# Guillaume-SOULIER/SOS-Radiative-Transfer

Hardware: AMD Instinct MI355X
Metric: SOS columns/sec to 1e-4 convergence (Ntau=200, Nmu=128) (higher is better)
Workload: dtype f64

## Files before the change

include/sosrt.h:

```cpp
#ifndef SOSRT_H
#define SOSRT_H

#ifdef __cplusplus
extern "C" {
#endif

typedef struct sosrt_handle sosrt_t;

#define SOSRT_OK              0
#define SOSRT_E_INVALID      -1
#define SOSRT_E_HIP          -2
#define SOSRT_E_STATE        -3
#define SOSRT_E_NOMEM        -4

#define SOSRT_COL_OK           0
#define SOSRT_COL_INDEXERROR   1
#define SOSRT_COL_MAXORDERS    2
#define SOSRT_COL_INTERNAL     3

#define SOSRT_GEOM_THREE_ZONE  0
#define SOSRT_GEOM_SINGLE_SLAB 1

#define SOSRT_SURFACE_NONE       0
#define SOSRT_SURFACE_SPECULAR   1
// ... 49 lines not shown
int sosrt_set_columns_zones(sosrt_t* h, int B, int surface, int nzmax, const int* nz, const int* zone_r0, const int* zone_mix,
                            const double* mu0, const double* grd_alb, const double* alb_atm, const double* dtau_atm,
                            const double* zone_alb_aer, const double* zone_dtau_aer, const double* tauStar_tot);

int sosrt_first_order(sosrt_t* h, int B, const double* tau, const double* P0_atm, const double* P0_aer,
                      double* I1_out);
int sosrt_source(sosrt_t* h, int B, const double* In_1, double* Jn_out);
int sosrt_transport(sosrt_t* h, int B, const double* tau, const double* Jn, double* In_out, int* status_out);

int sosrt_solve(sosrt_t* h, int B, const double* tau, const double* P0_atm, const double* P0_aer,
                double tol, const double* I1_in,
                double* I_out, double* I_saved_out, int* n_orders_out, int* status_out);
int sosrt_solve_dev(sosrt_t* h, int B, const double* d_tau, const double* d_P0_atm, const double* d_P0_aer,
                    double tol, const double* d_I1_in,
                    double* d_I_out, double* d_I_saved_out, int* d_n_orders_out, int* d_status_out);
int sosrt_last_solve_stats(sosrt_t* h, int* max_orders_run, long long* sum_orders);

int sosrt_fluxes(sosrt_t* h, int B, const double* tau, const double* I, int beam_norm,
                 double* flux_down, double* flux_up);

int sosrt_epilogue_dev(sosrt_t* h, int B, const double* d_tau, const double* d_I, int beam_norm,
                       const double* d_z_profile, double* d_flux_down, double* d_flux_up, double* d_diffusivity,
                       double* d_heating_rate, double* d_net_toa);
int sosrt_epilogue(sosrt_t* h, int B, int beam_norm, const double* z_profile, double* flux_down, double* flux_up,
                   double* diffusivity, double* heating_rate, double* net_toa);

#define SOSRT_PHASE_ISO       0
#define SOSRT_PHASE_RAYLEIGH  1
#define SOSRT_PHASE_HG        2
#define SOSRT_PHASE_TABLE     3
int sosrt_phase_table(sosrt_t* h, const double* tab_mu, const double* tab_p, int ntab);
int sosrt_phase_table_dev(sosrt_t* h, const double* d_tab_mu, const double* d_tab_p, int ntab);

#define SOSRT_MIE_MAX_X 20000.0
#define SOSRT_MIE_MAX_MX 200000.0
#define SOSRT_MIE_MAX_WORKSPACE (2ull << 30)
int sosrt_mie_ensembles(sosrt_t* h, int S, const double* wl, const double* m_re, const double* m_im, const double* r_m,
                        const double* sig, int nb_radius, double r_min, double r_max, int ntab, double* p_out, double* bulk_out);
int sosrt_mie_ensembles_dev(sosrt_t* h, int S, const double* wl, const double* m_re, const double* m_im, const double* r_m,
                            const double* sig, int nb_radius, double r_min, double r_max, int ntab, double* d_p_out,
                            double* d_bulk_out);
int sosrt_mie_efficiencies(sosrt_t* h, int K, const double* m_re, const double* m_im, const double* x, double* out);
int sosrt_mie_timing(sosrt_t* h, double* ms );

int sosrt_phase_p0_dev(sosrt_t* h, int B, int kind, double g, const double* d_mu0, double* d_P0_out);
int sosrt_phase_p0(sosrt_t* h, int B, int kind, double g, const double* mu0, double* P0_out);
int sosrt_phase_matrix(sosrt_t* h, int kind, double g, double* P_out);
int sosrt_phase_matrix_dev(sosrt_t* h, int kind, double g, double* d_P_out);

#define SOSRT_MAX_MODES 64
int sosrt_phase_modes(sosrt_t* h, int kind, double g, int m_first, int m_count, int nphi, double* P_out);
int sosrt_phase_p0_modes_dev(sosrt_t* h, int B, int kind, double g, int m_first, int m_count, int nphi, const double* d_mu0,
                             double* d_P0_out);
int sosrt_phase_p0_modes(sosrt_t* h, int B, int kind, double g, int m_first, int m_count, int nphi, const double* mu0,
                         double* P0_out);
int sosrt_set_order_targets(sosrt_t* h, const int* d_targets);
int sosrt_azimuth_accumulate_dev(sosrt_t* h, int B, int m, const double* d_Im, int nlev, const int* d_levels, int nphi_out,
                                 const double* d_phi, double* d_out);

int sosrt_comm_unique_id(void* id_out);
int sosrt_comm_init(sosrt_t* h, int rank, int world, const void* unique_id);
int sosrt_gather(sosrt_t* h, int root, const long long* counts, const double* d_send, double* d_recv);
int sosrt_comm_destroy(sosrt_t* h);

int sosrt_limit_mu_down(sosrt_t* h, int R, int idx, const double* rows, double* out);
int sosrt_asymptotic_down(sosrt_t* h, int R, int stride, const int* len, const double* J, const double* tau,
                          const double* tau_t, const double* mu, double* out);

int sosrt_plan_weights(sosrt_t* h, double* w_out );
int sosrt_plan_fold(sosrt_t* h, int which , double* W_out );
int sosrt_plan_fix_table(sosrt_t* h, int idx, int* s0, int* ns, double* C_out);
int sosrt_plan_fix_count(double tau_ref, int N);
#define SOSRT_PLAN_GEMM_DENSE        0
#define SOSRT_PLAN_GEMM_LIVE64       1
#define SOSRT_PLAN_GEMM_LIVE32       2
#define SOSRT_PLAN_GEMM_LIVE32_DEEP  3
#define SOSRT_PLAN_GEMM_LIVE16_REGS  4
#define SOSRT_PLAN_TRANSPORT_GENERAL 0
#define SOSRT_PLAN_TRANSPORT_FAST    1
#define SOSRT_PLAN_TRANSPORT_RING    3
#define SOSRT_PLAN_TRANSPORT_SCAN    4
int sosrt_plan_launch(sosrt_t* h, int batch, int live, int surface, int zones, int cus, int* out );

#define SOSRT_K_GEMM      0
#define SOSRT_K_TRANSPORT 1
#define SOSRT_K_FIRST     2
#define SOSRT_K_SMALLMU   3
#define SOSRT_K_ORDER_LOOP 4
#define SOSRT_K_COUNT     5
int sosrt_profile_enable(sosrt_t* h, int on);
int sosrt_profile_reset(sosrt_t* h);
int sosrt_profile_get(sosrt_t* h, int kernel, double* total_ms, long long* launches, double* work );

int sosrt_debug_stamps(sosrt_t* h, unsigned long long* d_stamps);

int sosrt_microbench(sosrt_t* h, int which, double* result);

#ifdef __cplusplus
}
#endif
#endif
```

sos-radiative-transfer_amd/csrc/api.hip:

```cpp
#include <hip/hip_runtime.h>

#include <algorithm>
#include <cmath>
#include <cstdarg>
#include <cstdio>
#include <cstdlib>
#include <chrono>
#include <cstring>
#include <mutex>
#include <new>
#include <string>
#include <vector>

#include "../../include/sosrt.h"
#include "comm.hpp"
#include "kernels.hpp"
#include "plan.hpp"

using namespace sosrt;

namespace {
thread_local std::string g_err;

int fail(int code, const char* fmt, ...) {
// ... 32 lines not shown
    int saved_slots = 0;
    bool gpu = false;
    hipStream_t own_stream = nullptr, stream = nullptr;
    static constexpr int kMaxGroups = 2;
    hipStream_t stream2 = nullptr;
    hipEvent_t ev_fork = nullptr, ev_join = nullptr;
    int ngroups = 1, want_groups = 0, split_min = 48;
    int split_at = -1;
    int prio2 = 0;
    int coresident_pad = 0;
    int diag_ks_mult = 1;
    int coresident_slots = 3;
    double stagger = 1.0;
    int gb[kMaxGroups + 1] = {0, 0, 0};
    int main_off[kMaxGroups + 1] = {0, 0, 0};
    int slab_off[kMaxGroups + 1] = {0, 0, 0};
    Plan plan;
    bool have_grid = false, have_phase = false, have_aer = false, have_cols = false;
    int B = 0, geom = 0, surface = 0;
    std::vector<double> Wa_h, Wr_h;
    Grid g{};
    double *d_mu = nullptr, *d_Wa = nullptr, *d_Wr = nullptr, *d_wfdn = nullptr, *d_wfup = nullptr;
    double *d_w = nullptr;
    int first_order_mode = SOSRT_FIRST_ORDER_CODED;
    double *d_phi = nullptr;
    double *d_z = nullptr;
    double *d_tab = nullptr;
    double *d_modetab = nullptr;
    size_t modetab_cap = 0;
    const int* d_targets = nullptr;
    int ntab = 0;
    char* d_mie = nullptr;
    char* h_mie = nullptr;
    size_t mie_cap = 0, mie_hcap = 0;
    hipEvent_t mie_ev = nullptr, mie_t[4] = {nullptr, nullptr, nullptr, nullptr};
    bool mie_timed = false;
    bool resident = false;
    int resident_B = 0;
    FixTab* d_fix = nullptr;
    int* d_small = nullptr;
    int *d_idx_up = nullptr, *d_idx_down = nullptr;
    int *d_nz = nullptr, *d_zr0 = nullptr, *d_zmix = nullptr;
    double *d_zwr = nullptr, *d_zdtr = nullptr;
    int max_nz = 1;
    bool simple_zones = true;
    double* d_scal = nullptr;
    ColDesc* d_desc = nullptr;
    double *d_rca = nullptr, *d_rcr = nullptr;
    int* d_slabrows = nullptr;
    int* d_mainrows = nullptr;
    int nslab = 0, nmain = 0;
    int max_main = 0, max_slab = 0;
    static constexpr int kMaxMixGroups = 32;
    static constexpr int kMaxMixGroupsSets = 128;
    static constexpr size_t kMixCacheBytes = 256ull << 20;
    int mix_groups_max = 1 << 30;
    bool wr_on_device = false;
    int nsets = 1;
    std::vector<std::vector<double>> Wrx_h;
    double* d_Wrsets = nullptr;
    size_t wrsets_capacity = 0;
    double* d_Wrsets_s = nullptr;
    size_t wrsets_s_capacity = 0;
    int* d_mixset = nullptr;
    int max_set_used = 0;
    int p0_zones = 0;
    double* d_P0rz = nullptr;
    size_t p0rz_capacity = 0;
    std::vector<int> c_nz, c_zr0, c_zmix, c_zset;
    std::vector<double> c_zwr, c_zdtr, c_alb_atm, c_dtau_atm;
    int mix_groups = 0;
    bool mix_dirty = true;
    double *d_Wmix = nullptr, *d_mixca = nullptr, *d_mixcr = nullptr;
    int* d_mixgroup = nullptr;
    int* d_slabtilegroup = nullptr;
    int contraction = SOSRT_CONTRACT_F64;
    double asymmetry = 0;
    bool sym_ok = false;
    bool sym_dirty = true, symmix_dirty = true, symsets_dirty = true;
    double *d_Wa_s = nullptr, *d_Wr_s = nullptr, *d_Wmix_s = nullptr;
    int lr_rank = -1;
    double lr_residual = 0;
    double *d_lrU = nullptr, *d_lrV = nullptr;
    size_t mixs_capacity = 0;
    float *d_Wa32 = nullptr, *d_Wmix32 = nullptr;
    size_t mix32_capacity = 0;
    bool w32_dirty = true;
    int* d_livelist = nullptr;
    size_t mix_capacity = 0;
    double *d_tau = nullptr, *d_P0a = nullptr, *d_P0r = nullptr;
    double *d_Jn = nullptr, *d_InA = nullptr, *d_InB = nullptr, *d_I = nullptr, *d_E = nullptr;
    int use_etab = 1;
    int *d_active = nullptr, *d_norders = nullptr, *d_status = nullptr, *d_redo = nullptr, *d_erep = nullptr;
    int *d_nactive_sets = nullptr, *d_nactive = nullptr;
    int nactive_set = 0;
    unsigned long long* d_tauhash = nullptr;
    int transport_mode = 3;
    int scan_cols = 200;
    bool ring_ok = false, scan_ok = false, scan_split_ok = false;
    int scan_split = 1;
    int cu_count = 0;
    double* d_scan_scratch = nullptr;
    int* d_scan_sync = nullptr;
    int gemm_tail_cols = 1 << 30;
    double gemm_tail_frac = 0.6;
    int gemm_small_cols = 200;
    int dense_live_list = 1;
    int gemm_regs_cols = -1;
    bool fast_ok = false;
    double* d_ratio = nullptr;
    int* h_pub = nullptr;
    bool need_small = true;
    int pub_seq = 0;
    int last_max_orders = 0;
    long long last_sum_orders = 0;
    Prof prof[kMaxGroups];
    int order_loop = 0;
    double ol_frac = 0.5;
    int* d_olsync = nullptr;
    int* h_oldone = nullptr;
    unsigned long long* d_ollog = nullptr;
    int ol_launches = 0, ol_refused = 0;
    bool ol_group_used[kMaxGroups] = {false, false};
    Rccl::comm_t comm = nullptr;
    int comm_rank = -1, comm_world = 0;
};

namespace {

size_t field_elems(const sosrt_handle* h) { return (size_t)h->max_batch * h->L * h->D; }

template <class T>
int dalloc(T** p, size_t n) {
    hipError_t e = hipMalloc((void**)p, n * sizeof(T));
    if (e != hipSuccess) return fail(SOSRT_E_NOMEM, "hipMalloc of %zu bytes failed: %s", n * sizeof(T), hipGetErrorString(e));
    return 0;
}

void mie_linspace(double a, double b, int n, double* out) {
    if (n == 1) { out[0] = a; return; }
    const double step = (b - a) / (n - 1);
    for (int i = 0; i < n; ++i) {
        volatile double t = i * step;
        out[i] = t + a;
    }
    out[n - 1] = b;
}

bool prof_room(Prof& p) {
    if (p.used + 2 > p.ev.size()) {
        const size_t n0 = p.ev.size();
        p.ev.resize(n0 + 4096);
        for (size_t i = n0; i < p.ev.size(); ++i)
            if (hipEventCreateWithFlags(&p.ev[i], hipEventDisableSystemFence) != hipSuccess) { p.ev.resize(i); break; }
        if (p.used + 2 > p.ev.size()) return false;
    }
    if (p.nint >= p.kind.size()) {
        const size_t n = p.kind.size() + 4096;
        p.kind.resize(n, -1); p.first.resize(n, 0); p.last.resize(n, 0);
    }
    return true;
}
hipStream_t group_stream(sosrt_handle* h, int grp) { return grp == 0 ? h->stream : h->stream2; }
void prof_begin(sosrt_handle* h, int kind, int grp = 0) {
    Prof& p = h->prof[grp];
    p.open = -1;
// ... 118 lines not shown
    if (!std::isfinite(wmax)) return -1;
    int rank = -1;
    for (int r = 0; r <= kLowRankMax; ++r) {
        size_t at = 0;
        const double amax = absmax(R, &at);
        *residual = wmax > 0 ? amax / wmax : amax;
        if (std::isnan(amax)) return -1;
        if (amax <= SOSRT_LOWRANK_TOL * wmax) { rank = r; break; }
        if (r == kLowRankMax) return -1;
        const int i = (int)(at / D), j = (int)(at % D);
        const long double piv = R[at];
        for (int k = 0; k < D; ++k) Ut[(size_t)r * D + k] = (double)(R[(size_t)k * D + j] / piv);
        for (int m = 0; m < D; ++m) V[(size_t)r * D + m] = R[(size_t)i * D + m];
        for (int k = 0; k < D; ++k) {
            const long double u = Ut[(size_t)r * D + k];
            double* row = &R[(size_t)k * D];
            const double* v = &V[(size_t)r * D];
            for (int m = 0; m < D; ++m) row[m] = (double)(row[m] - u * v[m]);
        }
    }
    double res = 0;
    for (int k = 0; k < D; ++k)
        for (int m = 0; m < D; ++m) {
            long double uv = 0;
            for (int q = 0; q < rank; ++q) uv += (long double)Ut[(size_t)q * D + k] * V[(size_t)q * D + m];
            const double d = std::fabs((double)(W[(size_t)k * D + m] - uv));
            if (!(d <= res)) res = d;
        }
    *residual = wmax > 0 ? res / wmax : res;
    return (res <= SOSRT_LOWRANK_TOL * wmax) ? rank : -1;
}

int ensure_matrices(sosrt_handle* h, hipStream_t s) {
    const Grid& g = h->g;
    const size_t per = (size_t)g.Dp * g.Wld;
    const bool mixed = h->mix_groups > 0 && h->mix_dirty;
    if (mixed) {
        prof_break(h);
        const bool sets = h->max_set_used > 0;
        launch_wmix(s, per, h->mix_groups, h->d_Wa, sets ? h->d_Wrsets : h->d_Wr, h->d_mixca, h->d_mixcr, h->d_Wmix,
                    sets ? h->d_mixset : nullptr);
        h->mix_dirty = false;
        h->symmix_dirty = true;
    }
    if (!use_sym(h)) return 0;
    if (h->sym_dirty) {
        prof_break(h);
        if (!h->d_Wa_s) { if (int e = dalloc(&h->d_Wa_s, per)) return e; }
        if (!h->d_Wr_s) { if (int e = dalloc(&h->d_Wr_s, per)) return e; }
        launch_symfold(s, 1, g.N, g.D, g.Dp, g.Wld, h->d_Wa, h->d_Wa_s);
        launch_symfold(s, 1, g.N, g.D, g.Dp, g.Wld, h->d_Wr, h->d_Wr_s);
        h->sym_dirty = false;
        h->symsets_dirty = true;
    }
    if (h->symsets_dirty && h->nsets > 1 && h->mix_groups == 0 && h->max_set_used > 0) {
        prof_break(h);
        {
            if (per * h->nsets > h->wrsets_s_capacity) {
                if (h->d_Wrsets_s) hipFree(h->d_Wrsets_s);
                h->d_Wrsets_s = nullptr; h->wrsets_s_capacity = 0;
                if (int e = dalloc(&h->d_Wrsets_s, per * h->nsets)) return e;
                h->wrsets_s_capacity = per * h->nsets;
            }
            launch_symfold(s, h->nsets, g.N, g.D, g.Dp, g.Wld, h->d_Wrsets, h->d_Wrsets_s);
        }
        h->symsets_dirty = false;
    }
    if (h->mix_groups > 0 && h->symmix_dirty) {
        prof_break(h);
        const size_t need = per * h->mix_groups;
        if (need > h->mixs_capacity) {
            if (h->d_Wmix_s) hipFree(h->d_Wmix_s);
            h->d_Wmix_s = nullptr; h->mixs_capacity = 0;
            if (int e = dalloc(&h->d_Wmix_s, need)) return e;
            h->mixs_capacity = need;
        }
        launch_symfold(s, h->mix_groups, g.N, g.D, g.Dp, g.Wld, h->d_Wmix, h->d_Wmix_s);
        h->symmix_dirty = false;
    }
    return 0;
}

void run_source(sosrt_handle* h, const double* In_1, double* Jn, const int* active, int tail_cols = 0, int pub_tag = 0,
                int grp = -1, bool all_live = false, bool regs_tile = false, int dense_live_cap = 0) {
    const int g0 = grp < 0 ? 0 : grp, g1 = grp < 0 ? h->ngroups : grp + 1;
    const int pg = grp < 0 ? 0 : grp;
    hipStream_t s = group_stream(h, pg);
    GemmArgs ga;
    ga.A = In_1; ga.Wa = h->d_Wa; ga.Wr = h->d_Wr; ga.ca = h->d_rca; ga.cr = h->d_rcr;
    if (h->nslab > 0) {
        ga.rows_main = h->d_mainrows + h->main_off[g0];
        ga.n_main = h->main_off[g1] - h->main_off[g0];
    } else {
        ga.rows_main = nullptr;
        ga.n_main = (h->gb[g1] - h->gb[g0]) * h->L;
        ga.A = In_1 + (size_t)h->gb[g0] * h->L * h->D;
        Jn += (size_t)h->gb[g0] * h->L * h->D;
        ga.ca = h->d_rca + (size_t)h->gb[g0] * h->L;
        ga.cr = h->d_rcr + (size_t)h->gb[g0] * h->L;
        if (active) active += h->gb[g0];
    }
    ga.rows_slab = h->d_slabrows + h->slab_off[g0]; ga.n_slab = h->slab_off[g1] - h->slab_off[g0];
    ga.D = h->g.D; ga.Dp = h->g.Dp; ga.Wld = h->g.Wld; ga.L = h->L; ga.C = Jn; ga.active = active;
    if (grp >= 0 && h->ngroups > 1) ga.pad_lds = h->coresident_pad;
    if (pub_tag) {
        ga.nactive = h->d_nactive + pg; ga.need_small = h->d_nactive + sosrt_handle::kMaxGroups;
        ga.host_pub = h->h_pub + 8 * pg; ga.tag = pub_tag;
    }
    ga.check_tiles = all_live ? 0 : 1;
    if (ensure_matrices(h, s)) return;
    if (h->mix_groups > 0) {
        ga.Wmix = h->d_Wmix; ga.mix_group = h->d_mixgroup; ga.slab_tile_group = h->d_slabtilegroup + h->slab_off[g0] / 32;
    }
    const bool two_pass_sets = h->mix_groups == 0 && h->max_set_used > 0 && h->nslab > 0;
    if (two_pass_sets) {
        ga.Wr = h->d_Wrsets; ga.mix_group = h->d_mixgroup; ga.slab_tile_group = h->d_slabtilegroup + h->slab_off[g0] / 32;
    }
    if (use_lowrank(h)) { ga.lr_rank = h->lr_rank; ga.lrU = h->d_lrU; ga.lrV = h->d_lrV; }
    if (use_sym(h)) {
        ga.sym = 1; ga.Ks = (h->g.N + GEMM_KC - 1) / GEMM_KC * GEMM_KC;
#ifdef SOSRT_DIAG
        if (h->diag_ks_mult > 1 && ga.Ks * h->diag_ks_mult <= h->g.Dp) ga.Ks *= h->diag_ks_mult;
#endif
        ga.Wa = h->d_Wa_s; ga.Wr = two_pass_sets ? h->d_Wrsets_s : h->d_Wr_s;
        if (ga.Wmix) ga.Wmix = h->d_Wmix_s;
    }
    if (h->contraction == SOSRT_CONTRACT_F32) {
        if (h->w32_dirty) {
            prof_break(h);
            const size_t per = (size_t)h->g.Dp * h->g.Wld;
            launch_to_float(s, per, h->d_Wa, h->d_Wa32);
            if (h->mix_groups > 0) launch_to_float(s, per * h->mix_groups, h->d_Wmix, h->d_Wmix32);
            h->w32_dirty = false;
        }
        prof_begin(h, SOSRT_K_GEMM, pg);
        launch_gemm_f32(s, ga, h->d_Wa32, h->d_Wmix32);
        prof_end(h, SOSRT_K_GEMM, pg);
        return;
    }
    prof_begin(h, SOSRT_K_GEMM, pg);
    if (tail_cols > 0 && active && h->nslab >= 0) {
        ga.col0 = h->nslab > 0 ? h->gb[g0] : 0; ga.B = h->gb[g1] - h->gb[g0];
        ga.max_main = h->max_main; ga.max_slab = h->max_slab;
        ga.idx_up = h->nslab > 0 ? h->d_idx_up : nullptr; ga.idx_down = h->nslab > 0 ? h->d_idx_down : nullptr;
        ga.live_list = h->d_livelist + h->gb[g0]; ga.live_cap = tail_cols;
        launch_gemm_tail(s, ga, tail_cols, tail_cols <= h->gemm_small_cols, regs_tile);
    } else {
        if (dense_live_cap > 0 && active && h->nslab >= 0) {
            ga.col0 = h->nslab > 0 ? h->gb[g0] : 0; ga.B = h->gb[g1] - h->gb[g0];
            ga.live_list = h->d_livelist + h->gb[g0]; ga.live_cap = dense_live_cap;
        }
        launch_gemm(s, ga);
    }
    prof_end(h, SOSRT_K_GEMM, pg);
}

struct SolveShape {
    bool ring_like = false;
    bool fast = false;
    int nzcap = kRingZones;
    int ring_mode = 1;
};
SolveShape solve_shape(const sosrt_handle* h, int max_nz) {
    SolveShape sh;
    sh.ring_like = h->transport_mode >= 2 && h->ring_ok && (max_nz <= kRingZones || transport_ring_fits(h->g, max_nz));
    sh.fast = h->transport_mode >= 1 && h->fast_ok && (max_nz <= kRingZones || sh.ring_like);
    sh.nzcap = max_nz > kRingZones ? max_nz : kRingZones;
    sh.ring_mode = (h->transport_mode >= 2 && h->ring_ok) ? 3 : 1;
    return sh;
}
struct OrderInputs {
    int nb = 0;
    int known = 0;
    int surface = SOSRT_SURFACE_NONE;
    bool simple_zones = true;
    bool slabs_mixed = true;
    bool need_small = false;
    bool saving = false;
    int orders_left = 1 << 30;
    int cu_share = 0;
};
struct LaunchPlan {
    int tail_cols = 0;
    int live_cap = 0;
    int gemm = SOSRT_PLAN_GEMM_DENSE;
    int transport = SOSRT_PLAN_TRANSPORT_GENERAL;
    int parts = 1;
    int repair = 0;
    int order_loop = 0;
    int ol_parts = 0;
    int ol_grid = 0;
};
LaunchPlan plan_order(const sosrt_handle* h, const SolveShape& sh, const OrderInputs& in) {
    LaunchPlan pl;
    const Grid& g = h->g;
    const bool live_tiling = h->contraction != SOSRT_CONTRACT_F32 && in.simple_zones && in.known <= h->gemm_tail_cols &&
                             (in.known <= h->gemm_tail_frac * in.nb || in.nb <= h->gemm_small_cols) &&
                             (in.known < in.nb || in.nb <= h->gemm_small_cols);
    pl.tail_cols = live_tiling ? in.known : 0;
    pl.gemm = !live_tiling ? SOSRT_PLAN_GEMM_DENSE
                           : (pl.tail_cols <= h->gemm_small_cols ? ((use_sym(h) && pl.tail_cols <= 32) ? SOSRT_PLAN_GEMM_LIVE32_DEEP : SOSRT_PLAN_GEMM_LIVE32)
                                                                 : SOSRT_PLAN_GEMM_LIVE64);
    {
        const int nct = (g.D + GEMM_BN - 1) / GEMM_BN;
        const int auto_cap = (3 * h->cu_count / 2) / (((g.L + 15) / 16 + 1) * nct);
        const int cap = h->gemm_regs_cols >= 0 ? h->gemm_regs_cols : auto_cap;
        if (live_tiling && use_sym(h) && pl.tail_cols <= cap && 16 * (g.D + 2) * 8 <= 150 * 1024 &&
            ((g.N + GEMM_KC - 1) / GEMM_KC * GEMM_KC) % 64 == 0) pl.gemm = SOSRT_PLAN_GEMM_LIVE16_REGS;
    }
    pl.live_cap = live_tiling ? pl.tail_cols : ((h->contraction != SOSRT_CONTRACT_F32 && h->dense_live_list && in.known < in.nb) ? in.known : 0);
    {
        const int cols_now = pl.live_cap > 0 ? pl.live_cap : in.nb;
        const int split_cap = sh.ring_mode == 3 ? h->cu_count : 4 * h->cu_count;
        const bool can_split = h->scan_split && h->scan_split_ok && transport_scan_parts(g) * cols_now <= split_cap &&
                               (in.surface == SOSRT_SURFACE_SPECULAR || in.surface == SOSRT_SURFACE_NONE);
        const bool want_scan = h->transport_mode == 4 || (h->transport_mode == 3 && cols_now <= h->scan_cols);
        const bool split = can_split && transport_scan_fits(g, sh.nzcap, true) && (sh.fast || (h->use_etab && h->transport_mode >= 3));
        const bool scan = want_scan && ((sh.fast && sh.ring_mode == 3 && h->scan_ok && transport_scan_fits(g, sh.nzcap, false)) || split);
        pl.transport = scan ? SOSRT_PLAN_TRANSPORT_SCAN
                            : (!sh.fast ? SOSRT_PLAN_TRANSPORT_GENERAL : (sh.ring_mode == 3 ? SOSRT_PLAN_TRANSPORT_RING : SOSRT_PLAN_TRANSPORT_FAST));
        if (scan && split) pl.parts = transport_scan_parts(g);
        pl.repair = (h->N - 3 > 61 && pl.transport == SOSRT_PLAN_TRANSPORT_FAST) ? 1 : 0;
    }
    if (h->order_loop && in.cu_share > 0 && h->transport_mode == 3 && sh.fast && sh.ring_mode == 3 && sh.nzcap <= kRingZones &&
        use_sym(h) && in.simple_zones && in.slabs_mixed && !in.saving && !in.need_small && in.orders_left >= 1 &&
        in.known <= kOrderLoopMaxCols) {
        Grid gt = g;
        gt.nsmall = 0;
        const bool split_ok = h->scan_split && (in.surface == SOSRT_SURFACE_SPECULAR || in.surface == SOSRT_SURFACE_NONE) && order_loop_ok(gt, true);
        const int sp = order_loop_parts(gt, true);
        if (split_ok && sp * in.known <= h->ol_frac * in.cu_share) {
            pl.order_loop = 1; pl.ol_parts = sp;
        } else if (order_loop_ok(gt, false) && in.known <= h->ol_frac * in.cu_share) {
            pl.order_loop = 1; pl.ol_parts = 1;
        }
        if (pl.order_loop) pl.ol_grid = in.cu_share;
    }
    return pl;
}

std::mutex g_ol_mutex;
int g_ol_held[64];
int ol_acquire(int device, int total, int want, int least) {
    if (device < 0 || device >= 64) return 0;
    std::lock_guard<std::mutex> lk(g_ol_mutex);
    int got = total - g_ol_held[device];
    if (got > want) got = want;
    if (got < least || got <= 0) return 0;
    g_ol_held[device] += got;
    return got;
}
void ol_release(int device, int n) {
    if (device < 0 || device >= 64 || n <= 0) return;
    std::lock_guard<std::mutex> lk(g_ol_mutex);
    g_ol_held[device] -= n;
}

}

extern "C" {

const char* sosrt_last_error(void) { return g_err.c_str(); }
int sosrt_version(void) { return SOSRT_VERSION; }

int sosrt_plan_fix_count(double tau_ref, int N) { return fix_count(tau_ref, N); }

int sosrt_create(int device, int L, int N, int max_batch, int max_orders, sosrt_t** out) {
    if (!out) return fail(SOSRT_E_INVALID, "out is null");
    *out = nullptr;
    if (L < 2) return fail(SOSRT_E_INVALID, "nb_layers must be >= 2 (got %d)", L);
    if (N < 4) return fail(SOSRT_E_INVALID, "nb_angles must be >= 4 (got %d)", N);
    if (N > 1024) return fail(SOSRT_E_INVALID, "nb_angles must be <= 1024 (got %d)", N);
    if (max_batch < 1 || max_orders < 1) return fail(SOSRT_E_INVALID, "max_batch and max_orders must be >= 1");
    {
        const int nt = (N + 63) / 64 * 64;
        const size_t need = (size_t)(3 * (size_t)L + nt + nt / 64 + 4) * sizeof(double);
        if (need > 64 * 1024)
            return fail(SOSRT_E_INVALID, "nb_layers = %d does not fit: at most %d layers at nb_angles = %d", L,
                        (int)((64 * 1024 / sizeof(double) - nt - nt / 64 - 4) / 3), N);
    }
    sosrt_handle* h = new (std::nothrow) sosrt_handle();
    if (!h) return fail(SOSRT_E_NOMEM, "out of host memory");
    h->device = device; h->L = L; h->N = N; h->D = 2 * N; h->max_batch = max_batch; h->max_orders = max_orders;
    h->order_budget = max_orders;
    h->saved_slots = max_orders;
    h->gpu = device >= 0;
    h->cu_count = 256;
    if (const char* ev = getenv("SOSRT_ETAB")) h->use_etab = atoi(ev);
    if (const char* ev = getenv("SOSRT_CONTRACT"))
        if (strcmp(ev, "full") == 0) h->contraction = SOSRT_CONTRACT_F64_FULL;
    if (const char* ev = getenv("SOSRT_TRANSPORT"))
        h->transport_mode = strcmp(ev, "general") == 0 ? 0 : (strcmp(ev, "ring") == 0 ? 2 : (strcmp(ev, "scan") == 0 ? 4 : (strcmp(ev, "auto") == 0 ? 3 : 1)));
    if (const char* ev = getenv("SOSRT_SCAN_COLS")) h->scan_cols = atoi(ev);
    if (const char* ev = getenv("SOSRT_SCAN_SPLIT")) h->scan_split = atoi(ev);
    if (const char* ev = getenv("SOSRT_GEMM_TAIL")) h->gemm_tail_cols = atoi(ev);
    if (const char* ev = getenv("SOSRT_GEMM_TAIL_FRAC")) h->gemm_tail_frac = atof(ev);
    if (const char* ev = getenv("SOSRT_GEMM_SMALL")) h->gemm_small_cols = atoi(ev);
    if (const char* ev = getenv("SOSRT_DENSE_LIVE_LIST")) h->dense_live_list = atoi(ev) != 0;
    if (const char* ev = getenv("SOSRT_GEMM_REGS")) h->gemm_regs_cols = atoi(ev);
    if (const char* ev = getenv("SOSRT_GROUPS")) h->want_groups = atoi(ev) >= 2 ? 2 : (atoi(ev) == 1 ? 1 : 0);
    if (const char* ev = getenv("SOSRT_SPLIT_MIN")) h->split_min = atoi(ev);
    if (const char* ev = getenv("SOSRT_MIX_GROUPS")) h->mix_groups_max = atoi(ev);
#ifdef SOSRT_DIAG
    if (const char* ev = getenv("SOSRT_STAGGER")) h->stagger = atof(ev);
    if (const char* ev = getenv("SOSRT_GROUP_SPLIT")) h->split_at = atoi(ev);
    if (const char* ev = getenv("SOSRT_GROUP_PRIO")) h->prio2 = atoi(ev);
    if (const char* ev = getenv("SOSRT_GEMM_PAD_LDS")) h->coresident_pad = atoi(ev);
    if (const char* ev = getenv("SOSRT_GEMM_KS_MULT")) h->diag_ks_mult = atoi(ev);
#endif
    if (const char* ev = getenv("SOSRT_GROUP_RING_SLOTS")) h->coresident_slots = atoi(ev);
    if (const char* ev = getenv("SOSRT_ORDER_LOOP")) h->order_loop = atoi(ev) != 0;
    if (const char* ev = getenv("SOSRT_RING_SLOTS")) g_ring_slots = atoi(ev);
#ifdef SOSRT_RING_DEBUG
    if (const char* ev = getenv("SOSRT_RING_DEBUG")) g_ring_debug = atoi(ev);
#endif
    Grid& g = h->g;
    g.L = L; g.N = N; g.D = 2 * N;
    g.Dp = (g.D + GEMM_KC - 1) / GEMM_KC * GEMM_KC;
    g.Wld = (g.D + GEMM_BN - 1) / GEMM_BN * GEMM_BN;
    if (h->gpu) {
        int e = 0;
        auto body = [&]() -> int {
            HIPCHK(hipSetDevice(device));
            HIPCHK(hipStreamCreateWithFlags(&h->own_stream, hipStreamDefault));
            h->stream = h->own_stream;
            HIPCHK(hipEventCreateWithFlags(&h->ev_fork, hipEventDisableTiming));
            HIPCHK(hipEventCreateWithFlags(&h->ev_join, hipEventDisableTiming));
            const size_t mb = max_batch, fe = field_elems(h);
            if ((e = dalloc(&h->d_mu, g.D))) return e;
            if ((e = dalloc(&h->d_Wa, (size_t)g.Dp * g.Wld))) return e;
            if ((e = dalloc(&h->d_Wr, (size_t)g.Dp * g.Wld))) return e;
            if ((e = dalloc(&h->d_lrU, (size_t)kLowRankMax * g.D))) return e;
            if ((e = dalloc(&h->d_lrV, (size_t)kLowRankMax * g.D))) return e;
            if ((e = dalloc(&h->d_wfdn, N))) return e;
            if ((e = dalloc(&h->d_wfup, N))) return e;
            if ((e = dalloc(&h->d_w, g.D))) return e;
            if ((e = dalloc(&h->d_phi, 2 * kNPhi))) return e;
            if ((e = dalloc(&h->d_z, L))) return e;
            if ((e = dalloc(&h->d_fix, 4))) return e;
            if ((e = dalloc(&h->d_small, N))) return e;
            if ((e = dalloc(&h->d_idx_up, mb))) return e;
            if ((e = dalloc(&h->d_idx_down, mb))) return e;
            if ((e = dalloc(&h->d_nz, mb))) return e;
            if ((e = dalloc(&h->d_zr0, mb * kMaxZones))) return e;
            if ((e = dalloc(&h->d_zmix, mb * kMaxZones))) return e;
            if ((e = dalloc(&h->d_zwr, mb * kMaxZones))) return e;
            if ((e = dalloc(&h->d_zdtr, mb * kMaxZones))) return e;
            if ((e = dalloc(&h->d_scal, 7 * mb))) return e;
            if ((e = dalloc(&h->d_desc, mb))) return e;
            if ((e = dalloc(&h->d_rca, mb * L))) return e;
            if ((e = dalloc(&h->d_rcr, mb * L))) return e;
            if ((e = dalloc(&h->d_slabrows, mb * L + 64 * (size_t)sosrt_handle::kMaxMixGroupsSets * sosrt_handle::kMaxGroups))) return e;
            if ((e = dalloc(&h->d_slabtilegroup, mb * L / 32 + 2 * sosrt_handle::kMaxMixGroupsSets * sosrt_handle::kMaxGroups + 2))) return e;
            if ((e = dalloc(&h->d_mainrows, mb * L))) return e;
            if ((e = dalloc(&h->d_tau, mb * L))) return e;
            if ((e = dalloc(&h->d_P0a, mb * g.D))) return e;
            if ((e = dalloc(&h->d_P0r, mb * g.D))) return e;
            if ((e = dalloc(&h->d_Jn, fe))) return e;
            if ((e = dalloc(&h->d_InA, fe))) return e;
            if ((e = dalloc(&h->d_InB, fe))) return e;
            if ((e = dalloc(&h->d_I, fe))) return e;
            if ((e = dalloc(&h->d_E, fe))) return e;
            if ((e = dalloc(&h->d_active, mb))) return e;
            if ((e = dalloc(&h->d_norders, mb))) return e;
            if ((e = dalloc(&h->d_status, mb))) return e;
            if ((e = dalloc(&h->d_nactive_sets, 2 * (sosrt_handle::kMaxGroups + 1)))) return e;
            HIPCHK(hipMemset(h->d_nactive_sets, 0, 2 * (sosrt_handle::kMaxGroups + 1) * sizeof(int)));
            h->d_nactive = h->d_nactive_sets;
            if ((e = dalloc(&h->d_redo, mb))) return e;
            if ((e = dalloc(&h->d_erep, mb))) return e;
            if ((e = dalloc(&h->d_mixgroup, mb))) return e;
            if ((e = dalloc(&h->d_livelist, mb))) return e;
            if ((e = dalloc(&h->d_mixca, sosrt_handle::kMaxMixGroupsSets))) return e;
            if ((e = dalloc(&h->d_mixcr, sosrt_handle::kMaxMixGroupsSets))) return e;
            if ((e = dalloc(&h->d_mixset, sosrt_handle::kMaxMixGroupsSets))) return e;
            if ((e = dalloc(&h->d_tauhash, mb))) return e;
            if ((e = dalloc(&h->d_ratio, mb))) return e;
            if ((e = dalloc(&h->d_scan_scratch, mb * transport_scan_scratch_doubles()))) return e;
            if ((e = dalloc(&h->d_scan_sync, 2 * mb))) return e;
            if ((e = dalloc(&h->d_olsync, sosrt_handle::kMaxGroups * order_loop_sync_ints(kOrderLoopMaxCols)))) return e;
            HIPCHK(hipHostMalloc((void**)&h->h_oldone, 2 * sosrt_handle::kMaxGroups * sizeof(int), hipHostMallocCoherent));
            memset(h->h_oldone, 0, 2 * sosrt_handle::kMaxGroups * sizeof(int));
            HIPCHK(hipMemset(h->d_scan_sync, 0, 2 * mb * sizeof(int)));
            HIPCHK(hipDeviceGetAttribute(&h->cu_count, hipDeviceAttributeMultiprocessorCount, device));
            HIPCHK(hipHostMalloc((void**)&h->h_pub, (8 * sosrt_handle::kMaxGroups + 2) * sizeof(int), hipHostMallocCoherent));
            memset(h->h_pub, 0, (8 * sosrt_handle::kMaxGroups + 2) * sizeof(int));

            HIPCHK(hipMemset(h->d_Wa, 0, (size_t)g.Dp * g.Wld * sizeof(double)));
            HIPCHK(hipMemset(h->d_Wr, 0, (size_t)g.Dp * g.Wld * sizeof(double)));
            HIPCHK(hipMemset(h->d_status, 0, mb * sizeof(int)));
            HIPCHK(hipMemset(h->d_redo, 0, mb * sizeof(int)));
            HIPCHK(hipMemset(h->d_tau, 0, mb * L * sizeof(double)));
            return 0;
        };
        if ((e = body())) { sosrt_destroy(h); return e; }
        g.mu = h->d_mu; g.Wa = h->d_Wa; g.Wr = h->d_Wr; g.fix = h->d_fix; g.small_lanes = h->d_small;
        g.wflux_dn = h->d_wfdn; g.wflux_up = h->d_wfup; g.nsmall = 0;
    }
    *out = h;
    return 0;
}

int sosrt_destroy(sosrt_t* h) {
    if (!h) return 0;
    if (h->gpu) {
        hipSetDevice(h->device);
        if (h->comm) { rccl().CommDestroy(h->comm); h->comm = nullptr; }
        if (h->own_stream) hipStreamSynchronize(h->own_stream);
        void* ptrs[] = {h->d_mu, h->d_Wa, h->d_Wr, h->d_wfdn, h->d_wfup, h->d_fix, h->d_small, h->d_idx_up,
                        h->d_idx_down, h->d_scal, h->d_desc, h->d_rca, h->d_rcr, h->d_slabrows, h->d_mainrows, h->d_tau, h->d_P0a,
                        h->d_P0r, h->d_Jn, h->d_InA, h->d_InB, h->d_I, h->d_E, h->d_active, h->d_norders, h->d_status,
                        h->d_nactive_sets, h->d_ratio, h->d_redo, h->d_erep, h->d_tauhash, h->d_Wmix, h->d_mixca, h->d_mixcr,
                        h->d_mixgroup, h->d_Wa_s, h->d_Wr_s, h->d_Wmix_s, h->d_scan_scratch, h->d_scan_sync, h->d_w, h->d_phi, h->d_z, h->d_tab, h->d_slabtilegroup, h->d_livelist, h->d_Wa32, h->d_Wmix32, h->d_nz, h->d_zr0, h->d_zmix, h->d_zwr, h->d_zdtr, h->d_olsync, h->d_ollog, h->d_modetab, h->d_lrU, h->d_lrV, h->d_Wrsets, h->d_Wrsets_s, h->d_mixset, h->d_P0rz};
        for (void* p : ptrs)
            if (p) hipFree(p);
        if (h->h_pub) hipHostFree(h->h_pub);
        if (h->h_oldone) hipHostFree(h->h_oldone);
        if (h->d_mie) hipFree(h->d_mie);
        if (h->h_mie) hipHostFree(h->h_mie);
        if (h->mie_ev) hipEventDestroy(h->mie_ev);
        for (auto& e : h->mie_t)
            if (e) hipEventDestroy(e);

        for (auto& p : h->prof)
            for (auto& e : p.ev) hipEventDestroy(e);
        if (h->stream2) { hipStreamSynchronize(h->stream2); hipStreamDestroy(h->stream2); }
        if (h->ev_fork) hipEventDestroy(h->ev_fork);
        if (h->ev_join) hipEventDestroy(h->ev_join);
        if (h->own_stream) hipStreamDestroy(h->own_stream);
    }
    delete h;
    return 0;
}

int sosrt_set_stream(sosrt_t* h, void* s) {
    if (int e = need_gpu(h)) return e;
    h->stream = (hipStream_t)s;
    return 0;
}

int sosrt_use_own_stream(sosrt_t* h) {
    if (int e = need_gpu(h)) return e;
    h->stream = h->own_stream;
    return 0;
}

int sosrt_set_saved_orders(sosrt_t* h, int slots) {
    if (!h) return fail(SOSRT_E_INVALID, "null handle");
    if (slots < 1 || slots > h->max_orders) return fail(SOSRT_E_INVALID, "slots must be in 1..max_orders=%d (got %d)", h->max_orders, slots);
    h->saved_slots = slots;
    return 0;
}

int sosrt_set_order_budget(sosrt_t* h, int max_orders) {
    if (!h) return fail(SOSRT_E_INVALID, "null handle");
    if (max_orders < 1 || max_orders > h->max_orders)
        return fail(SOSRT_E_INVALID, "the order budget must be in 1..max_orders=%d of sosrt_create (got %d)", h->max_orders, max_orders);
    h->order_budget = max_orders;
    return 0;
}

int sosrt_set_first_order(sosrt_t* h, int mode) {
    if (int e = need_gpu(h)) return e;
    if (mode != SOSRT_FIRST_ORDER_CODED && mode != SOSRT_FIRST_ORDER_README) return fail(SOSRT_E_INVALID, "unknown first-order mode %d", mode);
    if (mode == SOSRT_FIRST_ORDER_README && (h->nsets > 1 || h->p0_zones > 0))
        return fail(SOSRT_E_INVALID, "SOSRT_FIRST_ORDER_README reads one aerosol matrix: it cannot be combined with several phase sets");
    if (mode == SOSRT_FIRST_ORDER_README && h->geom != SOSRT_GEOM_THREE_ZONE)
        return fail(SOSRT_E_INVALID, "the README's Lambertian first order needs the three-zone geometry (it has a surface)");
    h->first_order_mode = mode;
    return 0;
}

int sosrt_set_contraction(sosrt_t* h, int mode) {
    if (int e = need_gpu(h)) return e;
    if (mode != SOSRT_CONTRACT_F64 && mode != SOSRT_CONTRACT_F32 && mode != SOSRT_CONTRACT_F64_FULL && mode != SOSRT_CONTRACT_F64_DENSE) return fail(SOSRT_E_INVALID, "unknown contraction mode %d", mode);
    if (mode == SOSRT_CONTRACT_F32) {
        HIPCHK(hipSetDevice(h->device));
        const size_t per = (size_t)h->g.Dp * h->g.Wld;
        if (!h->d_Wa32) { if (int e = dalloc(&h->d_Wa32, per)) return e; }
        h->w32_dirty = true;
    }
    h->contraction = mode;
    return 0;
}

int sosrt_set_order_loop(sosrt_t* h, int mode) {
    if (!h) return fail(SOSRT_E_INVALID, "null handle");
    if (mode < 0 || mode > 2) return fail(SOSRT_E_INVALID, "order-loop mode must be 0, 1 or 2 (got %d)", mode);
    h->order_loop = mode;
    return 0;
}

int sosrt_order_loop_stats(sosrt_t* h, int* launches, int* refused, long long* column_orders) {
    if (!h) return fail(SOSRT_E_INVALID, "null handle");
    if (launches) *launches = h->ol_launches;
    if (refused) *refused = h->ol_refused;
    if (column_orders) {
        *column_orders = 0;
        if (h->gpu && h->ol_launches > 0) {
            HIPCHK(hipSetDevice(h->device));
            HIPCHK(hipStreamSynchronize(h->stream));
            if (h->stream2) HIPCHK(hipStreamSynchronize(h->stream2));
            for (int k = 0; k < sosrt_handle::kMaxGroups; ++k) {
                if (!h->ol_group_used[k]) continue;
                int v = 0;
                HIPCHK(hipMemcpy(&v, h->d_olsync + (size_t)k * order_loop_sync_ints(kOrderLoopMaxCols) + kOlOrders, sizeof v, hipMemcpyDeviceToHost));
                *column_orders += v;
            }
        }
    }
    return 0;
}

int sosrt_plan_launch(sosrt_t* h, int batch, int live, int surface, int zones, int cus, int* out) {
    if (!h || !out) return fail(SOSRT_E_INVALID, "null argument");
    if (!h->have_grid) return fail(SOSRT_E_STATE, "sosrt_set_grid has not been called");
    if (batch < 1 || live < 0 || live > batch) return fail(SOSRT_E_INVALID, "need 0 <= live <= batch, batch >= 1");
    if (zones < 1 || zones > kMaxZones) return fail(SOSRT_E_INVALID, "zones must be in 1..%d", kMaxZones);
    int want = h->want_groups;
    if (want == 0) want = batch > h->split_min ? 2 : 1;
    const int ng = (want >= 2 && batch >= h->split_min && batch >= 2) ? 2 : 1;
    const int nb = ng == 2 ? batch / 2 : batch;
    const int saved_cus = h->cu_count;
    if (cus > 0) h->cu_count = cus;
    const SolveShape sh = solve_shape(h, zones);
    OrderInputs oi;
    oi.nb = nb; oi.known = live < nb ? live : nb; oi.surface = surface;
    oi.simple_zones = zones == 3 || zones == 1;
    oi.cu_share = h->cu_count / ng;
    const bool saved_sym = h->sym_ok;
    if (!h->have_phase) h->sym_ok = true;
    const LaunchPlan pl = plan_order(h, sh, oi);
    h->sym_ok = saved_sym;
    h->cu_count = saved_cus;
    out[0] = ng; out[1] = pl.gemm; out[2] = pl.tail_cols; out[3] = pl.transport; out[4] = pl.parts; out[5] = pl.repair;
    out[6] = pl.order_loop; out[7] = pl.ol_parts; out[8] = pl.ol_grid;
    return 0;
}

int sosrt_phase_asymmetry(sosrt_t* h, double* asymmetry, int* uses_symmetry) {
    if (!h) return fail(SOSRT_E_INVALID, "null handle");
    if (!h->have_phase) return fail(SOSRT_E_STATE, "sosrt_set_phase has not been called");
    if (asymmetry) *asymmetry = h->asymmetry;
    if (uses_symmetry) *uses_symmetry = use_sym(h) ? 1 : 0;
    return 0;
}

int sosrt_phase_rank(sosrt_t* h, int* rank, double* residual, int* uses) {
    if (!h) return fail(SOSRT_E_INVALID, "null handle");
    if (!h->have_phase) return fail(SOSRT_E_STATE, "sosrt_set_phase has not been called");
    if (rank) *rank = h->lr_rank;
    if (residual) *residual = h->lr_residual;
    if (uses) *uses = use_lowrank(h) ? 1 : 0;
    return 0;
}

int sosrt_synchronize(sosrt_t* h) {
    if (int e = need_gpu(h)) return e;
    HIPCHK(hipStreamSynchronize(h->stream));
    return 0;
}

int sosrt_set_grid(sosrt_t* h, const double* mu) {
    if (!h || !mu) return fail(SOSRT_E_INVALID, "null argument");
    for (int k = 0; k < h->D; ++k)
        if (!std::isfinite(mu[k])) return fail(SOSRT_E_INVALID, "mu[%d] is not finite", k);
    for (int k = 0; k < h->N; ++k) {
        if (!(mu[k] <= 0)) return fail(SOSRT_E_INVALID, "mu[%d]=%g: the first nb_angles directions must be <= 0", k, mu[k]);
        if (!(mu[h->N + k] >= 0)) return fail(SOSRT_E_INVALID, "mu[%d]=%g: the last nb_angles directions must be >= 0", h->N + k, mu[h->N + k]);
    }
    h->plan.set_grid(h->N, mu);
    for (int b = 0; b < 4; ++b)
        if (h->plan.fix[b].idx > kFixMaxIdx) return fail(SOSRT_E_INVALID, "nb_angles too large for the extrapolation tables");
    h->have_grid = true;
    h->have_phase = false;
    h->fast_ok = transport_fast_ok(h->plan);
    if (h->gpu) {
        HIPCHK(hipSetDevice(h->device));
        HIPCHK(hipMemcpy(h->d_mu, mu, h->D * sizeof(double), hipMemcpyHostToDevice));
        HIPCHK(hipMemcpy(h->d_wfdn, h->plan.wflux_dn.data(), h->N * sizeof(double), hipMemcpyHostToDevice));
        HIPCHK(hipMemcpy(h->d_wfup, h->plan.wflux_up.data(), h->N * sizeof(double), hipMemcpyHostToDevice));
        HIPCHK(hipMemcpy(h->d_w, h->plan.w.data(), h->D * sizeof(double), hipMemcpyHostToDevice));
        {
            double phi[kNPhi], tab[2 * kNPhi];
            const double step = 3.141592653589793 / (kNPhi - 1);
            for (int q = 0; q < kNPhi; ++q) phi[q] = q * step;
            phi[kNPhi - 1] = 3.141592653589793;
            for (int q = 0; q < kNPhi; ++q) {
                tab[q] = std::cos(0 - phi[q]);
                tab[kNPhi + q] = ((q > 0 ? phi[q] - phi[q - 1] : 0.0) + (q + 1 < kNPhi ? phi[q + 1] - phi[q] : 0.0)) / 2;
            }
            HIPCHK(hipMemcpy(h->d_phi, tab, sizeof tab, hipMemcpyHostToDevice));
        }
        std::vector<FixTab> ft(4);
        for (int b = 0; b < 4; ++b) {
            const FixTable& t = h->plan.fix[b];
            memset(&ft[b], 0, sizeof(FixTab));
            ft[b].idx = t.idx; ft[b].s0 = t.s0; ft[b].ns = t.ns;
            for (size_t i = 0; i < t.C.size(); ++i) ft[b].C[i] = t.C[i];
        }
        HIPCHK(hipMemcpy(h->d_fix, ft.data(), 4 * sizeof(FixTab), hipMemcpyHostToDevice));
        h->g.nsmall = (int)h->plan.small_lanes.size();
        if (h->g.nsmall)
            HIPCHK(hipMemcpy(h->d_small, h->plan.small_lanes.data(), h->g.nsmall * sizeof(int), hipMemcpyHostToDevice));
    }
    h->g.nsmall = (int)h->plan.small_lanes.size();
    h->ring_ok = h->fast_ok && transport_ring_ok(h->g);
    h->scan_ok = h->ring_ok && transport_scan_ok(h->g);
    h->scan_split_ok = transport_scan_split_ok(h->g);
    return 0;
}

static int mix_group_cap(const sosrt_handle* h, bool sets);
static int set_phase_impl(sosrt_handle* h, const double* P_atm, int S, const double* P_aer, const double* d_P_aer = nullptr) {
    if (!h || !P_atm) return fail(SOSRT_E_INVALID, "null argument");
    if (!h->have_grid) return fail(SOSRT_E_STATE, "sosrt_set_grid has not been called");
    if (h->have_cols && h->max_set_used >= (S > 0 ? S : 1))
        return fail(SOSRT_E_INVALID, "the current columns use aerosol set %d, but only %d set(s) are given (sosrt_set_columns resets them to set 0)",
                    h->max_set_used, S > 0 ? S : 1);
// ... 530 lines not shown
    const double* src = I1 + (size_t)b * n;
    for (size_t i = tid; i < n; i += blockDim.x) {
        const double v = src[i];
        In1[(size_t)b * n + i] = v;
        I[(size_t)b * n + i] = v;
        if (saved) saved[(size_t)b * saved_col_stride + i] = v;
    }
    if (tid == 0) {
        double a = 1.0 / src[g.N];
        for (int m = g.N + 1; m < g.D; ++m) { const double x = 1.0 / src[m]; if (x > a) a = x; }
        const double* last = src + (size_t)(g.L - 1) * g.D;
        double bb = 1.0 / last[0];
        for (int m = 1; m < g.N; ++m) { const double x = 1.0 / last[m]; if (x > bb) bb = x; }
        const double r = (bb > a) ? bb : a;
        cv.ratio[b] = r; cv.norders[b] = 1; cv.status[b] = SOSRT_COL_OK;
        const int go = conv_go(cv, b, 1, r) ? 1 : 0;
        cv.active[b] = go;
        if (go) atomicAdd(cv.nactive, 1);
    }
}

int sosrt_solve_dev(sosrt_t* h, int B, const double* d_tau, const double* d_P0_atm, const double* d_P0_aer, double tol,
                    const double* d_I1_in, double* d_I_out, double* d_I_saved_out, int* d_n_orders_out,
                    int* d_status_out) {
    if (int e = check_ready(h, B, true)) return e;
    if (!d_tau || !d_I_out) return fail(SOSRT_E_INVALID, "null argument");
    if (!d_I1_in && !d_P0_atm) return fail(SOSRT_E_INVALID, "P0_atm is required unless I1 is supplied");
    if (!d_I1_in && h->geom == SOSRT_GEOM_THREE_ZONE && !d_P0_aer) return fail(SOSRT_E_INVALID, "three-zone geometry needs P0_aer");
    if (h->max_orders >= 65536) return fail(SOSRT_E_INVALID, "max_orders must be < 65536");
    HIPCHK(hipSetDevice(h->device));
    if (int e = ensure_w32(h)) return e;
    hipStream_t s = h->stream;
    const Grid& g = h->g;
    const size_t LD = (size_t)h->L * h->D;
    const size_t saved_stride = (size_t)h->saved_slots * LD;
    const int NG = h->ngroups;

    prof_break(h);
    h->nactive_set ^= 1;
    h->d_nactive = h->d_nactive_sets + h->nactive_set * (sosrt_handle::kMaxGroups + 1);
    SolveSetup su;
    su.zero_next = h->d_nactive_sets + (h->nactive_set ^ 1) * (sosrt_handle::kMaxGroups + 1);
    su.n_zero = sosrt_handle::kMaxGroups + 1;
    su.redo = h->d_redo;
    su.hash = h->d_tauhash;
    su.scan_sync = h->d_scan_sync;
    launch_prepare(s, g, B, h->geom, h->surface, scalars_of(h), d_tau, h->d_desc, h->d_rca, h->d_rcr,
                   h->d_nactive + sosrt_handle::kMaxGroups, su);
    h->need_small = true;
    const int small_tag = ((++h->pub_seq) & 0x3fffffff) | 0x40000000;
    bool small_published = false;
    const SolveShape shape = solve_shape(h, h->max_nz);
    const bool fast = shape.fast;
    const int nzcap = shape.nzcap;
    if (h->use_etab || fast) {
        launch_tau_groups(s, g, B, d_tau, h->d_tauhash, h->d_erep, h->d_nactive + sosrt_handle::kMaxGroups,
                          h->h_pub + 8 * sosrt_handle::kMaxGroups, small_tag);
        launch_attenuation(s, g, B, d_tau, h->d_E, h->d_erep);
        small_published = true;
    }
    if (int e = ensure_matrices(h, s)) return e;
    bool forked = false;
    int ol_held[sosrt_handle::kMaxGroups] = {0, 0};
    auto bail = [&](int code) {
        if (forked && hipEventRecord(h->ev_join, h->stream2) == hipSuccess) (void)hipStreamWaitEvent(s, h->ev_join, 0);
        for (int k = 0; k < NG; ++k)
            if (ol_held[k]) {
                (void)hipStreamSynchronize(group_stream(h, k));
                ol_release(h->device, ol_held[k]);
                ol_held[k] = 0;
            }
        return code;
    };

    struct GroupState {
        int b0 = 0, nb = 0, n = 1, known = 0;
        bool done = false, started = false;
        bool ol_pending = false, ol_off = false;
        int ol_tag = 0;
        unsigned ol_polls = 0;
        double *In_1 = nullptr, *In = nullptr;
        Conv cv;
    } gs[sosrt_handle::kMaxGroups];
    h->ol_launches = 0; h->ol_refused = 0;
    for (bool& u : h->ol_group_used) u = false;
    bool used_order_loop = false;
    const int tagbase = ((++h->pub_seq) & 0x3fff) << 16;
    for (int k = 0; k < NG; ++k) {
        GroupState& q = gs[k];
        q.b0 = h->gb[k]; q.nb = h->gb[k + 1] - h->gb[k]; q.known = q.nb;
        q.In_1 = h->d_InA; q.In = h->d_InB;
        if (!d_I1_in && h->first_order_mode != SOSRT_FIRST_ORDER_README) q.In_1 = d_I_out;
        q.cv = make_conv(h, tol);
        q.cv.active += q.b0; q.cv.norders += q.b0; q.cv.status += q.b0; q.cv.ratio += q.b0; q.cv.redo += q.b0;
        q.cv.nactive = h->d_nactive + k;
        if (h->d_targets) q.cv.target = h->d_targets + q.b0;
    }
    auto start_group = [&](int k) {
        GroupState& q = gs[k];
        q.started = true;
        hipStream_t sg = group_stream(h, k);
        const size_t fo = (size_t)q.b0 * LD;
        prof_begin(h, SOSRT_K_FIRST, k);
        if (d_I1_in)
            hipLaunchKernelGGL(k_init_from_I1, dim3(q.nb), dim3(256), 0, sg, g, d_I1_in + fo, q.In_1 + fo, d_I_out + fo,
                               d_I_saved_out ? d_I_saved_out + (size_t)q.b0 * saved_stride : nullptr, saved_stride, q.cv);
        else if (h->first_order_mode == SOSRT_FIRST_ORDER_README)
            launch_first_order_readme(sg, g, h->d_w, q.nb, d_tau + (size_t)q.b0 * h->L, d_P0_atm + (size_t)q.b0 * g.D,
                                      d_P0_aer ? d_P0_aer + (size_t)q.b0 * g.D : nullptr, h->d_desc + q.b0, q.In_1 + fo,
                                      d_I_out + fo, d_I_saved_out ? d_I_saved_out + (size_t)q.b0 * saved_stride : nullptr,
                                      saved_stride, q.cv, 1);
        else
            launch_first_order(sg, g, q.nb, d_tau + (size_t)q.b0 * h->L, d_P0_atm + (size_t)q.b0 * g.D,
                               d_P0_aer ? d_P0_aer + (size_t)q.b0 * g.D * (h->p0_zones > 0 ? h->p0_zones : 1) : nullptr, h->d_desc + q.b0,
                               d_I_out + fo, nullptr, d_I_saved_out ? d_I_saved_out + (size_t)q.b0 * saved_stride : nullptr, saved_stride,
                               q.cv, 1, h->p0_zones);
        prof_end(h, SOSRT_K_FIRST, k);
    };
    start_group(0);
    if (NG > 1) {
        HIPCHK(hipEventRecord(h->ev_fork, s));
        HIPCHK(hipStreamWaitEvent(h->stream2, h->ev_fork, 0));
        forked = true;
    }
    if (small_published && g.nsmall > 0) {
        volatile int* slot = h->h_pub + 8 * sosrt_handle::kMaxGroups;
        const auto t0 = std::chrono::steady_clock::now();
        for (unsigned it = 1; __atomic_load_n(&slot[1], __ATOMIC_ACQUIRE) != small_tag; ++it) {
            if ((it & 0x3fff) == 0 && std::chrono::steady_clock::now() - t0 > std::chrono::seconds(120))
                return bail(fail(SOSRT_E_HIP, "order loop: no progress for 120 s"));
            __builtin_ia32_pause();
        }
        h->need_small = slot[0] != 0;
    }
    int live_groups = NG, n_max = 1;
    while (live_groups > 0) {
        bool progressed = false;
        for (int k = 0; k < NG; ++k) {
            GroupState& q = gs[k];
            if (q.done) continue;
            if (q.ol_pending) {
                volatile int* dw = h->h_oldone + 2 * k;
                if (__atomic_load_n(&dw[1], __ATOMIC_ACQUIRE) != q.ol_tag) {
                    if ((++q.ol_polls & 0x3fff) != 0) continue;
                    const hipError_t qe = hipStreamQuery(group_stream(h, k));
                    if (qe != hipSuccess && qe != hipErrorNotReady) return bail(fail(SOSRT_E_HIP, "order loop: %s", hipGetErrorString(qe)));
                    if (qe == hipSuccess && __atomic_load_n(&dw[1], __ATOMIC_ACQUIRE) != q.ol_tag)
                        return bail(fail(SOSRT_E_HIP, "order loop: the order-loop launch ended without reporting"));
                    continue;
                }
                const int state = dw[0];
                q.ol_pending = false;
                ol_release(h->device, ol_held[k]);
                ol_held[k] = 0;
                progressed = true;
#ifdef SOSRT_OL_STAMPS
                if (h->d_ollog && getenv("SOSRT_OL_LOG")) {
                    std::vector<unsigned long long> lg(65001);
                    (void)hipStreamSynchronize(group_stream(h, k));
                    (void)hipMemcpy(lg.data(), h->d_ollog, lg.size() * 8, hipMemcpyDeviceToHost);
                    if (FILE* f = fopen(getenv("SOSRT_OL_LOG"), "a")) {
                        fprintf(f, "# launch columns<=%d order0=%d events=%llu\n", q.known, q.n + 1, lg[0]);
                        for (unsigned long long i = 0; i < lg[0] && i < 65000; ++i)
                            fprintf(f, "%llu %llu %llu %llu\n", lg[1 + i] >> 48, (lg[1 + i] >> 40) & 0xff, (lg[1 + i] >> 32) & 0xff, lg[1 + i] & 0xffffffffull);
                        fclose(f);
                    }
                }
// ... 14 lines not shown
                                     w[kOlArrive], w[kOlLeft], q.n + 1, q.known, cols.c_str()));
                }
                q.ol_off = true;
                ++h->ol_refused;
            }
            if (!q.started) {
                const GroupState& p = gs[k - 1];
                if (!(p.done || (p.n >= 2 && p.known <= h->stagger * p.nb))) continue;
                start_group(k);
            }
            progressed = true;
            if (q.n >= h->order_budget) { q.done = true; --live_groups; continue; }
            if (q.n >= 2) {
                const int live = wait_published(h, k, tagbase + q.n - 1);
                if (live < 0) return bail(live);
                if (live == 0) { q.done = true; --live_groups; continue; }
                q.known = live;
            }
            hipStream_t sg = group_stream(h, k);
            const size_t fo = (size_t)q.b0 * LD;
            const double* tau_g = d_tau + (size_t)q.b0 * h->L;
            const int* erep_g = h->d_erep + q.b0;
            OrderInputs oi;
            oi.nb = q.nb; oi.known = q.known; oi.surface = h->surface;
            oi.simple_zones = h->simple_zones; oi.slabs_mixed = h->nslab == 0 || h->mix_groups > 0;
            oi.need_small = g.nsmall > 0 && h->need_small; oi.saving = d_I_saved_out != nullptr;
            oi.orders_left = h->order_budget - q.n;
            oi.cu_share = (q.ol_off || h->d_targets) ? 0 : h->cu_count / NG;
            LaunchPlan pl = plan_order(h, shape, oi);
            if (pl.order_loop) {
                const int got = ol_acquire(h->device, h->cu_count, pl.ol_grid, (int)(pl.ol_parts * q.known / h->ol_frac));
                if (got == 0) { oi.cu_share = 0; pl = plan_order(h, shape, oi); }
                else { pl.ol_grid = got; ol_held[k] = got; }
            }
            if (pl.order_loop && h->order_loop == 2) pl.ol_grid = 2 * h->cu_count;
            if (pl.order_loop) {
                OrderLoopArgs oa;
                Grid gt = g;
                gt.nsmall = 0;
                oa.t = TransportArgs{gt, tau_g, h->d_Jn + fo, nullptr, d_I_out + fo, nullptr, 0, h->d_desc + q.b0, q.cv, 0, 1, h->d_E, erep_g, nullptr};
                oa.t.nzcap = kRingZones;
                oa.t.scan_split = pl.ol_parts > 1 ? 1 : 0;
                oa.t.scan_scratch = h->d_scan_scratch + (size_t)q.b0 * transport_scan_scratch_doubles();
                oa.t.scan_sync = h->d_scan_sync + 2 * q.b0;
                GemmArgs& ga = oa.gm;
                ga.A = nullptr; ga.Wa = h->d_Wa_s; ga.Wr = h->d_Wr_s; ga.ca = h->d_rca; ga.cr = h->d_rcr;
                ga.D = g.D; ga.Dp = g.Dp; ga.Wld = g.Wld; ga.L = h->L; ga.C = h->d_Jn;
                ga.sym = 1; ga.Ks = (g.N + GEMM_KC - 1) / GEMM_KC * GEMM_KC;
                if (use_lowrank(h)) { ga.lr_rank = h->lr_rank; ga.lrU = h->d_lrU; ga.lrV = h->d_lrV; }
                ga.max_main = h->max_main; ga.max_slab = h->max_slab;
                ga.idx_up = h->nslab > 0 ? h->d_idx_up : nullptr; ga.idx_down = h->nslab > 0 ? h->d_idx_down : nullptr;
                if (h->mix_groups > 0) { ga.Wmix = h->d_Wmix_s; ga.mix_group = h->d_mixgroup; }
                oa.in0 = q.In_1;
                oa.gbufP = q.In;
                oa.gbufQ = (q.In_1 == d_I_out) ? h->d_InA : q.In_1;
                oa.bufP = oa.gbufP + fo; oa.bufQ = oa.gbufQ + fo;
                oa.order0 = q.n + 1; oa.kmax = h->order_budget - q.n;
                oa.B = q.nb; oa.col0 = q.b0;
                oa.fixcap = (int)(0.06 * g.N) + 1;
                oa.sync = h->d_olsync + (size_t)k * order_loop_sync_ints(kOrderLoopMaxCols);
                oa.host_done = h->h_oldone + 2 * k;
                oa.tag = q.ol_tag = ((++h->pub_seq) & 0x3fffffff) | 0x40000000;
#ifdef SOSRT_OL_STAMPS
                if (getenv("SOSRT_OL_LOG")) {
                    if (!h->d_ollog) { if (int e = dalloc(&h->d_ollog, 65001)) return bail(e); }
                    HIPCHK(hipMemsetAsync(h->d_ollog, 0, 8, sg));
                    oa.log = h->d_ollog;
                }
#endif
                prof_break(h);
                HIPCHK(hipMemsetAsync(oa.sync, 0, order_loop_sync_ints(q.known) * sizeof(int), sg));
                prof_begin(h, SOSRT_K_ORDER_LOOP, k);
                const hipError_t le = launch_order_loop(sg, pl.ol_grid, pl.ol_parts > 1, oa);
                prof_end(h, SOSRT_K_ORDER_LOOP, k);
                if (le != hipSuccess) return bail(fail(SOSRT_E_HIP, "order-loop launch failed: %s", hipGetErrorString(le)));
                q.ol_pending = true;
                used_order_loop = true;
                ++h->ol_launches;
                continue;
            }
            const int n = ++q.n;
            n_max = n > n_max ? n : n_max;
            const int tail_cols = pl.tail_cols;
            run_source(h, q.In_1, h->d_Jn, h->d_active, tail_cols, tagbase + n - 1, k, q.known == q.nb, pl.gemm == SOSRT_PLAN_GEMM_LIVE16_REGS,
                       tail_cols > 0 ? 0 : pl.live_cap);
            if (g.nsmall > 0 && h->need_small) {
                prof_begin(h, SOSRT_K_SMALLMU, k);
                launch_smallmu(sg, g, q.nb, tau_g, h->d_Jn + fo, q.In + fo, h->d_desc + q.b0, q.cv.active);
                prof_end(h, SOSRT_K_SMALLMU, k);
            }
            prof_begin(h, SOSRT_K_TRANSPORT, k);
            double* sv_n = (d_I_saved_out && n <= h->saved_slots) ? d_I_saved_out + (size_t)q.b0 * saved_stride + (size_t)(n - 1) * LD : nullptr;
            if (pl.transport != SOSRT_PLAN_TRANSPORT_GENERAL) {
                Grid gt = g;
                if (pl.transport >= SOSRT_PLAN_TRANSPORT_RING && !h->need_small) gt.nsmall = 0;
                launch_transport(sg, gt, q.nb, tau_g, h->d_Jn + fo, q.In + fo, d_I_out + fo, sv_n, saved_stride, h->d_desc + q.b0, q.cv, n, 1,
                                 h->d_E, pl.transport, erep_g, pl.live_cap, h->d_livelist + q.b0, NG > 1 ? h->coresident_slots : 0,
                                 pl.parts > 1 ? 1 : 0, h->d_scan_scratch + (size_t)q.b0 * transport_scan_scratch_doubles(),
                                 h->d_scan_sync + 2 * q.b0, nzcap);
                if (pl.repair)
                    launch_transport(sg, g, q.nb, tau_g, h->d_Jn + fo, q.In + fo, d_I_out + fo, sv_n, saved_stride, h->d_desc + q.b0, q.cv, n, 1,
                                     h->d_E, 2, erep_g);
            } else {
                launch_transport(sg, g, q.nb, tau_g, h->d_Jn + fo, q.In + fo, d_I_out + fo, sv_n, saved_stride, h->d_desc + q.b0, q.cv, n, 1,
                                 h->use_etab ? h->d_E : nullptr, 0, erep_g);
            }
            prof_end(h, SOSRT_K_TRANSPORT, k);
            if (q.In_1 == d_I_out) { q.In_1 = q.In; q.In = h->d_InA; }
            else { double* tmp = q.In_1; q.In_1 = q.In; q.In = tmp; }
        }
        if (!progressed) __builtin_ia32_pause();
    }
    if (NG > 1) {
        HIPCHK(hipEventRecord(h->ev_join, h->stream2));
        HIPCHK(hipStreamWaitEvent(s, h->ev_join, 0));
    }
    prof_break(h);
    launch_finalize(s, B, make_conv(h, tol), h->order_budget, d_n_orders_out, d_status_out);
    HIPCHK(hipGetLastError());
    h->last_max_orders = used_order_loop ? -1 : n_max;
    h->last_sum_orders = -1;
    return 0;
}

int sosrt_solve(sosrt_t* h, int B, const double* tau, const double* P0_atm, const double* P0_aer, double tol,
                const double* I1_in, double* I_out, double* I_saved_out, int* n_orders_out, int* status_out) {
    if (int e = check_ready(h, B, true)) return e;
    if (!tau) return fail(SOSRT_E_INVALID, "null argument");
    HIPCHK(hipSetDevice(h->device));
    hipStream_t s = h->stream;
    h->resident = false;
    const size_t LD = (size_t)h->L * h->D, n = (size_t)B * LD;
    HIPCHK(hipMemcpyAsync(h->d_tau, tau, (size_t)B * h->L * sizeof(double), hipMemcpyHostToDevice, s));
    if (P0_atm) HIPCHK(hipMemcpyAsync(h->d_P0a, P0_atm, (size_t)B * h->D * sizeof(double), hipMemcpyHostToDevice, s));
    const double* d_p0r = nullptr;
    if (int e = stage_p0_aer(h, B, P0_aer, s, &d_p0r)) return e;
    double* d_I1 = nullptr;
    double* d_saved = nullptr;
    int rc = 0;
    auto body = [&]() -> int {
        if (I1_in) {
            if (int e = dalloc(&d_I1, n)) return e;
            HIPCHK(hipMemcpyAsync(d_I1, I1_in, n * sizeof(double), hipMemcpyHostToDevice, s));
        }
        if (I_saved_out) {
            if (int e = dalloc(&d_saved, (size_t)B * h->saved_slots * LD)) return e;
            HIPCHK(hipMemsetAsync(d_saved, 0, (size_t)B * h->saved_slots * LD * sizeof(double), s));
        }
        if (int e = sosrt_solve_dev(h, B, h->d_tau, P0_atm ? h->d_P0a : nullptr, d_p0r, tol, d_I1,
                                    h->d_I, d_saved, nullptr, nullptr))
            return e;
        if (I_out) HIPCHK(hipMemcpyAsync(I_out, h->d_I, n * sizeof(double), hipMemcpyDeviceToHost, s));
        if (I_saved_out)
            HIPCHK(hipMemcpyAsync(I_saved_out, d_saved, (size_t)B * h->saved_slots * LD * sizeof(double), hipMemcpyDeviceToHost, s));
        std::vector<int> no(B);
        HIPCHK(hipMemcpyAsync(no.data(), h->d_norders, B * sizeof(int), hipMemcpyDeviceToHost, s));
        if (status_out) HIPCHK(hipMemcpyAsync(status_out, h->d_status, B * sizeof(int), hipMemcpyDeviceToHost, s));
        HIPCHK(hipStreamSynchronize(s));
        long long sum = 0;
        int mx = 1;
        for (int b = 0; b < B; ++b) { sum += no[b] - 1; mx = no[b] > mx ? no[b] : mx; if (n_orders_out) n_orders_out[b] = no[b]; }
        h->last_sum_orders = sum;
        if (h->last_max_orders < 0) h->last_max_orders = mx;
        h->resident = true; h->resident_B = B;
        return 0;
    };
    rc = body();
    if (d_I1) hipFree(d_I1);
    if (d_saved) hipFree(d_saved);
    return rc;
}

int sosrt_last_solve_stats(sosrt_t* h, int* max_orders_run, long long* sum_orders) {
    if (int e = need_gpu(h)) return e;
    if ((h->last_sum_orders < 0 || h->last_max_orders < 0) && h->B > 0) {
        std::vector<int> no(h->B);
        HIPCHK(hipMemcpyAsync(no.data(), h->d_norders, h->B * sizeof(int), hipMemcpyDeviceToHost, h->stream));
        HIPCHK(hipStreamSynchronize(h->stream));
        long long sum = 0;
        int mx = 1;
        for (int v : no) { sum += v - 1; mx = v > mx ? v : mx; }
        h->last_sum_orders = sum;
// ... 729 lines not shown
```

sos-radiative-transfer_amd/csrc/jn_gemm_tile.hpp:

```cpp
#pragma once
#include "kernels.hpp"
#include "transport_util.hpp"

namespace sosrt {

namespace {

typedef double f64x4 __attribute__((ext_vector_type(4)));

constexpr int A_LD = GEMM_KC + 2;
constexpr int B_LD = GEMM_BN + 16;

struct ListRows {
    const int* rows;
    int n;
    __device__ int operator()(int lr) const { return lr < n ? (rows ? rows[lr] : lr) : -1; }
};
struct ColumnRows {
    int base, iu, ns, n;
    bool slab;
    __device__ int operator()(int lr) const {
        if (lr >= n) return -1;
        return base + (slab ? iu + lr : (lr < iu ? lr : lr + ns));
    }
// ... 260 lines not shown
    }
}
template <bool SLAB, bool PRELOADED>
__device__ __forceinline__ void gemm_tile_lone(const GemmArgs& g, double* sRaw, int tile, int bn0, ColumnRows row_of,
                                               LoneFrag& f0, LoneFrag& f1, const double* __restrict__ wmix = nullptr) {
    static_assert(!(SLAB && PRELOADED), "two passes start from the column's own coefficients");
    typedef __attribute__((address_space(3))) void* lds_ptr_t_;
    const int tid = threadIdx.x, lane = tid & 63;
    const int wave = __builtin_amdgcn_readfirstlane(tid) >> 6;
    const int D = g.D, Wld = g.Wld, Nn = D >> 1, Nh = Wld >> 1;
    const int RS = D + 2;
    const int fr = lane & 15, fk = lane >> 4;
    const int nkb = (g.Ks >> 2) / LONE_KB;
    const int nblk = (SLAB ? 2 : 1) * nkb;
    const int grow = row_of(tile * 16 + fr);
    const double cf_a = grow >= 0 ? (wmix ? 1.0 : g.ca[grow]) : 0.0;
    const double cf_r = (SLAB && grow >= 0) ? g.cr[grow] : 0.0;
    const __amdgpu_buffer_rsrc_t rA = make_rsrc(g.A + (size_t)row_of.base * D, g.L * D * 8);
    const int rowbytes = D * 8, pieces = (rowbytes + 1023) / 1024;
    for (int r = wave; r < 16; r += 4) {
        const int gr_ = row_of(tile * 16 + r);
        if (gr_ < 0) continue;
        const int ro = (gr_ - row_of.base) * rowbytes;
        for (int pc = 0; pc < pieces; ++pc)
            if (pc * 1024 + lane * 16 < rowbytes)
                __builtin_amdgcn_raw_ptr_buffer_load_lds(rA, (lds_ptr_t_)(sRaw + (size_t)r * RS + pc * 128), 16, lane * 16, ro + pc * 1024, 0, 0);
    }
    const int mcol = (bn0 >> 1) + wave * 16 + fr;
#define SOSRT_LONE_LOAD(F, blk_)                                                                                  \
    {                                                                                                             \
        const int b_ = (blk_);                                                                                    \
        if (b_ < nblk) {                                                                                          \
            const int pass_ = b_ >= nkb ? 1 : 0;                                                                  \
            lone_load(F, pass_ ? rW1 : rW0, b_ - pass_ * nkb, fk, Wld, Nh, mcol);                                 \
        }                                                                                                         \
    }
    const __amdgpu_buffer_rsrc_t rW0 = make_rsrc(wmix ? wmix : g.Wa, g.Dp * Wld * 8);
    const __amdgpu_buffer_rsrc_t rW1 = make_rsrc(SLAB ? g.Wr : g.Wa, g.Dp * Wld * 8);
    if (!PRELOADED) {
        SOSRT_LONE_LOAD(f0, 0);
        SOSRT_LONE_LOAD(f1, 1);
    }
    asm volatile("s_waitcnt vmcnt(0)" ::: "memory");
    __syncthreads();
    f64x4 accx = (f64x4){0, 0, 0, 0}, accy = (f64x4){0, 0, 0, 0};
    const double* __restrict__ arow = sRaw + (size_t)fr * RS;
#define SOSRT_LONE_COMPUTE(F, blk_)                                                                               \
    {                                                                                                             \
        const int b_ = (blk_);                                                                                    \
        const int pass_ = b_ >= nkb ? 1 : 0;                                                                      \
        const double cf_ = pass_ ? cf_r : cf_a;                                                                   \
        const int k0_ = 4 * (b_ - pass_ * nkb) * LONE_KB + fk;                                                    \
        _Pragma("unroll") for (int q = 0; q < LONE_KB; ++q) {                                                     \
            const int k_ = k0_ + 4 * q;                                                                           \
            const bool ok_ = grow >= 0 && k_ < Nn;                                                                \
            const double a_ = arow[k_], m_ = arow[D - 1 - k_];                  \
            const double u_ = ok_ ? cf_ * (a_ + m_) : 0.0, v_ = ok_ ? cf_ * (a_ - m_) : 0.0;                      \
            accx = __builtin_amdgcn_mfma_f64_16x16x4f64(u_, F.s[q], accx, 0, 0, 0);                               \
            accy = __builtin_amdgcn_mfma_f64_16x16x4f64(v_, F.a[q], accy, 0, 0, 0);                               \
        }                                                                                                         \
    }
    for (int blk = 0; blk < nblk; blk += 2) {
        SOSRT_LONE_COMPUTE(f0, blk);
        SOSRT_LONE_LOAD(f0, blk + 2);
        if (blk + 1 < nblk) {
            SOSRT_LONE_COMPUTE(f1, blk + 1);
            SOSRT_LONE_LOAD(f1, blk + 3);
        }
    }
#undef SOSRT_LONE_LOAD
#undef SOSRT_LONE_COMPUTE
#pragma unroll
    for (int r = 0; r < 4; ++r) {
        const int gr = row_of(tile * 16 + 4 * r + fk);
        if (gr >= 0 && mcol < Nn) {
            const double x = accx[r], y = accy[r];
            g.C[(size_t)gr * D + mcol] = x + y;
            g.C[(size_t)gr * D + D - 1 - mcol] = x - y;
        }
    }
}

constexpr int LR_ROWS = 4;
template <bool COH>
__device__ __forceinline__ void lowrank_rows(const GemmArgs& g, const int (&rows)[LR_ROWS], int lane) {
    const int D = g.D, R = g.lr_rank;
    __amdgpu_buffer_rsrc_t rA[LR_ROWS], rC[LR_ROWS];
    double cf[LR_ROWS];
#pragma unroll
    for (int i = 0; i < LR_ROWS; ++i) {
        const int r = rows[i] >= 0 ? rows[i] : rows[0];
        const int bytes = rows[i] >= 0 ? D * 8 : 0;
        rA[i] = make_rsrc(g.A + (size_t)r * D, bytes);
        rC[i] = make_rsrc(g.C + (size_t)r * D, bytes);
        cf[i] = rows[i] >= 0 ? g.ca[rows[i]] : 0.0;
    }
    const double* __restrict__ U = g.lrU;
    const double* __restrict__ V = g.lrV;
    double m[LR_ROWS][kLowRankMax];
#pragma unroll
    for (int i = 0; i < LR_ROWS; ++i)
#pragma unroll
        for (int q = 0; q < kLowRankMax; ++q) m[i][q] = 0.0;
#pragma unroll 2
    for (int k = 2 * lane; k < D; k += 128) {
        double2 x[LR_ROWS];
#pragma unroll
        for (int i = 0; i < LR_ROWS; ++i) x[i] = bload2_aux<COH ? 16 : 0>(rA[i], k * 8, 0);
#pragma unroll
        for (int q = 0; q < kLowRankMax; ++q) {
            if (q < R) {
                const double2 u = *reinterpret_cast<const double2*>(U + (size_t)q * D + k);
#pragma unroll
                for (int i = 0; i < LR_ROWS; ++i) m[i][q] = __builtin_fma(x[i].y, u.y, __builtin_fma(x[i].x, u.x, m[i][q]));
            }
        }
    }
#pragma unroll
    for (int s = 32; s >= 1; s >>= 1)
#pragma unroll
        for (int q = 0; q < kLowRankMax; ++q)
            if (q < R) {
#pragma unroll
                for (int i = 0; i < LR_ROWS; ++i) m[i][q] += __shfl_xor(m[i][q], s);
            }
#pragma unroll 2
    for (int k = 2 * lane; k < D; k += 128) {
        double2 o[LR_ROWS];
#pragma unroll
        for (int i = 0; i < LR_ROWS; ++i) o[i] = make_double2(0.0, 0.0);
#pragma unroll
        for (int q = 0; q < kLowRankMax; ++q) {
            if (q < R) {
                const double2 v = *reinterpret_cast<const double2*>(V + (size_t)q * D + k);
#pragma unroll
                for (int i = 0; i < LR_ROWS; ++i) {
                    o[i].x = __builtin_fma(m[i][q], v.x, o[i].x);
                    o[i].y = __builtin_fma(m[i][q], v.y, o[i].y);
                }
            }
        }
#pragma unroll
        for (int i = 0; i < LR_ROWS; ++i) bstore2_aux<COH ? 17 : 0>(rC[i], k * 8, 0, make_double2(cf[i] * o[i].x, cf[i] * o[i].y));
    }
}
template <bool COH, class RowOf>
__device__ __forceinline__ void lowrank_tile(const GemmArgs& g, RowOf row_of, int tile, int BM, int bn0, bool check_active) {
    const int nct = (g.D + GEMM_BN - 1) / GEMM_BN, ct = bn0 / GEMM_BN;
    const int lane = threadIdx.x & 63, wave = __builtin_amdgcn_readfirstlane(threadIdx.x) >> 6;
    const int per = (BM - ct + nct - 1) / nct;
    const bool chk = check_active && g.active && g.check_tiles;
    for (int j = LR_ROWS * wave; j < per; j += 4 * LR_ROWS) {
        int rows[LR_ROWS];
        int n = 0;
#pragma unroll
        for (int i = 0; i < LR_ROWS; ++i) {
            int r = j + i < per ? __builtin_amdgcn_readfirstlane(row_of(tile * BM + ct + nct * (j + i))) : -1;
            if (chk && r >= 0 && !g.active[r / g.L]) r = -1;
            rows[i] = r;
            n += r >= 0 ? 1 : 0;
        }
        if (n == 0) continue;
        if (rows[0] < 0)
#pragma unroll
            for (int i = 1; i < LR_ROWS; ++i)
                if (rows[i] >= 0) { rows[0] = rows[i]; rows[i] = -1; break; }
        lowrank_rows<COH>(g, rows, lane);
    }
}

constexpr int TAIL_RT_SLAB = 1;
constexpr int TAIL_RT = 2;

}
}
```

sos-radiative-transfer_amd/csrc/kernels.hip:

```cpp
#include <cstdlib>

#include "kernels.hpp"

#include "../../include/sosrt.h"

namespace sosrt {


typedef double f64x4 __attribute__((ext_vector_type(4)));

#define SOSRT_PI 3.14159265358979323846

__device__ __forceinline__ double wave_fmax(double v) {
#pragma unroll
    for (int o = 32; o > 0; o >>= 1) v = fmax(v, __shfl_xor(v, o, 64));
    return v;
}
__device__ __forceinline__ double wave_sum(double v) {
#pragma unroll
    for (int o = 32; o > 0; o >>= 1) v += __shfl_xor(v, o, 64);
    return v;
}

__device__ double block_pymax(double x, bool valid, double* s_red, int first_tid = 0) {
// ... 927 lines not shown
        } else {
            const double dl = tau[min(t + 1, g.L - 1)] - tau[t];
            if (m > g.N) E = exp(-dl * (1.0 / mu));
        }
        E_all[(size_t)b * LD + i] = E;
    }
}

void launch_attenuation(hipStream_t s, const Grid& g, int B, const double* tau, double* Etab, const int* erep) {
    const int slices = erep ? 64 : 8;
    hipLaunchKernelGGL(k_attenuation, dim3(slices, B), dim3(256), 0, s, g, B, tau, Etab, erep);
}

__global__ void k_tau_rep(int L, const double* __restrict__ tau_all, const unsigned long long* __restrict__ hash,
                          int* __restrict__ erep, const int* __restrict__ need_small, int* __restrict__ host_flag, int tag) {
    const int b = blockIdx.x, lane = threadIdx.x;
    if (host_flag && b == 0 && lane == 0) {
        __hip_atomic_store(host_flag, need_small[0], __ATOMIC_RELAXED, __HIP_MEMORY_SCOPE_SYSTEM);
        __hip_atomic_store(host_flag + 1, tag, __ATOMIC_RELEASE, __HIP_MEMORY_SCOPE_SYSTEM);
    }
    const unsigned long long hb = hash[b];
    const double* tb = tau_all + (size_t)b * L;
    int rep = b;
    for (int c0 = 0; c0 < b && rep == b; c0 += 64) {
        const int c = c0 + lane;
        unsigned long long cand = __ballot(c < b && hash[c] == hb);
        while (cand && rep == b) {
            const int cc = c0 + __ffsll((long long)cand) - 1;
            cand &= cand - 1;
            const double* tc = tau_all + (size_t)cc * L;
            bool same = true;
            for (int i = lane; i < L; i += 64) same = same && (tb[i] == tc[i]);
            if (__ballot(!same) == 0) rep = cc;
        }
    }
    if (lane == 0) erep[b] = rep;
}
void launch_tau_groups(hipStream_t s, const Grid& g, int B, const double* tau, unsigned long long* hash, int* erep,
                       const int* need_small, int* host_flag, int tag) {
    hipLaunchKernelGGL(k_tau_rep, dim3(B), dim3(64), 0, s, g.L, tau, hash, erep, need_small, host_flag, tag);
}

template <int MAXT>
static void launch_transport_t(hipStream_t s, dim3 grid, dim3 block, size_t shm, const TransportArgs& a, int mode) {
    if (mode == 1) {
        launch_transport_fast(s, grid, block, a);
    } else if (mode == 3) {
        launch_transport_ring(s, grid, a, g_ring_slots);
    } else if (mode == 4) {
        launch_transport_scan(s, grid, a);
    } else if (mode == 2) {
        if (a.accumulate) {
            if (a.saved) hipLaunchKernelGGL((k_transport<MAXT, true, true, true, true>), grid, block, shm, s, a);
            else hipLaunchKernelGGL((k_transport<MAXT, true, false, true, true>), grid, block, shm, s, a);
        } else {
            hipLaunchKernelGGL((k_transport<MAXT, false, false, true, true>), grid, block, shm, s, a);
        }
    } else if (a.accumulate) {
        if (a.Etab) {
            if (a.saved) hipLaunchKernelGGL((k_transport<MAXT, true, true, true>), grid, block, shm, s, a);
            else hipLaunchKernelGGL((k_transport<MAXT, true, false, true>), grid, block, shm, s, a);
        } else {
            if (a.saved) hipLaunchKernelGGL((k_transport<MAXT, true, true, false>), grid, block, shm, s, a);
            else hipLaunchKernelGGL((k_transport<MAXT, true, false, false>), grid, block, shm, s, a);
        }
    } else {
        if (a.Etab) hipLaunchKernelGGL((k_transport<MAXT, false, false, true>), grid, block, shm, s, a);
        else hipLaunchKernelGGL((k_transport<MAXT, false, false, false>), grid, block, shm, s, a);
    }
}

unsigned long long* g_transport_stamps = nullptr;
int g_ring_slots = 3, g_ring_debug = 0;

bool transport_fast_ok(const Plan& plan) {
    for (int bkt = 0; bkt < 4; ++bkt)
        if (plan.fix[bkt].idx > 0 && (plan.fix[bkt].s0 >> 6) != ((plan.N - 1) >> 6)) return false;
    return true;
}

void launch_transport(hipStream_t s, const Grid& g, int B, const double* tau, const double* Jn, double* In, double* I,
                      double* saved, size_t saved_col_stride, const ColDesc* desc, Conv cv, int order,
                      int accumulate, const double* Etab, int mode, const int* erep, int live, const int* live_list,
                      int ring_slots, int scan_split, double* scan_scratch, int* scan_sync, int nzcap) {
    const int nt = round64(g.N);
    const size_t shm = (size_t)(g.L + 2 * TC * (nt + 2) + 2 * nt + nt / 64 + 2) * sizeof(double);
    TransportArgs a{g, tau, Jn, In, I, accumulate ? saved : nullptr, saved_col_stride, desc, cv, order, accumulate, Etab, Etab ? erep : nullptr, g_transport_stamps};
    a.slots = ring_slots;
    a.nzcap = nzcap > kRingZones ? nzcap : kRingZones;
    if (mode == 4 && scan_split && scan_scratch && scan_sync) { a.scan_split = 1; a.scan_scratch = scan_scratch; a.scan_sync = scan_sync; }
    if ((mode == 3 || mode == 4) && accumulate && live > 0 && live < B && live_list) {
        a.live = live;
        a.live_list = live_list;
        B = live;
    }
    if (nt <= 128) launch_transport_t<128>(s, dim3(B), dim3(nt), shm, a, mode);
    else if (nt <= 256) launch_transport_t<256>(s, dim3(B), dim3(nt), shm, a, mode);
    else if (nt <= 512) launch_transport_t<512>(s, dim3(B), dim3(nt), shm, a, mode);
    else launch_transport_t<1024>(s, dim3(B), dim3(nt), shm, a, mode);
}

__global__ void k_finalize(int B, Conv cv, int max_orders, int* __restrict__ n_out, int* __restrict__ status_out) {
    const int b = blockIdx.x * blockDim.x + threadIdx.x;
    if (b >= B) return;
    int st = cv.status[b];
    if (cv.active[b]) { st = SOSRT_COL_MAXORDERS; cv.status[b] = st; }
    if (n_out) n_out[b] = cv.norders[b];
    if (status_out) status_out[b] = st;
}
void launch_finalize(hipStream_t s, int B, Conv cv, int max_orders, int* n_out, int* status_out) {
    hipLaunchKernelGGL(k_finalize, dim3((B + 127) / 128), dim3(128), 0, s, B, cv, max_orders, n_out, status_out);
}

__global__ void k_fluxes(Grid g, int B, const double* __restrict__ tau_all, const double* __restrict__ I_all,
                         const ColDesc* __restrict__ desc, int beam_norm, double* __restrict__ fdn,
                         double* __restrict__ fup) {
    const int row = blockIdx.x * (blockDim.x >> 6) + (threadIdx.x >> 6);
    if (row >= B * g.L) return;
    const int lane = threadIdx.x & 63, b = row / g.L, t = row % g.L;
    const double* I = I_all + (size_t)row * g.D;
    double sd = 0, su = 0;
    for (int k = lane; k < g.N; k += 64) {
        sd += g.wflux_dn[k] * I[k];
        su += g.wflux_up[k] * I[g.N + k];
    }
    sd = wave_sum(sd);
    su = wave_sum(su);
    if (lane == 0) {
        const ColDesc& d = desc[b];
        const double* tau = tau_all + (size_t)b * g.L;
        const double F0 = SOSRT_PI / d.mu0;
        const double fb = beam_norm ? F0 : F0 / (4 * SOSRT_PI);
        fdn[row] = sd - fb * exp(-tau[t] / d.mu0);
        fup[row] = su + fb * d.rho * exp(-(2 * tau[g.L - 1] - tau[t]) / d.mu0);
    }
}
void launch_fluxes(hipStream_t s, const Grid& g, int B, const double* tau, const double* I, const ColDesc* desc,
                   int beam_norm, double* fdn, double* fup) {
    const int rows = B * g.L;
    hipLaunchKernelGGL(k_fluxes, dim3((rows + 3) / 4), dim3(256), 0, s, g, B, tau, I, desc, beam_norm, fdn, fup);
}

__global__ void k_limit_rows(Grid g, int R, int table, const double* __restrict__ rows, double* __restrict__ out) {
    const FixTab& ft = g.fix[table];
    const int e = blockIdx.x * blockDim.x + threadIdx.x;
    if (e >= R * ft.idx) return;
    const int r = e / ft.idx, i = e % ft.idx;
    double acc = 0;
    for (int q = 0; q < ft.ns; ++q) acc += ft.C[i * ft.ns + q] * rows[(size_t)r * g.N + ft.s0 + q];
    out[e] = acc;
}
void launch_limit_rows(hipStream_t s, const Grid& g, int R, int table, const double* rows, double* out) {
    const int n = R * kFixMaxIdx;
    hipLaunchKernelGGL(k_limit_rows, dim3((n + 127) / 128), dim3(128), 0, s, g, R, table, rows, out);
}

__global__ void k_asymptotic(int R, int stride, const int* __restrict__ len, const double* __restrict__ J,
                             const double* __restrict__ tau, const double* __restrict__ tau_t,
                             const double* __restrict__ mu, double* __restrict__ out) {
    const int r = blockIdx.x * blockDim.x + threadIdx.x;
    if (r >= R) return;
    const int n = len[r];
    if (n <= 0) { out[r] = 0.0; return; }
    const double* Jr = J + (size_t)r * stride;
    const double* tr = tau + (size_t)r * stride;
    const double m = mu[r], tt = tau_t[r];
    const double Jl = Jr[n - 1];
    if (fabs(m) < kMuVerySmall) {
        double slope = 0;
        if (n > 1) slope = (Jl - Jr[n - 2]) / (tr[n - 1] - tr[n - 2]);
        out[r] = -Jl + m * slope;
        return;
// ... 73 lines not shown
```

sos-radiative-transfer_amd/csrc/kernels.hpp:

```cpp
#pragma once
#include <hip/hip_runtime.h>

#include "plan.hpp"

namespace sosrt {

constexpr int kMaxZones = 8;
constexpr int kRingZones = 3;

struct alignas(16) ColDesc {
    int nz;
    int r0[kMaxZones];
    int r1[kMaxZones];
    int mix[kMaxZones];
    int nfix[kMaxZones];
    int fixtab[kMaxZones];
    int surface;
    int geom;
    double mu0, rho, T, tau_bottom;
    double wa;
    double wr[kMaxZones];
    double fa[kMaxZones];
    double fr[kMaxZones];
    double ca[kMaxZones];
// ... 5 lines not shown
    double C[kFixMaxIdx * kFixMaxSrc];
};

struct ColScalars {
    const int* nz;
    const int* zr0;
    const int* zmix;
    const double* zwr;
    const double* zdtr;
    const int* idx_up;
    const int* idx_down;
    const double* mu0;
    const double* rho;
    const double* alb_atm;
    const double* alb_aer;
    const double* dtau_atm;
    const double* dtau_aer;
    const double* T;
};

struct Grid {
    int L, N, D;
    int Dp;
    int Wld;
    const double* mu;
    const double* Wa;
    const double* Wr;
    const FixTab* fix;
    const int* small_lanes;
    int nsmall;
    const double* wflux_dn;
    const double* wflux_up;
};

struct Conv {
    int* active;
    int* norders;
    int* status;
    int* nactive;
    double* ratio;
    int* redo;
    const int* target;
    double tol;
};

__device__ __forceinline__ bool conv_go(const Conv& cv, int b, int order, double r) {
    return cv.target ? order < cv.target[b] : r >= cv.tol;
}

constexpr int GEMM_BM = 64, GEMM_BN = 128, GEMM_KC = 16;
#ifndef SOSRT_GEMM_RT
#define SOSRT_GEMM_RT 4
#endif
#ifndef SOSRT_GEMM_WPS
#define SOSRT_GEMM_WPS 3
#endif
constexpr int GEMM_RT = SOSRT_GEMM_RT;
constexpr int GEMM_WPS = SOSRT_GEMM_WPS;

constexpr int TC = 8;

struct TransportArgs {
    Grid g;
    const double* tau;
    const double* Jn;
    double* In;
    double* I;
    double* saved;
    size_t saved_col_stride;
    const ColDesc* desc;
    Conv cv;
    int order;
    int accumulate;
    const double* Etab;
    const int* erep;
    unsigned long long* stamps;
    int live = 0;
    const int* live_list = nullptr;
    int slots = 0;
    int nzcap = kRingZones;
    int scan_split = 0;
    double* scan_scratch = nullptr;
    int* scan_sync = nullptr;
};
void launch_transport_fast(hipStream_t s, dim3 grid, dim3 block, const TransportArgs& a);
bool transport_ring_ok(const Grid& g);
bool transport_ring_fits(const Grid& g, int nzcap);
void launch_transport_ring(hipStream_t s, dim3 grid, const TransportArgs& a, int slots);
bool transport_scan_ok(const Grid& g);
bool transport_scan_split_ok(const Grid& g);
bool transport_scan_fits(const Grid& g, int nzcap, bool split);
int transport_scan_parts(const Grid& g);
size_t transport_scan_scratch_doubles();
void launch_transport_scan(hipStream_t s, dim3 grid, const TransportArgs& a);
constexpr int kOrderLoopMaxCols = 256;
constexpr int kOlArrive = 0, kOlState = 32, kOlLeft = 64, kOlAbort = 96, kOlOrders = 100, kOlCols = 128;
constexpr int kOlColStride = 64, kOlOrdDone = 0, kOlColStop = 1, kOlJnDone = 32;
constexpr int kOlReady = 1, kOlNotResident = 2, kOlAborted = 3;
inline size_t order_loop_sync_ints(int cols) { return (size_t)kOlCols + (size_t)cols * kOlColStride; }
extern int g_ring_slots, g_ring_debug;
extern unsigned long long* g_transport_stamps;

struct SolveSetup {
    int* zero_next = nullptr;
    int n_zero = 0;
    int* redo = nullptr;
    unsigned long long* hash = nullptr;
    int* scan_sync = nullptr;
};
void launch_prepare(hipStream_t s, const Grid& g, int B, int geom, int surface, ColScalars sc, const double* tau,
                    ColDesc* desc, double* rowcoef_a, double* rowcoef_r, int* need_small = nullptr, SolveSetup su = SolveSetup());
void launch_first_order_readme(hipStream_t s, const Grid& g, const double* w, int B, const double* tau, const double* P0a,
                               const double* P0r, const ColDesc* desc, double* I1_out, double* I_out, double* saved,
                               size_t saved_col_stride, Conv cv, int do_conv);
void launch_first_order(hipStream_t s, const Grid& g, int B, const double* tau, const double* P0a, const double* P0r,
                        const ColDesc* desc, double* I1_out, double* I_out, double* saved, size_t saved_col_stride,
                        Conv cv, int do_conv, int p0r_zones = 0 );
struct GemmArgs {
    const double* A;
    const double* Wa;
    const double* Wr;
    const double* ca;
    const double* cr;
    const int* rows_main;
    int n_main;
    const int* rows_slab;
    int n_slab;
    int D, Dp, Wld, L;
    double* C;
    const int* active;
    int B = 0;
    int col0 = 0;
    const int* idx_up = nullptr;
    const int* idx_down = nullptr;
    int max_main = 0, max_slab = 0;
    const double* Wmix = nullptr;
    const int* mix_group = nullptr;
    int pad_lds = 0;
    int* live_list = nullptr;
    int live_cap = 0;
    const int* slab_tile_group = nullptr;
    const int* nactive = nullptr;
    const int* need_small = nullptr;
    int* host_pub = nullptr;
    int tag = 0;
    int sym = 0;
    int Ks = 0;
    int check_tiles = 1;
    int lr_rank = -1;
    const double* lrU = nullptr;
    const double* lrV = nullptr;
};
constexpr int kLowRankMax = 4;

__device__ inline void publish_live_now(const GemmArgs& g) {
    const int live = __hip_atomic_load(g.nactive, __ATOMIC_RELAXED, __HIP_MEMORY_SCOPE_AGENT);
    int* slot = g.host_pub + 4 * (g.tag & 1);
    __hip_atomic_store(slot, live, __ATOMIC_RELAXED, __HIP_MEMORY_SCOPE_SYSTEM);
    __hip_atomic_store(slot + 2, g.need_small ? g.need_small[0] : 1, __ATOMIC_RELAXED, __HIP_MEMORY_SCOPE_SYSTEM);
    __hip_atomic_store(slot + 1, g.tag, __ATOMIC_RELEASE, __HIP_MEMORY_SCOPE_SYSTEM);
}
__device__ inline void publish_live(const GemmArgs& g) {
    if (g.host_pub && blockIdx.x == 0 && blockIdx.y == 0 && threadIdx.x == 0) publish_live_now(g);
}
struct PerDeviceOnce {
    bool seen[64] = {};
    bool first() {
        int d = 0;
        if (hipGetDevice(&d) != hipSuccess || d < 0 || d >= 64) return true;
        if (seen[d]) return false;
        seen[d] = true;
        return true;
    }
};
void launch_gemm(hipStream_t s, const GemmArgs& a);
struct OrderLoopArgs {
    TransportArgs t;
    GemmArgs gm;
    const double* in0;
    double* gbufP;
    double* gbufQ;
    double* bufP;
    double* bufQ;
    int order0;
    int kmax;
    int B, col0;
    int fixcap;
    int* sync;
    int* host_done;
    int tag;
    unsigned long long* log = nullptr;
    int astage = 0;
};
bool order_loop_ok(const Grid& g, bool split);
int order_loop_parts(const Grid& g, bool split);
hipError_t launch_order_loop(hipStream_t s, int grid, bool split, const OrderLoopArgs& p);
void launch_gemm_f32(hipStream_t s, const GemmArgs& a, const float* Wa32, const float* Wmix32);
void launch_to_float(hipStream_t s, size_t n, const double* src, float* dst);
void launch_wmix(hipStream_t s, size_t n, int ngroups, const double* Wa, const double* Wr, const double* ca, const double* cr,
                 double* Wmix, const int* gset = nullptr );
void launch_fold_sets(hipStream_t s, int S, int D, int Wld, size_t per, const double* w, const double* P, double* W);
void launch_fold_asymmetry(hipStream_t s, int S, int nblk, int D, int Wld, size_t per, const double* W, double* out);
void launch_symfold(hipStream_t s, int nmat, int N, int D, int Dp, int Wld, const double* W, double* SA);
void launch_gemm_tail(hipStream_t s, const GemmArgs& a, int cols, bool small_tiles, bool regs = false);
void launch_smallmu(hipStream_t s, const Grid& g, int B, const double* tau, const double* Jn, double* In,
                    const ColDesc* desc, const int* active);
void launch_transport(hipStream_t s, const Grid& g, int B, const double* tau, const double* Jn, double* In, double* I,
                      double* saved, size_t saved_col_stride, const ColDesc* desc, Conv cv, int order, int accumulate,
                      const double* Etab, int mode, const int* erep = nullptr, int live = 0, const int* live_list = nullptr,
                      int ring_slots = 0, int scan_split = 0, double* scan_scratch = nullptr, int* scan_sync = nullptr,
                      int nzcap = kRingZones);
bool transport_fast_ok(const Plan& plan);
void launch_attenuation(hipStream_t s, const Grid& g, int B, const double* tau, double* Etab, const int* erep);
void launch_tau_groups(hipStream_t s, const Grid& g, int B, const double* tau, unsigned long long* hash, int* erep,
                       const int* need_small = nullptr, int* host_flag = nullptr, int tag = 0);
void launch_fluxes(hipStream_t s, const Grid& g, int B, const double* tau, const double* I, const ColDesc* desc,
                   int beam_norm, double* fdn, double* fup);
struct EpilogueOut {
    double* flux_down;
    double* flux_up;
    double* diffusivity;
    double* heating_rate;
    double* net_toa;
};
void launch_epilogue(hipStream_t s, const Grid& g, const double* w, int B, const double* tau, const double* I,
                     const ColDesc* desc, int beam_norm, const double* z_profile, const EpilogueOut& out);
void launch_phase_p0(hipStream_t s, const Grid& g, const double* w, int B, int kind, double gpar, const double* tab_mu,
                     const double* tab_p, int ntab, const double* cosphi, const double* wphi, int nphi,
                     const double* mu0, double* P0);
void launch_phase_matrix(hipStream_t s, const Grid& g, const double* w, int kind, double gpar, const double* tab_mu,
                         const double* tab_p, int ntab, const double* cosphi, const double* wphi, int nphi, double* P);
constexpr int kMaxModes = 64;
void launch_phase_modes(hipStream_t s, const Grid& g, const double* w, int kind, double gpar, const double* tab_mu,
                        const double* tab_p, int ntab, const double* cosphi, const double* tab, int nphi, int m_first,
                        int m_count, double* P_out);
void launch_phase_p0_modes(hipStream_t s, const Grid& g, const double* w, int B, int kind, double gpar, const double* tab_mu,
                           const double* tab_p, int ntab, const double* cosphi, const double* tab, int nphi, int m_first,
                           int m_count, const double* mu0, double* P0_out);
void launch_azimuth_accumulate(hipStream_t s, const Grid& g, int B, int m, const double* Im, int nlev, const int* levels,
                               int nphi_out, const double* phi, double* out);
constexpr int kMieQ = 6;
constexpr int kMieChunk = 4;
inline int mie_chunks(int R) { return (R + kMieChunk - 1) / kMieChunk; }
void launch_mie_coefficients(hipStream_t s, int nlanes, int R, int n_cap, const double* x, const int* nmax, const int* nstart,
                             const double* m_re, const double* m_im, const double* radii, const double* r_m, const double* sig,
                             double* ab, double* qw);
void launch_mie_angles(hipStream_t s, int S, int R, int ntab, int n_cap, const double* mu, const double* ab, const int* nmax,
                       const double* tn, const double* qw, double* part);
void launch_mie_integrate(hipStream_t s, int S, int R, int ntab, const double* part, const double* radii, const double* qw,
                          double* p, double* bulk);
void launch_limit_rows(hipStream_t s, const Grid& g, int R, int table, const double* rows, double* out);
void launch_asymptotic(hipStream_t s, int R, int stride, const int* len, const double* J, const double* tau,
                       const double* tau_t, const double* mu, double* out);
void launch_finalize(hipStream_t s, int B, Conv cv, int max_orders, int* n_out = nullptr, int* status_out = nullptr);
void launch_bench(hipStream_t s, int which, double* a, double* b, size_t n, int iters);

}
```

sos-radiative-transfer_amd/csrc/transport_ring.hip:

```cpp
#include <type_traits>

#include "../../include/sosrt.h"
#include "kernels.hpp"
#include "transport_util.hpp"

namespace sosrt {

namespace {

#ifndef SOSRT_RING_STORE_AUX
#define SOSRT_RING_STORE_AUX 0
#endif
__device__ __forceinline__ void rstore(__amdgpu_buffer_rsrc_t r, int voff, int soff, double x) { bstore_aux<SOSRT_RING_STORE_AUX>(r, voff, soff, x); }

typedef __attribute__((address_space(3))) void* lds_ptr_t;

constexpr size_t kRingLdsBytes = 152 * 1024;

template <int CNT>
__device__ __forceinline__ void wait_vm() {
    asm volatile("s_waitcnt vmcnt(%0)" ::"n"(CNT) : "memory");
}
__device__ __forceinline__ void wg_barrier() {
    asm volatile("s_waitcnt lgkmcnt(0)\n\ts_barrier" ::: "memory");
}

template <bool ACC, bool SAVED, int PIECES, bool MZ>
__global__ __launch_bounds__(512) void k_transport_ring(TransportArgs a, int NS, int dbg_arg, int fixcap) {
    constexpr int NWL = 2;
#ifdef SOSRT_RING_DEBUG
    const int dbg = dbg_arg;
#else
    constexpr int dbg = 0;
    (void)dbg_arg;
#endif
    int b = blockIdx.x;
    if (ACC && a.live > 0) {
        b = a.live_list[blockIdx.x];
        if (b < 0) return;
    } else if (ACC && !a.cv.active[b]) {
        return;
    }
    const Grid& g = a.g;
    const int tid = threadIdx.x, lane = tid & 63;
    const int wid = __builtin_amdgcn_readfirstlane(tid) >> 6;
    const int L = g.L, N = g.N, D = g.D;
    const int nwc = (N + 63) >> 6;
    const bool loader = wid >= nwc;
    const int lid = wid - nwc;
    const bool w0 = wid == 0 && !(dbg & 8);
    const bool wl = wid == ((N - 1) >> 6) && !(dbg & 4);
    auto stamp = [&](int i) {
        if (a.stamps && (tid == 0 || tid == 64)) a.stamps[((size_t)b * 2 + (tid >> 6)) * 8 + i] = clock64();
    };
    stamp(0);
    constexpr int NARR = ACC ? 3 : 2;
    constexpr int RS = 128 * PIECES;
    constexpr int SLOT = NARR * TC * RS;
    constexpr int IPC = NARR * TC * PIECES;
    extern __shared__ double sm[];
    double* ring = sm;
    double* s_sfc = ring + (size_t)NS * SLOT;
    double* s_fixc = s_sfc;
    double* s_red = s_sfc + max(RS, (MZ ? a.nzcap : kRingZones) * fixcap * kFixMaxSrc);
    double* s_hd = s_red + (blockDim.x >> 6) + 2;
    double* s_S = s_hd + L + 1;
    double* s_x = s_S + (size_t)g.nsmall * L;
    double* s_prmu = s_x + TC * 16;
    int* s_nf = reinterpret_cast<int*>(s_prmu + 16);
    const int xb_dn = max(((N - 1) & 63) - 15, 0);
    __shared__ int s_flag[3];
    const ColDesc* __restrict__ dg = a.desc + b;
    const int nz = dg->nz;
    const ZoneRows<MZ> zr(dg);
    const int nfix0 = dg->nfix[0], nfix1 = dg->nfix[1], nfix2 = dg->nfix[2];
    const int surface = dg->surface;
    const double rho = dg->rho;
    const int fbytes = L * D * 8, RB = D * 8;
    const int lbytes = (dbg & 1) ? 0 : fbytes, sbytes = (dbg & 2) ? 0 : fbytes;
    const __amdgpu_buffer_rsrc_t rJ = make_rsrc(a.Jn + (size_t)b * L * D, lbytes);
    const __amdgpu_buffer_rsrc_t rE = make_rsrc(a.Etab + (size_t)(a.erep ? a.erep[b] : b) * L * D, lbytes);
    const __amdgpu_buffer_rsrc_t rIn = make_rsrc(a.In + (size_t)b * L * D, sbytes);
    const __amdgpu_buffer_rsrc_t rIl = make_rsrc(ACC ? a.I + (size_t)b * L * D : a.In, ACC ? lbytes : 0);
    const __amdgpu_buffer_rsrc_t rI = make_rsrc(ACC ? a.I + (size_t)b * L * D : a.In, ACC ? sbytes : 0);
    const __amdgpu_buffer_rsrc_t rS = make_rsrc(SAVED ? a.saved + (size_t)b * a.saved_col_stride : a.In, SAVED ? sbytes : 0);
    const int NCH = (L + TC - 1) / TC, NQ = 2 * NCH, R = NS - 1;
    const bool valid = tid < N;
    const int tidc = valid ? tid : N - 1;
    unsigned long long sp_dn = NCH > 64 ? ~0ull : 1ull << (NCH - 1), sp_up = sp_dn;
    if (NCH <= 64) {
        sp_dn |= zr.boundary_chunks(L, TC, false);
        sp_up |= zr.boundary_chunks(L, TC, true);
    }
    auto plain_run = [&](unsigned long long mask, int j) {
        const unsigned long long rest = NCH > 64 ? 1ull : mask >> j;
        return rest ? __builtin_ctzll(rest) : 0;
    };
    double rdn_v = 0, rdn_i = 1, rup_v = 0, rup_i = 1;
    double sfc_own = 0;
    int slot_rd = 0;

    int slot_ld = 0;
    auto issue = [&](int q) {
        const bool up = q >= NCH;
        const int j = up ? q - NCH : q;
        double* dst = ring + (size_t)slot_ld * SLOT;
        slot_ld = slot_ld + 1 == NS ? 0 : slot_ld + 1;
        const int half = up ? N * 8 : 0;
        const int vo = lane * 16;
#pragma unroll
        for (int i = 0; i < TC / NWL; ++i) {
            const int u = i * NWL + lid;
            const int row = up ? max(L - 1 - j * TC - u, 0) : min(j * TC + u, L - 1);
#pragma unroll
            for (int p = 0; p < PIECES; ++p) {
                const int so = row * RB + half + p * 1024;
                __builtin_amdgcn_raw_ptr_buffer_load_lds(rJ, (lds_ptr_t)(dst + (0 * TC + u) * RS + p * 128), 16, vo, so, 0, 0);
                __builtin_amdgcn_raw_ptr_buffer_load_lds(rE, (lds_ptr_t)(dst + (1 * TC + u) * RS + p * 128), 16, vo, so, 0, 0);
                if (ACC) __builtin_amdgcn_raw_ptr_buffer_load_lds(rIl, (lds_ptr_t)(dst + (2 * TC + u) * RS + p * 128), 16, vo, so, 0, 0);
            }
        }
    };
    auto loader_phase = [&](auto keep_t, int qa, int qb) {
        constexpr int KEEP = decltype(keep_t)::value;
        for (int q = qa; q < qb; ++q) {
            if (q + R < NQ) {
                issue(q + R);
                wait_vm<KEEP>();
            } else {
                wait_vm<0>();
            }
            wg_barrier();
        }
    };
    const int ncomp = nwc * 64;
    if (loader) {
        for (int q = 0; q < min(R, NQ); ++q) issue(q);
    } else {
        for (int zz = 0; zz < (MZ ? nz : kRingZones); ++zz) {
            const FixTab& src = g.fix[dg->fixtab[zz]];
            for (int i = tid; i < fixcap * kFixMaxSrc; i += ncomp) s_fixc[zz * fixcap * kFixMaxSrc + i] = src.C[i];
        }
        if (tid < 3) s_flag[tid] = 0;
        for (int i = tid; i < (L + 31) / 32; i += ncomp) s_nf[i] = 0;
        const double* __restrict__ tau = a.tau + (size_t)b * L;
        for (int t = tid; t <= L; t += ncomp) s_hd[t] = (t == 0 || t == L) ? 0.0 : (tau[t] - tau[t - 1]) * 0.5;
        if (tid < 16) s_prmu[tid] = (tid > 0 && tid < N) ? 1.0 / g.mu[N + tid] : 0.0;
        const double* __restrict__ In0 = a.In + (size_t)b * L * D;
        for (int i = tid; i < g.nsmall * L; i += ncomp) {
            const int k = i / L, t = i - k * L;
            s_S[i] = In0[(size_t)t * D + g.small_lanes[k]];
        }
    }
    __syncthreads();

    const int seam_barriers = surface == SOSRT_SURFACE_NONE ? 0 : (surface == SOSRT_SURFACE_SPECULAR ? 1 : 3);
    double Bv = 0;
    if (loader) {
        constexpr int PER = IPC / NWL;
        auto run = [&](auto keep_t) {
            loader_phase(keep_t, 0, NCH);
            for (int i = 0; i < seam_barriers; ++i) wg_barrier();
            loader_phase(keep_t, NCH, NQ);
            wait_vm<0>();
        };
        if (R <= 1) run(std::integral_constant<int, 0>{});
        else if (R == 2) run(std::integral_constant<int, (PER < 60 ? PER : 60)>{});
        else if (R == 3) run(std::integral_constant<int, (2 * PER < 60 ? 2 * PER : 60)>{});
        else run(std::integral_constant<int, (3 * PER < 60 ? 3 * PER : 60)>{});
    } else {
    stamp(1);
    const double mu_up = (valid && tid > 0) ? g.mu[N + tidc] : 1.0;
    const int uT = lane >> 3, pT = lane & 7;
    const double muT = (pT + 1 < N) ? g.mu[N + pT + 1] : 1.0;
    const double* xrow = s_x + uT * 16;
    {
        const int m = tidc;
        const int vo = m * 8;
        const double mu = g.mu[m];
        const bool tr = valid && m <= N - 2;
        const bool small = tr && fabs(mu) < kMuThreshold;
        const bool stdl = tr && !small;
        const double nrmu = stdl ? -1.0 / mu : 0.0;
        const bool has_small = wl && g.nsmall > 0;
        double Dv = 0, Jprev = 0;
        double c[kFixMaxSrc] = {0, 0, 0, 0, 0};
        double cT[kFixMaxSrc] = {0, 0, 0, 0, 0};
        int sl[kFixMaxSrc] = {0, 0, 0, 0, 0};
        int nfx = 0;
        bool fixlane = false;
        auto load_fix = [&](int zz) {
            const double* ftC = s_fixc + zz * fixcap * kFixMaxSrc;
            nfx = zz == 0 ? nfix0 : (zz == 1 ? nfix1 : ((!MZ || zz == 2) ? nfix2 : zr.nfix(zz)));
            const int ns = nfx < 2 ? 2 : (nfx < kFixMaxSrc ? nfx : kFixMaxSrc);
            fixlane = valid && nfx > 0 && m >= N - nfx;
            const int i = fixlane ? N - 1 - m : 0;
            const int s0 = nfx < 2 ? N - nfx - 2 : N - nfx - ns;
#pragma unroll
            for (int q = 0; q < kFixMaxSrc; ++q) {
                c[q] = (fixlane && q < ns) ? ftC[i * ns + min(q, ns - 1)] : 0.0;
                cT[q] = (pT < nfx && q < ns) ? ftC[pT * ns + min(q, ns - 1)] : 0.0;
                sl[q] = (s0 + min(q, ns - 1)) & 63;
            }
        };
        if (wl) load_fix(0);
        const int sbase = small ? (m - g.small_lanes[0]) * L : 0;
        int t0 = 0, q = 0;
        auto process = [&](auto special_t, auto mode_t, const double* slot, double (&Jc)[TC], double (&Ic)[TC], double (&Ec)[TC]) __attribute__((always_inline)) {
            constexpr bool SP = decltype(special_t)::value;
            constexpr int MODE = decltype(mode_t)::value;
            double cc[TC], v[TC], Sc[TC];
#pragma unroll
            for (int u = 0; u < TC; ++u) Sc[u] = 0;
            if ((SP || MODE == 2) && has_small) {
#pragma unroll
                for (int u = 0; u < TC; ++u) {
                    const double sv = s_S[sbase + min(t0 + u, L - 1)];
                    Sc[u] = small ? sv : 0.0;
                }
            }
#pragma unroll
            for (int u = 0; u < TC; ++u) {
                const int t = SP ? min(t0 + u, L - 1) : t0 + u;
                const double hk = s_hd[t];
                const double Jp = u == 0 ? Jprev : Jc[u - 1];
                cc[u] = rec_src(rec_hr(hk, nrmu), Jp, Ec[u], Jc[u]);
            }
            if (!SP) {
                {
                    double d = 0, p = 1, dl[TC], pl[TC];
#pragma unroll
                    for (int u = 0; u < TC; ++u) {
                        d = rec_step(d, Ec[u], cc[u]);
                        p = u == 0 ? Ec[0] : rec_hr(p, Ec[u]);
                        dl[u] = d; pl[u] = p;
                    }
#pragma unroll
                    for (int u = 0; u < TC; ++u) v[u] = rec_step(Dv, pl[u], dl[u]);
                    Dv = v[TC - 1];
                }
                if (MODE == 2 && has_small) {
#pragma unroll
                    for (int u = 0; u < TC; ++u) v[u] = rec_add(v[u], Sc[u]);
                }
                const bool tfix = MODE == 1 || (MODE == 2 && wl && nfx > 0 && nfx <= 8 && sl[0] >= xb_dn);
                if (tfix) {
#pragma unroll
                    for (int u = 0; u < TC; ++u)
                        if (lane >= xb_dn && lane < xb_dn + 16) s_x[u * 16 + lane - xb_dn] = v[u];
                    double acc = 0;
#pragma unroll
                    for (int k = 0; k < kFixMaxSrc; ++k) acc = fix_acc(cT[k], xrow[max(sl[k] - xb_dn, 0)], acc);
                    const int mT = N - 1 - pT;
                    const double IcT = ACC ? slot[(2 * TC + uT) * RS + max(mT, 0)] : 0.0;
                    if (pT < nfx) {
                        const int voT = (t0 + uT) * RB + mT * 8;
                        rstore(rIn, voT, 0, acc);
                        if (ACC) rstore(rI, voT, 0, IcT + acc);
                        if (SAVED) rstore(rS, voT, 0, acc);
                    }
                } else if (MODE == 2 && wl && nfx > 0) {
#pragma unroll
                    for (int u = 0; u < TC; ++u) {
                        double acc = 0;
#pragma unroll
                        for (int k = 0; k < kFixMaxSrc; ++k) acc = fix_acc(c[k], readlane_f64(v[u], sl[k]), acc);
                        v[u] = fixlane ? acc : v[u];
                    }
                }
                if (valid && !(tfix && fixlane)) {
#pragma unroll
                    for (int u = 0; u < TC; ++u) {
                        const int so = (t0 + u) * RB;
                        rstore(rIn, vo, so, v[u]);
                        if (ACC) rstore(rI, vo, so, Ic[u] + v[u]);
                        if (SAVED) rstore(rS, vo, so, v[u]);
                    }
                }
            } else {
#pragma unroll
                for (int u = 0; u < TC; ++u) {
                    const int t = t0 + u;
                    if (wl) { const int zs = zr.starts(t); if (zs) load_fix(zs); }
                    const double Dn = rec_step(Dv, Ec[u], cc[u]);
                    double x = has_small ? rec_add(Dn, Sc[u]) : Dn;
                    if (wl && nfx > 0) {
                        double acc = 0;
#pragma unroll
                        for (int k = 0; k < kFixMaxSrc; ++k) acc = fix_acc(c[k], readlane_f64(x, sl[k]), acc);
                        x = fixlane ? acc : x;
                    }
                    v[u] = x;
                    const bool zone_end = zr.ends(t);
                    Dv = t < L ? (zone_end ? (stdl ? x : 0.0) : Dn) : Dv;
                    if (valid && t < L) {
                        const int so = t * RB;
                        rstore(rIn, vo, so, x);
                        if (ACC) rstore(rI, vo, so, Ic[u] + x);
                        if (SAVED) rstore(rS, vo, so, x);
                    }
                }
            }
            if (SP && t0 + TC >= L) {
#pragma unroll
                for (int u = 0; u < TC; ++u)
                    if (t0 + u == L - 1) { sfc_own = v[u]; rdn_v = v[u]; rdn_i = Ic[u] + v[u]; }
            }
            Jprev = Jc[TC - 1];
            t0 += TC;
        };
        auto chunk = [&](auto special_t, auto mode_t) __attribute__((always_inline)) {
            const double* sp = ring + (size_t)slot_rd * SLOT + tid;
            slot_rd = slot_rd + 1 == NS ? 0 : slot_rd + 1;
            double Jc[TC], Ic[TC], Ec[TC];
#pragma unroll
            for (int u = 0; u < TC; ++u) {
                Jc[u] = sp[(0 * TC + u) * RS];
                Ec[u] = sp[(1 * TC + u) * RS];
                Ic[u] = ACC ? sp[(2 * TC + u) * RS] : 0.0;
            }
            process(special_t, mode_t, sp - tid, Jc, Ic, Ec);
            wg_barrier();
        };
        using M0 = std::integral_constant<int, 0>;
        using M1 = std::integral_constant<int, 1>;
        using M2 = std::integral_constant<int, 2>;
        while (q < NCH) {
            const int qe = q + plain_run(sp_dn, q);
            const int mode = (!wl || (nfx == 0 && !has_small)) ? 0 : ((!has_small && nfx <= 8 && sl[0] >= xb_dn) ? 1 : 2);
            if (mode == 0) for (; q < qe; ++q) chunk(std::false_type{}, M0{});
            else if (mode == 1) for (; q < qe; ++q) chunk(std::false_type{}, M1{});
            else for (; q < qe; ++q) chunk(std::false_type{}, M2{});
            if (q < NCH) { chunk(std::true_type{}, M2{}); ++q; }
        }
    }

    stamp(2);
    if (surface != SOSRT_SURFACE_NONE) {
        if (valid) s_sfc[tid] = sfc_own;
        wg_barrier();
    }
    if (surface == SOSRT_SURFACE_SPECULAR) {
        Bv = valid ? rho * s_sfc[N - 1 - tid] : 0.0;
    } else if (surface == SOSRT_SURFACE_LAMBERTIAN || surface == SOSRT_SURFACE_LAMBERTIAN_README) {
        double term = 0;
        if (tid <= N - 3) {
            const int k0 = N - 2 - tid, k1 = k0 - 1;
            const double x0 = g.mu[k0], x1 = g.mu[k1];
            term = (x1 - x0) * (s_sfc[k1] * x1 + s_sfc[k0] * x0) / 2;
        }
        double ws = wave_sum_(term);
        wg_barrier();
        if (lane == 0) s_red[tid >> 6] = ws;
        wg_barrier();
        double S = 0;
        for (int i = 0; i < nwc; ++i) S += s_red[i];
        Bv = (surface == SOSRT_SURFACE_LAMBERTIAN_README ? 2 : -2) * rho * S;
    }

    stamp(3);
    {
        const int mj = N + tidc;
        const int vo = mj * 8;
        const bool tr = valid && tid > 0;
        const double mu = mu_up;
        const double prmu = tr ? 1.0 / mu : 0.0;
        const int last_cand = min(N - 3, 61);
        bool notfound = false;
        double U = Bv, Jnext = 0;
        auto blend = [&](double x, int t) {
            const double x1 = lane_up1(x), x2 = lane_up1(x1);
            const bool stop = lane >= 1 && lane <= last_cand && !(fabs((x - x1) - (x1 - x2)) > 0.0001);
            const unsigned long long mk = __ballot(stop);
            const int kf = mk ? __ffsll((long long)mk) : 1;
            if (mk == 0) {
                notfound = true;
                if (N - 3 > 61 && lane == 0) {
                    if (zr.starts(t)) s_flag[0] = 1;
                    else { flag_row(s_nf, t); s_flag[2] = 1; }
                }
            }
            const double r0 = readlane_f64(x, 0), rk = readlane_f64(x, kf);
            const double w = blend_weight(mu, readlane_f64(prmu, kf));
            const double bl = blend_val(w, r0, rk);
            return (tr && tid < kf) ? bl : x;
        };
        int t0 = L - 1, q = NCH;
        auto process = [&](auto special_t, auto mode_t, const double* slot, double (&Jc)[TC], double (&Ic)[TC], double (&Ec)[TC]) __attribute__((always_inline)) {
            constexpr bool SP = decltype(special_t)::value;
            constexpr int MODE = decltype(mode_t)::value;
            double cc[TC], v[TC];
#pragma unroll
            for (int u = 0; u < TC; ++u) {
                const int t = SP ? max(t0 - u, 0) : t0 - u;
                const double hk = s_hd[t + 1];
                const double Jx = u == 0 ? Jnext : Jc[u - 1];
                const double src = rec_src(rec_hr(hk, prmu), Jx, Ec[u], Jc[u]);
                cc[u] = (SP && zr.ends(t)) ? 0.0 : src;
            }
            if (!SP) {
                {
                    double d = 0, p = 1, dl[TC], pl[TC];
// ... 3 lines not shown
                        p = u == 0 ? Ec[0] : rec_hr(p, Ec[u]);
                        dl[u] = d; pl[u] = p;
                    }
#pragma unroll
                    for (int u = 0; u < TC; ++u) v[u] = rec_step(U, pl[u], dl[u]);
                    U = v[TC - 1];
                }
                bool tblend = false;
                if (MODE == 1) {
#pragma unroll
                    for (int u = 0; u < TC; ++u) {
                        v[u] = tid == 0 ? Jc[u] : v[u];
                        if (lane < 16) s_x[u * 16 + lane] = v[u];
                    }
                    const int k = pT + 1;
                    const double xa = xrow[k], xb = xrow[k + 1], xc = xrow[k + 2];
                    const bool stop = (k <= last_cand) & !(fabs((xa - xb) - (xb - xc)) > 0.0001);
                    const unsigned long long mk = __ballot(stop);
                    const unsigned bits = (unsigned)(mk >> (8 * uT)) & 0xffu;
                    tblend = __ballot(bits != 0) == ~0ull;
                    if (tblend) {
                        const int kf = __ffs((int)bits) + 1;
                        const double r0 = xrow[0], rk = xrow[kf];
                        const double w = blend_weight(muT, s_prmu[kf]);
                        const double bl = blend_val(w, r0, rk);
                        const double val = k < kf ? bl : xa;
                        const double IcT = ACC ? slot[(2 * TC + uT) * RS + k] : 0.0;
                        if (k < N) {
                            const int voT = (t0 - uT) * RB + (N + k) * 8;
                            rstore(rIn, voT, 0, val);
                            if (ACC) rstore(rI, voT, 0, IcT + val);
                            if (SAVED) rstore(rS, voT, 0, val);
                        }
                    } else {
#pragma unroll
                        for (int u = 0; u < TC; ++u) {
                            const double xb_ = blend(v[u], t0 - u);
                            if (valid) {
                                const int so = (t0 - u) * RB;
                                rstore(rIn, vo, so, xb_);
                                if (ACC) rstore(rI, vo, so, Ic[u] + xb_);
                                if (SAVED) rstore(rS, vo, so, xb_);
                            }
                        }
                    }
                }
                if (valid && (MODE == 0 || (tblend && !(tid >= 1 && tid <= 8)))) {
#pragma unroll
                    for (int u = 0; u < TC; ++u) {
                        const int so = (t0 - u) * RB;
                        rstore(rIn, vo, so, v[u]);
                        if (ACC) rstore(rI, vo, so, Ic[u] + v[u]);
                        if (SAVED) rstore(rS, vo, so, v[u]);
                    }
                }
            } else {
#pragma unroll
                for (int u = 0; u < TC; ++u) {
                    const int t = t0 - u;
                    const double Un = rec_step(U, Ec[u], cc[u]);
                    double x = Un;
                    if (w0 && t >= 0) x = blend(tid == 0 ? Jc[u] : Un, t);
                    v[u] = x;
                    const bool zone_start = zr.starts(t) != 0;
                    U = t >= 0 ? ((zone_start && tr) ? x : Un) : U;
                    if (valid && t >= 0) {
                        const int so = t * RB;
                        rstore(rIn, vo, so, x);
                        if (ACC) rstore(rI, vo, so, Ic[u] + x);
                        if (SAVED) rstore(rS, vo, so, x);
                    }
                }
            }
            if (SP && t0 - TC < 0) {
#pragma unroll
                for (int u = 0; u < TC; ++u)
                    if (t0 - u == 0) { rup_v = v[u]; rup_i = Ic[u] + v[u]; }
            }
            Jnext = Jc[TC - 1];
            t0 -= TC;
        };
        auto chunk = [&](auto special_t, auto mode_t) __attribute__((always_inline)) {
            const double* sp = ring + (size_t)slot_rd * SLOT + tid;
            slot_rd = slot_rd + 1 == NS ? 0 : slot_rd + 1;
            double Jc[TC], Ic[TC], Ec[TC];
#pragma unroll
            for (int u = 0; u < TC; ++u) {
                Jc[u] = sp[(0 * TC + u) * RS];
                Ec[u] = sp[(1 * TC + u) * RS];
                Ic[u] = ACC ? sp[(2 * TC + u) * RS] : 0.0;
            }
            process(special_t, mode_t, sp - tid, Jc, Ic, Ec);
            wg_barrier();
        };
        using M0 = std::integral_constant<int, 0>;
        using M1 = std::integral_constant<int, 1>;
        while (q < NQ) {
            const int qe = q + plain_run(sp_up, q - NCH);
            if (!w0) for (; q < qe; ++q) chunk(std::false_type{}, M0{});
            else for (; q < qe; ++q) chunk(std::false_type{}, M1{});
            if (q < NQ) { chunk(std::true_type{}, M1{}); ++q; }
        }
        if (w0 && notfound && lane == 0 && N - 3 <= 61) s_flag[1] = 1;
    }
    }
    stamp(4);
    __syncthreads();
    stamp(5);
    if (s_flag[1]) {
        if (tid == 0) {
            a.cv.status[b] = SOSRT_COL_INDEXERROR;
            if (ACC) { a.cv.active[b] = 0; a.cv.norders[b] = a.order; atomicSub(a.cv.nactive, 1); }
        }
        return;
    }
    if (!s_flag[0] && s_flag[2]) {
        if (finish_flagged_rows<ACC, SAVED>(s_nf, L, N, RB, g.mu, rIn, rI, rS, ring, rup_v, rup_i)) {
            if (tid == 0) {
                a.cv.status[b] = SOSRT_COL_INDEXERROR;
                if (ACC) { a.cv.active[b] = 0; a.cv.norders[b] = a.order; atomicSub(a.cv.nactive, 1); }
            }
            return;
        }
    }
    if (s_flag[0]) {
        const bool missing = redo_upward_sweep<ACC, SAVED, MZ>(L, N, RB, zr, s_hd, g.mu, rJ, rE, rIn, rI, rS, Bv, ring,
                                                            rup_v, rup_i);
        if (missing) {
            if (tid == 0) {
                a.cv.status[b] = SOSRT_COL_INDEXERROR;
                if (ACC) { a.cv.active[b] = 0; a.cv.norders[b] = a.order; atomicSub(a.cv.nactive, 1); }
            }
            return;
        }
    }
    if (ACC) {
        const double ra = block_pymax_(rup_v / rup_i, valid, s_red, 0);
        const double rb = block_pymax_(rdn_v / rdn_i, valid, s_red, 0);
        const double r = (rb > ra) ? rb : ra;
        if (tid == 0) {
            a.cv.ratio[b] = r;
            a.cv.norders[b] = a.order;
            if (!conv_go(a.cv, b, a.order, r)) {
                a.cv.active[b] = 0;
                atomicSub(a.cv.nactive, 1);
            }
        }
    } else if (tid == 0 && a.cv.status) {
        a.cv.status[b] = SOSRT_COL_OK;
    }
}

inline int ring_fixcap(const Grid& g) { return (int)(0.06 * g.N) + 1; }
inline size_t ring_extra_doubles(const Grid& g, int nt, int nzcap = kRingZones) {
    const int rs = g.N <= 128 ? 128 : 256, fc = nzcap * ring_fixcap(g) * kFixMaxSrc;
    return (size_t)(rs > fc ? rs : fc) + nt / 64 + 2 + g.L + 1 + (size_t)g.nsmall * g.L + TC * 16 + 16 + (g.L + 63) / 64;
}

template <int PIECES>
void launch_p(hipStream_t s, dim3 grid, dim3 block, const TransportArgs& a, int NS) {
    const int nt = (int)block.x;
    const int narr = a.accumulate ? 3 : 2;
    const size_t shm = ((size_t)NS * narr * TC * 128 * PIECES + ring_extra_doubles(a.g, nt, a.nzcap)) * sizeof(double);
#define SOSRT_RING_LAUNCH_Z(ACC_, SAVED_, MZ_)                                                                 \
    do {                                                                                                       \
        auto kern = k_transport_ring<ACC_, SAVED_, PIECES, MZ_>;                                               \
        static PerDeviceOnce big_lds;                                                                                 \
        if (big_lds.first()) {                                                                                        \
            hipFuncSetAttribute(reinterpret_cast<const void*>(kern), hipFuncAttributeMaxDynamicSharedMemorySize, \
                                (int)kRingLdsBytes);                                                                   \
        }                                                                                                      \
        hipLaunchKernelGGL(kern, grid, block, shm, s, a, NS, g_ring_debug, ring_fixcap(a.g));                           \
    } while (0)
#define SOSRT_RING_LAUNCH(ACC_, SAVED_)                                                                        \
    do {                                                                                                       \
        if (a.nzcap > kRingZones) SOSRT_RING_LAUNCH_Z(ACC_, SAVED_, true);                                     \
        else SOSRT_RING_LAUNCH_Z(ACC_, SAVED_, false);                                                         \
    } while (0)
    if (a.accumulate) {
        if (a.saved) SOSRT_RING_LAUNCH(true, true);
        else SOSRT_RING_LAUNCH(true, false);
    } else {
        SOSRT_RING_LAUNCH(false, false);
    }
#undef SOSRT_RING_LAUNCH
#undef SOSRT_RING_LAUNCH_Z
}

}

bool transport_ring_ok(const Grid& g) {
    if (g.N % 2 || g.N < 4 || g.N > 256) return false;
    const int nwc = (g.N + 63) / 64, pieces = g.N <= 128 ? 1 : 2;
    const size_t slot_bytes = (size_t)3 * TC * 128 * pieces * sizeof(double);
    if (flagged_rows_work_doubles(g.L, g.N) * sizeof(double) > 2 * slot_bytes * 2 / 3) return false;
    return 2 * slot_bytes + ring_extra_doubles(g, (nwc + 4) * 64) * sizeof(double) <= kRingLdsBytes;
}

bool transport_ring_fits(const Grid& g, int nzcap) {
    if (!transport_ring_ok(g)) return false;
    const int nwc = (g.N + 63) / 64, pieces = g.N <= 128 ? 1 : 2;
    const size_t slot_bytes = (size_t)3 * TC * 128 * pieces * sizeof(double);
    return 2 * slot_bytes + ring_extra_doubles(g, (nwc + 4) * 64, nzcap < kRingZones ? kRingZones : nzcap) * sizeof(double) <= kRingLdsBytes;
}

void launch_transport_ring(hipStream_t s, dim3 grid, const TransportArgs& a, int slots) {
    if (a.slots > 0) slots = a.slots;
    const int N = a.g.N;
    const int nwc = (N + 63) / 64;
    const int pieces = N <= 128 ? 1 : 2;
    const int narr = a.accumulate ? 3 : 2;
    const dim3 block((nwc + 2) * 64);
    const size_t slot_bytes = (size_t)narr * TC * 128 * pieces * sizeof(double);
    const size_t extra = ring_extra_doubles(a.g, (int)block.x, a.nzcap) * sizeof(double);
    int NS = slots < 2 ? 2 : slots;
    while (NS > 2 && NS * slot_bytes + extra > kRingLdsBytes) --NS;
    if (pieces == 1) launch_p<1>(s, grid, block, a, NS);
    else launch_p<2>(s, grid, block, a, NS);
}

}
```

sos-radiative-transfer_amd/csrc/transport_util.hpp:

```cpp
#pragma once
#include <hip/hip_runtime.h>

#include "kernels.hpp"

namespace sosrt {
namespace {

__device__ __forceinline__ double readlane_f64(double v, int srclane) {
    int lo = __double2loint(v), hi = __double2hiint(v);
    lo = __builtin_amdgcn_readlane(lo, srclane);
    hi = __builtin_amdgcn_readlane(hi, srclane);
    return __hiloint2double(hi, lo);
}

typedef unsigned int u32x2 __attribute__((ext_vector_type(2)));

__device__ __forceinline__ __amdgpu_buffer_rsrc_t make_rsrc(const void* p, int bytes) {
    return __builtin_amdgcn_make_buffer_rsrc(const_cast<void*>(p), 0, bytes, 0x00020000);
}
__device__ __forceinline__ double bload(__amdgpu_buffer_rsrc_t r, int voff, int soff) {
    const u32x2 v = __builtin_amdgcn_raw_buffer_load_b64(r, voff, soff, 0);
    return __hiloint2double((int)v.y, (int)v.x);
}
__device__ __forceinline__ double bload_glc(__amdgpu_buffer_rsrc_t r, int voff, int soff) {
// ... 155 lines not shown
                m |= 1ull << ((up ? L - 1 - rb : rb) / tc);
                m |= 1ull << ((up ? L - 1 - re : re) / tc);
            }
        }
        return m;
    }
};

constexpr int kNfBatch = 8;
__host__ __device__ inline size_t flagged_rows_work_doubles(int L, int N) { return (size_t)kNfBatch * (N + 2) + (L + kNfBatch + 2 + 1) / 2 + 1; }
__device__ __forceinline__ void flag_row(int* s_nf, int t) { atomicOr(&s_nf[t >> 5], 1 << (t & 31)); }
#ifdef SOSRT_HELPERS_AS_CALLS
#define SOSRT_HELPER_INLINE __attribute__((noinline))
#else
#define SOSRT_HELPER_INLINE __forceinline__
#endif
template <bool ACC, bool SAVED, int LDX = 0, int STX = 0>
__device__ SOSRT_HELPER_INLINE bool finish_flagged_rows(const int* s_nf, int L, int N, int RB, const double* __restrict__ gmu, __amdgpu_buffer_rsrc_t rIn,
                                    __amdgpu_buffer_rsrc_t rI, __amdgpu_buffer_rsrc_t rS, double* s_work, double& rup_v, double& rup_i) {
    const int tid = threadIdx.x, NP = N + 2;
    double* s_rows = s_work;
    int* s_list = reinterpret_cast<int*>(s_work + kNfBatch * NP);
    int* s_kf = s_list + L;
    int* s_cnt = s_kf + kNfBatch;
    if (tid == 0) {
        int c = 0;
        for (int t = L - 1; t >= 0; --t)
            if ((s_nf[t >> 5] >> (t & 31)) & 1) s_list[c++] = t;
        *s_cnt = c;
    }
    __syncthreads();
    const int cnt = *s_cnt;
    const bool act = tid < N, tr = act && tid > 0;
    const int j = act ? tid : 0;
    const double mu = tr ? gmu[N + j] : 1.0;
    const int vo = (N + j) * 8;
    bool missing = false;
    for (int c0 = 0; c0 < cnt; c0 += kNfBatch) {
        const int nb = min(kNfBatch, cnt - c0);
        double xo[kNfBatch], Io[kNfBatch];
#pragma unroll
        for (int i = 0; i < kNfBatch; ++i) {
            const int t = s_list[c0 + min(i, nb - 1)];
            xo[i] = bload_aux<LDX ? LDX : 1>(rIn, vo, t * RB);
            Io[i] = ACC ? bload_aux<LDX ? LDX : 1>(rI, vo, t * RB) : 0.0;
        }
#pragma unroll
        for (int i = 0; i < kNfBatch; ++i)
            if (act) s_rows[i * NP + j] = xo[i];
        if (tid < kNfBatch) s_kf[tid] = 1 << 30;
        __syncthreads();
#pragma unroll
        for (int i = 0; i < kNfBatch; ++i) {
            const double* r = s_rows + i * NP;
            if (i < nb && act && j >= 1 && j <= N - 3 && !(fabs((r[j] - r[j + 1]) - (r[j + 1] - r[j + 2])) > 0.0001)) atomicMin(&s_kf[i], j);
        }
        __syncthreads();
#pragma unroll
        for (int i = 0; i < kNfBatch; ++i) {
            if (i >= nb) continue;
            const double* r = s_rows + i * NP;
            const int ks = s_kf[i];
            missing |= ks == (1 << 30);
            const int kf = ks == (1 << 30) ? 1 : ks + 1;
            const int t = s_list[c0 + i];
            if (tr && tid < kf) {
                const double x = blend_val(blend_weight(mu, 1.0 / gmu[N + kf]), r[0], r[kf]);
                bstore_aux<STX>(rIn, vo, t * RB, x);
                double It = 0;
                if (ACC) {
                    It = Io[i] + (x - xo[i]);
                    bstore_aux<STX>(rI, vo, t * RB, It);
                }
                if (SAVED) bstore_aux<STX>(rS, vo, t * RB, x);
                if (t == 0) { rup_v = x; rup_i = It; }
            }
        }
        __syncthreads();
    }
    return missing;
}

constexpr int kRedoRows = 8;
template <bool ACC, bool SAVED, bool MZ, int LDX = 0, int STX = 0>
__device__ SOSRT_HELPER_INLINE bool redo_upward_sweep(int L, int N, int RB, const ZoneRows<MZ>& zr, const double* s_hd,
                                  const double* __restrict__ gmu, __amdgpu_buffer_rsrc_t rJ, __amdgpu_buffer_rsrc_t rE,
                                  __amdgpu_buffer_rsrc_t rIn, __amdgpu_buffer_rsrc_t rI, __amdgpu_buffer_rsrc_t rS, double U0,
                                  double* s_work, double& rup_v, double& rup_i) {
    const int tid = threadIdx.x;
    double* s_row = s_work;
    int* s_kf = reinterpret_cast<int*>(s_work + 2 * (N + 2));
    const bool act = tid < N, tr = act && tid > 0;
    const int j = act ? tid : 0;
    const double mu = tr ? gmu[N + j] : 1.0;
    const double prmu = tr ? 1.0 / mu : 0.0;
    const int vo = (N + j) * 8;
    double U = U0, Jnext = 0;
    bool missing = false;
    if (tid < 2) s_kf[tid] = 1 << 30;
    __syncthreads();
    int par = 0;
    for (int t0 = L - 1; t0 >= 0; t0 -= kRedoRows) {
        double Jc[kRedoRows], Ec[kRedoRows], xo[kRedoRows], Io[kRedoRows];
#pragma unroll
        for (int u = 0; u < kRedoRows; ++u) {
            const int t = max(t0 - u, 0);
            Jc[u] = bload_aux<LDX>(rJ, vo, t * RB);
            Ec[u] = bload(rE, vo, t * RB);
            xo[u] = bload_aux<LDX ? LDX : 1>(rIn, vo, t * RB);
            Io[u] = ACC ? bload_aux<LDX ? LDX : 1>(rI, vo, t * RB) : 0.0;
        }
#pragma unroll
        for (int u = 0; u < kRedoRows; ++u) {
            const int t = t0 - u;
            if (t < 0) break;
            double* row = s_row + par * (N + 2);
            const double src = rec_src(rec_hr(s_hd[t + 1], prmu), Jnext, Ec[u], Jc[u]);
            const double Un = rec_step(U, Ec[u], zr.ends(t) ? 0.0 : src);
            if (act) row[j] = tid == 0 ? Jc[u] : Un;
            __syncthreads();
            if (act && j >= 1 && j <= N - 3 && !(fabs((row[j] - row[j + 1]) - (row[j + 1] - row[j + 2])) > 0.0001)) atomicMin(&s_kf[par], j);
            if (tid == 0) s_kf[par ^ 1] = 1 << 30;
            __syncthreads();
            const int ks = s_kf[par];
            missing |= ks == (1 << 30);
            const int kf = ks == (1 << 30) ? 1 : ks + 1;
            double x = act ? row[j] : 0.0;
            if (tr && tid < kf) x = blend_val(blend_weight(mu, 1.0 / gmu[N + kf]), row[0], row[kf]);
            const bool zone_start = zr.starts(t) != 0;
            U = (zone_start && tr) ? x : Un;
            Jnext = Jc[u];
            if (act) {
                bstore_aux<STX>(rIn, vo, t * RB, x);
                double It = 0;
                if (ACC) {
                    It = Io[u] + (x - xo[u]);
                    bstore_aux<STX>(rI, vo, t * RB, It);
                }
                if (SAVED) bstore_aux<STX>(rS, vo, t * RB, x);
                if (t == 0) { rup_v = x; rup_i = It; }
            }
            par ^= 1;
        }
    }
    __syncthreads();
    return missing;
}

__device__ __forceinline__ double block_pymax_(double x, bool valid, double* s_red, int first_tid) {
    const int tid = threadIdx.x, nw = blockDim.x >> 6;
    double v = wave_fmax_(valid ? x : __builtin_nan(""));
    __syncthreads();
    if ((tid & 63) == 0) s_red[tid >> 6] = v;
    if (tid == first_tid) s_red[nw] = x;
    __syncthreads();
    double r = s_red[0];
    for (int i = 1; i < nw; ++i) r = fmax(r, s_red[i]);
    const double first = s_red[nw];
    return (first != first) ? first : r;
}

}
}
```

sos-radiative-transfer_amd/sosrt/_lib.py:

```python
import ctypes
import os
from ctypes import POINTER, c_char_p, c_double, c_int, c_longlong, c_void_p

_HERE = os.path.dirname(os.path.abspath(__file__))
LIB_PATH = os.environ.get("SOSRT_LIB") or os.path.join(os.path.dirname(_HERE), "libsosrt.so")

SOSRT_OK, E_INVALID, E_HIP, E_STATE, E_NOMEM = 0, -1, -2, -3, -4
COL_OK, COL_INDEXERROR, COL_MAXORDERS, COL_INTERNAL = 0, 1, 2, 3
GEOM_THREE_ZONE, GEOM_SINGLE_SLAB = 0, 1
SURFACE_NONE, SURFACE_SPECULAR, SURFACE_LAMBERTIAN, SURFACE_LAMBERTIAN_README = 0, 1, 2, 3
K_GEMM, K_TRANSPORT, K_FIRST, K_SMALLMU, K_ORDER_LOOP = 0, 1, 2, 3, 4
PLAN_GEMM_DENSE, PLAN_GEMM_LIVE64, PLAN_GEMM_LIVE32, PLAN_GEMM_LIVE32_DEEP, PLAN_GEMM_LIVE16_REGS = 0, 1, 2, 3, 4
PLAN_TRANSPORT_GENERAL, PLAN_TRANSPORT_FAST, PLAN_TRANSPORT_RING, PLAN_TRANSPORT_SCAN = 0, 1, 3, 4
CONTRACT_F64, CONTRACT_F32, CONTRACT_F64_FULL, CONTRACT_F64_DENSE = 0, 1, 2, 3
FIRST_ORDER_CODED, FIRST_ORDER_README = 0, 1
PHASE_ISO, PHASE_RAYLEIGH, PHASE_HG, PHASE_TABLE = 0, 1, 2, 3
MAX_MODES = 64
MAX_PHASE_SETS = 64

_dp = POINTER(c_double)
_ip = POINTER(c_int)

SIGNATURES = {
    "sosrt_last_error": (c_char_p, []),
    "sosrt_version": (c_int, []),
    "sosrt_create": (c_int, [c_int, c_int, c_int, c_int, c_int, POINTER(c_void_p)]),
    "sosrt_destroy": (c_int, [c_void_p]),
    "sosrt_set_stream": (c_int, [c_void_p, c_void_p]),
    "sosrt_use_own_stream": (c_int, [c_void_p]),
    "sosrt_synchronize": (c_int, [c_void_p]),
    "sosrt_set_saved_orders": (c_int, [c_void_p, c_int]),
    "sosrt_set_order_budget": (c_int, [c_void_p, c_int]),
    "sosrt_set_contraction": (c_int, [c_void_p, c_int]),
    "sosrt_phase_asymmetry": (c_int, [c_void_p, POINTER(c_double), _ip]),
    "sosrt_phase_rank": (c_int, [c_void_p, _ip, POINTER(c_double), _ip]),
    "sosrt_set_order_loop": (c_int, [c_void_p, c_int]),
    "sosrt_order_loop_stats": (c_int, [c_void_p, _ip, _ip, POINTER(c_longlong)]),
    "sosrt_plan_launch": (c_int, [c_void_p, c_int, c_int, c_int, c_int, c_int, _ip]),
    "sosrt_set_first_order": (c_int, [c_void_p, c_int]),
    "sosrt_set_grid": (c_int, [c_void_p, c_void_p]),
    "sosrt_set_phase": (c_int, [c_void_p, c_void_p, c_void_p]),
    "sosrt_set_phase_sets": (c_int, [c_void_p, c_void_p, c_int, c_void_p]),
    "sosrt_set_phase_sets_dev": (c_int, [c_void_p, c_void_p, c_int, c_void_p]),
    "sosrt_phase_matrix_dev": (c_int, [c_void_p, c_int, c_double, c_void_p]),
    "sosrt_set_aerosol_sets": (c_int, [c_void_p, c_int, c_int, c_void_p]),
    "sosrt_phase_sets_info": (c_int, [c_void_p, _ip]),
    "sosrt_set_columns": (c_int, [c_void_p, c_int, c_int, c_int] + [c_void_p] * 9),
    "sosrt_set_columns_zones": (c_int, [c_void_p, c_int, c_int, c_int] + [c_void_p] * 10),
    "sosrt_first_order": (c_int, [c_void_p, c_int, c_void_p, c_void_p, c_void_p, c_void_p]),
    "sosrt_source": (c_int, [c_void_p, c_int, c_void_p, c_void_p]),
    "sosrt_transport": (c_int, [c_void_p, c_int, c_void_p, c_void_p, c_void_p, c_void_p]),
    "sosrt_solve": (c_int, [c_void_p, c_int, c_void_p, c_void_p, c_void_p, c_double, c_void_p, c_void_p, c_void_p, c_void_p, c_void_p]),
    "sosrt_solve_dev": (c_int, [c_void_p, c_int, c_void_p, c_void_p, c_void_p, c_double, c_void_p, c_void_p, c_void_p, c_void_p, c_void_p]),
    "sosrt_last_solve_stats": (c_int, [c_void_p, _ip, POINTER(c_longlong)]),
    "sosrt_fluxes": (c_int, [c_void_p, c_int, c_void_p, c_void_p, c_int, c_void_p, c_void_p]),
    "sosrt_epilogue_dev": (c_int, [c_void_p, c_int, c_void_p, c_void_p, c_int] + [c_void_p] * 6),
    "sosrt_epilogue": (c_int, [c_void_p, c_int, c_int] + [c_void_p] * 6),
    "sosrt_phase_table": (c_int, [c_void_p, c_void_p, c_void_p, c_int]),
    "sosrt_phase_table_dev": (c_int, [c_void_p, c_void_p, c_void_p, c_int]),
    "sosrt_mie_ensembles": (c_int, [c_void_p, c_int] + [c_void_p] * 5 + [c_int, c_double, c_double, c_int, c_void_p, c_void_p]),
    "sosrt_mie_ensembles_dev": (c_int, [c_void_p, c_int] + [c_void_p] * 5 + [c_int, c_double, c_double, c_int, c_void_p, c_void_p]),
    "sosrt_mie_efficiencies": (c_int, [c_void_p, c_int, c_void_p, c_void_p, c_void_p, c_void_p]),
    "sosrt_mie_timing": (c_int, [c_void_p, _dp]),
    "sosrt_phase_p0_dev": (c_int, [c_void_p, c_int, c_int, c_double, c_void_p, c_void_p]),
    "sosrt_phase_p0": (c_int, [c_void_p, c_int, c_int, c_double, c_void_p, c_void_p]),
    "sosrt_phase_matrix": (c_int, [c_void_p, c_int, c_double, c_void_p]),
    "sosrt_phase_modes": (c_int, [c_void_p, c_int, c_double, c_int, c_int, c_int, c_void_p]),
    "sosrt_phase_p0_modes_dev": (c_int, [c_void_p, c_int, c_int, c_double, c_int, c_int, c_int, c_void_p, c_void_p]),
    "sosrt_phase_p0_modes": (c_int, [c_void_p, c_int, c_int, c_double, c_int, c_int, c_int, c_void_p, c_void_p]),
    "sosrt_set_order_targets": (c_int, [c_void_p, c_void_p]),
    "sosrt_azimuth_accumulate_dev": (c_int, [c_void_p, c_int, c_int, c_void_p, c_int, c_void_p, c_int, c_void_p, c_void_p]),
    "sosrt_comm_unique_id": (c_int, [c_void_p]),
    "sosrt_comm_init": (c_int, [c_void_p, c_int, c_int, c_void_p]),
    "sosrt_gather": (c_int, [c_void_p, c_int, c_void_p, c_void_p, c_void_p]),
    "sosrt_comm_destroy": (c_int, [c_void_p]),
    "sosrt_limit_mu_down": (c_int, [c_void_p, c_int, c_int, c_void_p, c_void_p]),
    "sosrt_asymptotic_down": (c_int, [c_void_p, c_int, c_int, c_void_p, c_void_p, c_void_p, c_void_p, c_void_p, c_void_p]),
    "sosrt_plan_weights": (c_int, [c_void_p, c_void_p]),
    "sosrt_plan_fold": (c_int, [c_void_p, c_int, c_void_p]),
    "sosrt_plan_fix_table": (c_int, [c_void_p, c_int, _ip, _ip, c_void_p]),
    "sosrt_plan_fix_count": (c_int, [c_double, c_int]),
    "sosrt_debug_stamps": (c_int, [c_void_p, c_void_p]),
    "sosrt_microbench": (c_int, [c_void_p, c_int, _dp]),
    "sosrt_profile_enable": (c_int, [c_void_p, c_int]),
    "sosrt_profile_reset": (c_int, [c_void_p]),
    "sosrt_profile_get": (c_int, [c_void_p, c_int, _dp, POINTER(c_longlong), _dp]),
}

_lib = None


def _preload_hip_runtime():
    import importlib.util
    try:
        spec = importlib.util.find_spec("torch")
    except (ImportError, ValueError):
        spec = None
    if spec is None or not spec.submodule_search_locations:
        return
    p = os.path.join(list(spec.submodule_search_locations)[0], "lib", "libamdhip64.so")
    if os.path.exists(p):
        try:
            ctypes.CDLL(p, mode=ctypes.RTLD_GLOBAL)
        except OSError:
            pass


def lib():
    global _lib
    if _lib is None:
        if not os.path.exists(LIB_PATH):
            raise ImportError(
                "libsosrt.so not found at %s: build it with `python __graft_entry__.py build` "
                "(hipcc --offload-arch=gfx950); there is no CPU fallback" % LIB_PATH)
        _preload_hip_runtime()
        L = ctypes.CDLL(LIB_PATH)
# ... 22 lines not shown
```

sos-radiative-transfer_amd/sosrt/solver.py:

```python
from __future__ import annotations

import ctypes
from dataclasses import dataclass
from typing import Optional

import numpy as np

from . import _lib
from ._lib import check, lib


def _f64(a, shape=None, name="array"):
    a = np.ascontiguousarray(a, dtype=np.float64)
    if shape is not None and a.shape != tuple(shape):
        raise ValueError("%s has shape %s, expected %s" % (name, a.shape, tuple(shape)))
    return a


def _i32(a, n, name):
    a = np.ascontiguousarray(a, dtype=np.int32)
    if a.shape != (n,):
        raise ValueError("%s has shape %s, expected (%d,)" % (name, a.shape, n))
    return a


def _ptr(a):
    return None if a is None else a.ctypes.data_as(ctypes.c_void_p)


def _vec(x, B, name):
    a = np.ascontiguousarray(np.broadcast_to(np.asarray(x, dtype=np.float64), (B,)))
    return a


@dataclass
class DevicePhaseSets:
    address: int
    S: int
    keep: object = None


@dataclass
class SolveResult:
    I: np.ndarray
    n: np.ndarray
    status: np.ndarray
    I_saved: Optional[np.ndarray]


class Solver:

    def __init__(self, nb_layers: int, nb_angles: int, max_batch: int = 1, max_orders: int = 64, device: int = 0):
        self.L, self.N, self.D = int(nb_layers), int(nb_angles), 2 * int(nb_angles)
        self.max_batch, self.max_orders, self.device = int(max_batch), int(max_orders), int(device)
        self._h = ctypes.c_void_p()
        check(lib().sosrt_create(self.device, self.L, self.N, self.max_batch, self.max_orders, ctypes.byref(self._h)))
        self.B = 0
        self.order_budget = self.max_orders
        self.mu = None
        self._P = (None, None)
        self._p0_zones = 0

    def close(self):
        if getattr(self, "_h", None) is not None and self._h.value:
            lib().sosrt_destroy(self._h)
            self._h = ctypes.c_void_p()

    def __del__(self):
        try:
            self.close()
        except Exception:
            pass

    def set_stream(self, stream_handle: Optional[int]):
        if stream_handle is None:
            check(lib().sosrt_use_own_stream(self._h))
        else:
            check(lib().sosrt_set_stream(self._h, ctypes.c_void_p(stream_handle) if stream_handle else None))

    def synchronize(self):
        check(lib().sosrt_synchronize(self._h))

    def set_contraction(self, mode="f64"):
        m = {"f64": _lib.CONTRACT_F64, "f32": _lib.CONTRACT_F32, "f64_full": _lib.CONTRACT_F64_FULL,
             "f64_dense": _lib.CONTRACT_F64_DENSE}.get(mode)
        if m is None:
            raise ValueError("contraction must be 'f64', 'f64_dense', 'f64_full' or 'f32'")
        check(lib().sosrt_set_contraction(self._h, m))

    def set_order_budget(self, max_orders: int):
        check(lib().sosrt_set_order_budget(self._h, int(max_orders)))
        self.order_budget = int(max_orders)

    def set_order_loop(self, on=True):
        check(lib().sosrt_set_order_loop(self._h, int(on) if on in (0, 1, 2) else (1 if on else 0)))

    def order_loop_stats(self, column_orders=False):
        a, b, c = ctypes.c_int(), ctypes.c_int(), ctypes.c_longlong()
        check(lib().sosrt_order_loop_stats(self._h, ctypes.byref(a), ctypes.byref(b), ctypes.byref(c) if column_orders else None))
        return (a.value, b.value, c.value) if column_orders else (a.value, b.value)

    def phase_asymmetry(self):
        a, u = ctypes.c_double(), ctypes.c_int()
        check(lib().sosrt_phase_asymmetry(self._h, ctypes.byref(a), ctypes.byref(u)))
        return a.value, bool(u.value)

    def phase_rank(self):
        r, a, u = ctypes.c_int(), ctypes.c_double(), ctypes.c_int()
        check(lib().sosrt_phase_rank(self._h, ctypes.byref(r), ctypes.byref(a), ctypes.byref(u)))
        return r.value, a.value, bool(u.value)

    def set_first_order(self, mode="coded"):
        m = {"coded": _lib.FIRST_ORDER_CODED, "readme": _lib.FIRST_ORDER_README}.get(mode)
        if m is None:
            raise ValueError("first_order must be 'coded' or 'readme'")
        check(lib().sosrt_set_first_order(self._h, m))

    def set_grid(self, mu):
        mu = _f64(mu, (self.D,), "mu")
        check(lib().sosrt_set_grid(self._h, _ptr(mu)))
        self.mu = mu.copy()
        self._P = (None, None)

    def set_phase(self, P_atm, P_aer=None):
        Pa = _f64(P_atm, (self.D, self.D), "P_atm")
        Pr = None if P_aer is None else _f64(P_aer, (self.D, self.D), "P_aer")
        check(lib().sosrt_set_phase(self._h, _ptr(Pa), _ptr(Pr)))
        self._P = (Pa.copy(), None if Pr is None else Pr.copy())

    def set_phase_sets(self, P_atm, P_aer_sets):
        Pa = _f64(P_atm, (self.D, self.D), "P_atm")
        Pr = np.ascontiguousarray(P_aer_sets, dtype=np.float64)
        if Pr.ndim != 3 or Pr.shape[1:] != (self.D, self.D):
            raise ValueError("P_aer_sets has shape %s, expected (S, %d, %d)" % (Pr.shape, self.D, self.D))
        check(lib().sosrt_set_phase_sets(self._h, _ptr(Pa), int(Pr.shape[0]), _ptr(Pr)))
        self._P = (Pa.copy(), Pr.copy())

    def set_phase_sets_device(self, P_atm, d_P_aer: int, S: int):
        Pa = _f64(P_atm, (self.D, self.D), "P_atm")
        check(lib().sosrt_set_phase_sets_dev(self._h, _ptr(Pa), int(S), ctypes.c_void_p(d_P_aer) if d_P_aer else None))
        self._P = (None, None)

    def set_aerosol_sets(self, sets):
        z = np.ascontiguousarray(sets, dtype=np.int32)
        if z.ndim == 1:
            z = z.reshape(-1, 1)
        if z.ndim != 2 or z.shape[0] != self.B:
            raise ValueError("sets has shape %s, expected (%d,) or (%d, nzmax)" % (np.shape(sets), self.B, self.B))
        check(lib().sosrt_set_aerosol_sets(self._h, int(z.shape[0]), int(z.shape[1]), _ptr(z)))
        self._p0_zones = int(z.shape[1]) if z.shape[1] > 1 else 0

    def phase_sets_info(self):
        out = (ctypes.c_int * 4)()
        check(lib().sosrt_phase_sets_info(self._h, out))
        return {"sets": out[0], "groups": out[1], "single_pass": bool(out[2]), "group_cap": out[3]}

    def same_grid(self, mu):
        return self.mu is not None and np.array_equal(self.mu, np.asarray(mu, dtype=np.float64))

    def same_phase(self, P_atm, P_aer=None):
        a, r = self._P
        if a is None or not np.array_equal(a, P_atm):
            return False
        if (r is None) != (P_aer is None):
            return False
        return r is None or (np.shape(r) == np.shape(P_aer) and np.array_equal(r, P_aer))

    def set_columns(self, idx_up, idx_down, mu0, grd_alb, alb_atm, alb_aer, dtau_atm, dtau_aer, tauStar_tot,
                    surface="specular"):
        B = int(np.size(idx_up))
        sf = {"specular": _lib.SURFACE_SPECULAR, "lambertian": _lib.SURFACE_LAMBERTIAN,
# ... 307 lines not shown
```

Measured before the change: 117,700.

## Store low-rank source moments and expand J inside ring transport

When the phase matrix is low-rank, the source GEMM now writes only a few per-row moments (the projections onto U plus the single-scattering coefficient) for rows in plain chunks, instead of materialising the full J row. The ring transport kernel rebuilds J on the fly from these moments and V, including in the redo upward sweep. This aims to cut the global write and read traffic of the full Jn array between source and transport. In exchange it adds a moments buffer, extra LDS, a reworked butterfly reduction in the low-rank kernel, and a new kernel template variant. It is enabled by default (expand=1) when the plan selects the dense GEMM and ring transport.

```diff
diff --git a/include/sosrt.h b/include/sosrt.h
--- a/include/sosrt.h
+++ b/include/sosrt.h
@@ -155,6 +155,9 @@
 #define SOSRT_PLAN_TRANSPORT_SCAN    4
 int sosrt_plan_launch(sosrt_t* h, int batch, int live, int surface, int zones, int cus, int* out );
 
+int sosrt_set_expand(sosrt_t* h, int mode);
+int sosrt_expand_stats(sosrt_t* h, int* planned, int* launches);
+
 #define SOSRT_K_GEMM      0
 #define SOSRT_K_TRANSPORT 1
 #define SOSRT_K_FIRST     2
diff --git a/sos-radiative-transfer_amd/csrc/api.hip b/sos-radiative-transfer_amd/csrc/api.hip
--- a/sos-radiative-transfer_amd/csrc/api.hip
+++ b/sos-radiative-transfer_amd/csrc/api.hip
@@ -138,6 +138,10 @@
     int lr_rank = -1;
     double lr_residual = 0;
     double *d_lrU = nullptr, *d_lrV = nullptr;
+    double* d_moments = nullptr;
+    int expand = 1;
+    int expanded_launches = 0;
+    int plan_expand = 0;
     size_t mixs_capacity = 0;
     float *d_Wa32 = nullptr, *d_Wmix32 = nullptr;
     size_t mix32_capacity = 0;
@@ -422,7 +426,7 @@
 }
 
 void run_source(sosrt_handle* h, const double* In_1, double* Jn, const int* active, int tail_cols = 0, int pub_tag = 0,
-                int grp = -1, bool all_live = false, bool regs_tile = false, int dense_live_cap = 0) {
+                int grp = -1, bool all_live = false, bool regs_tile = false, int dense_live_cap = 0, bool expand = false) {
     const int g0 = grp < 0 ? 0 : grp, g1 = grp < 0 ? h->ngroups : grp + 1;
     const int pg = grp < 0 ? 0 : grp;
     hipStream_t s = group_stream(h, pg);
@@ -457,6 +461,11 @@
         ga.Wr = h->d_Wrsets; ga.mix_group = h->d_mixgroup; ga.slab_tile_group = h->d_slabtilegroup + h->slab_off[g0] / 32;
     }
     if (use_lowrank(h)) { ga.lr_rank = h->lr_rank; ga.lrU = h->d_lrU; ga.lrV = h->d_lrV; }
+    if (expand && use_lowrank(h) && tail_cols == 0) {
+        const size_t c0 = h->nslab > 0 ? 0 : (size_t)h->gb[g0];
+        ga.moments = h->d_moments + c0 * h->L * kMomentRec;
+        ga.desc = h->d_desc + c0;
+    }
     if (use_sym(h)) {
         ga.sym = 1; ga.Ks = (h->g.N + GEMM_KC - 1) / GEMM_KC * GEMM_KC;
 #ifdef SOSRT_DIAG
@@ -530,11 +539,15 @@
     int order_loop = 0;
     int ol_parts = 0;
     int ol_grid = 0;
+    int expand = 0;
 };
 LaunchPlan plan_order(const sosrt_handle* h, const SolveShape& sh, const OrderInputs& in) {
     LaunchPlan pl;
     const Grid& g = h->g;
-    const bool live_tiling = h->contraction != SOSRT_CONTRACT_F32 && in.simple_zones && in.known <= h->gemm_tail_cols &&
+    const bool expand_ok = h->expand && use_lowrank(h) && g.N % 64 == 0 && g.L % TC == 0 && g.L / TC <= 64 && h->contraction != SOSRT_CONTRACT_F32 &&
+                           !in.need_small && !in.saving;
+    const bool force_expand = h->expand == 2 && expand_ok && sh.fast && sh.ring_mode == 3;
+    const bool live_tiling = !force_expand && h->contraction != SOSRT_CONTRACT_F32 && in.simple_zones && in.known <= h->gemm_tail_cols &&
                              (in.known <= h->gemm_tail_frac * in.nb || in.nb <= h->gemm_small_cols) &&
                              (in.known < in.nb || in.nb <= h->gemm_small_cols);
     pl.tail_cols = live_tiling ? in.known : 0;
@@ -556,12 +569,13 @@
                                (in.surface == SOSRT_SURFACE_SPECULAR || in.surface == SOSRT_SURFACE_NONE);
         const bool want_scan = h->transport_mode == 4 || (h->transport_mode == 3 && cols_now <= h->scan_cols);
         const bool split = can_split && transport_scan_fits(g, sh.nzcap, true) && (sh.fast || (h->use_etab && h->transport_mode >= 3));
-        const bool scan = want_scan && ((sh.fast && sh.ring_mode == 3 && h->scan_ok && transport_scan_fits(g, sh.nzcap, false)) || split);
+        const bool scan = !force_expand && want_scan && ((sh.fast && sh.ring_mode == 3 && h->scan_ok && transport_scan_fits(g, sh.nzcap, false)) || split);
         pl.transport = scan ? SOSRT_PLAN_TRANSPORT_SCAN
                             : (!sh.fast ? SOSRT_PLAN_TRANSPORT_GENERAL : (sh.ring_mode == 3 ? SOSRT_PLAN_TRANSPORT_RING : SOSRT_PLAN_TRANSPORT_FAST));
         if (scan && split) pl.parts = transport_scan_parts(g);
         pl.repair = (h->N - 3 > 61 && pl.transport == SOSRT_PLAN_TRANSPORT_FAST) ? 1 : 0;
     }
+    pl.expand = (expand_ok && pl.transport == SOSRT_PLAN_TRANSPORT_RING && pl.gemm == SOSRT_PLAN_GEMM_DENSE) ? 1 : 0;
     if (h->order_loop && in.cu_share > 0 && h->transport_mode == 3 && sh.fast && sh.ring_mode == 3 && sh.nzcap <= kRingZones &&
         use_sym(h) && in.simple_zones && in.slabs_mixed && !in.saving && !in.need_small && in.orders_left >= 1 &&
         in.known <= kOrderLoopMaxCols) {
@@ -649,6 +663,7 @@
     if (const char* ev = getenv("SOSRT_GEMM_KS_MULT")) h->diag_ks_mult = atoi(ev);
 #endif
     if (const char* ev = getenv("SOSRT_GROUP_RING_SLOTS")) h->coresident_slots = atoi(ev);
+    if (const char* ev = getenv("SOSRT_EXPAND")) { const int v = atoi(ev); h->expand = v < 0 ? 0 : (v > 2 ? 2 : v); }
     if (const char* ev = getenv("SOSRT_ORDER_LOOP")) h->order_loop = atoi(ev) != 0;
     if (const char* ev = getenv("SOSRT_RING_SLOTS")) g_ring_slots = atoi(ev);
 #ifdef SOSRT_RING_DEBUG
@@ -672,6 +687,7 @@
             if ((e = dalloc(&h->d_Wr, (size_t)g.Dp * g.Wld))) return e;
             if ((e = dalloc(&h->d_lrU, (size_t)kLowRankMax * g.D))) return e;
             if ((e = dalloc(&h->d_lrV, (size_t)kLowRankMax * g.D))) return e;
+            if ((e = dalloc(&h->d_moments, (size_t)max_batch * L * kMomentRec))) return e;
             if ((e = dalloc(&h->d_wfdn, N))) return e;
             if ((e = dalloc(&h->d_wfup, N))) return e;
             if ((e = dalloc(&h->d_w, g.D))) return e;
@@ -751,7 +767,7 @@
                         h->d_idx_down, h->d_scal, h->d_desc, h->d_rca, h->d_rcr, h->d_slabrows, h->d_mainrows, h->d_tau, h->d_P0a,
                         h->d_P0r, h->d_Jn, h->d_InA, h->d_InB, h->d_I, h->d_E, h->d_active, h->d_norders, h->d_status,
                         h->d_nactive_sets, h->d_ratio, h->d_redo, h->d_erep, h->d_tauhash, h->d_Wmix, h->d_mixca, h->d_mixcr,
-                        h->d_mixgroup, h->d_Wa_s, h->d_Wr_s, h->d_Wmix_s, h->d_scan_scratch, h->d_scan_sync, h->d_w, h->d_phi, h->d_z, h->d_tab, h->d_slabtilegroup, h->d_livelist, h->d_Wa32, h->d_Wmix32, h->d_nz, h->d_zr0, h->d_zmix, h->d_zwr, h->d_zdtr, h->d_olsync, h->d_ollog, h->d_modetab, h->d_lrU, h->d_lrV, h->d_Wrsets, h->d_Wrsets_s, h->d_mixset, h->d_P0rz};
+                        h->d_mixgroup, h->d_Wa_s, h->d_Wr_s, h->d_Wmix_s, h->d_scan_scratch, h->d_scan_sync, h->d_w, h->d_phi, h->d_z, h->d_tab, h->d_slabtilegroup, h->d_livelist, h->d_Wa32, h->d_Wmix32, h->d_nz, h->d_zr0, h->d_zmix, h->d_zwr, h->d_zdtr, h->d_olsync, h->d_ollog, h->d_modetab, h->d_lrU, h->d_lrV, h->d_moments, h->d_Wrsets, h->d_Wrsets_s, h->d_mixset, h->d_P0rz};
         for (void* p : ptrs)
             if (p) hipFree(p);
         if (h->h_pub) hipHostFree(h->h_pub);
@@ -875,6 +891,21 @@
     h->cu_count = saved_cus;
     out[0] = ng; out[1] = pl.gemm; out[2] = pl.tail_cols; out[3] = pl.transport; out[4] = pl.parts; out[5] = pl.repair;
     out[6] = pl.order_loop; out[7] = pl.ol_parts; out[8] = pl.ol_grid;
+    h->plan_expand = pl.expand;
+    return 0;
+}
+
+int sosrt_set_expand(sosrt_t* h, int on) {
+    if (!h) return fail(SOSRT_E_INVALID, "null handle");
+    if (on < 0 || on > 2) return fail(SOSRT_E_INVALID, "expand mode must be 0, 1 or 2 (got %d)", on);
+    h->expand = on;
+    return 0;
+}
+
+int sosrt_expand_stats(sosrt_t* h, int* planned, int* launches) {
+    if (!h) return fail(SOSRT_E_INVALID, "null handle");
+    if (planned) *planned = h->plan_expand;
+    if (launches) *launches = h->expanded_launches;
     return 0;
 }
 
@@ -1571,7 +1602,7 @@
         double *In_1 = nullptr, *In = nullptr;
         Conv cv;
     } gs[sosrt_handle::kMaxGroups];
-    h->ol_launches = 0; h->ol_refused = 0;
+    h->ol_launches = 0; h->ol_refused = 0; h->expanded_launches = 0;
     for (bool& u : h->ol_group_used) u = false;
     bool used_order_loop = false;
     const int tagbase = ((++h->pub_seq) & 0x3fff) << 16;
@@ -1752,8 +1783,10 @@
             const int n = ++q.n;
             n_max = n > n_max ? n : n_max;
             const int tail_cols = pl.tail_cols;
+            const bool expand = pl.expand != 0;
+            if (expand) ++h->expanded_launches;
             run_source(h, q.In_1, h->d_Jn, h->d_active, tail_cols, tagbase + n - 1, k, q.known == q.nb, pl.gemm == SOSRT_PLAN_GEMM_LIVE16_REGS,
-                       tail_cols > 0 ? 0 : pl.live_cap);
+                       tail_cols > 0 ? 0 : pl.live_cap, expand);
             if (g.nsmall > 0 && h->need_small) {
                 prof_begin(h, SOSRT_K_SMALLMU, k);
                 launch_smallmu(sg, g, q.nb, tau_g, h->d_Jn + fo, q.In + fo, h->d_desc + q.b0, q.cv.active);
@@ -1767,7 +1800,8 @@
                 launch_transport(sg, gt, q.nb, tau_g, h->d_Jn + fo, q.In + fo, d_I_out + fo, sv_n, saved_stride, h->d_desc + q.b0, q.cv, n, 1,
                                  h->d_E, pl.transport, erep_g, pl.live_cap, h->d_livelist + q.b0, NG > 1 ? h->coresident_slots : 0,
                                  pl.parts > 1 ? 1 : 0, h->d_scan_scratch + (size_t)q.b0 * transport_scan_scratch_doubles(),
-                                 h->d_scan_sync + 2 * q.b0, nzcap);
+                                 h->d_scan_sync + 2 * q.b0, nzcap, expand ? h->d_moments + (size_t)q.b0 * h->L * kMomentRec : nullptr,
+                                 h->lr_rank, h->d_lrV);
                 if (pl.repair)
                     launch_transport(sg, g, q.nb, tau_g, h->d_Jn + fo, q.In + fo, d_I_out + fo, sv_n, saved_stride, h->d_desc + q.b0, q.cv, n, 1,
                                      h->d_E, 2, erep_g);
diff --git a/sos-radiative-transfer_amd/csrc/jn_gemm_tile.hpp b/sos-radiative-transfer_amd/csrc/jn_gemm_tile.hpp
--- a/sos-radiative-transfer_amd/csrc/jn_gemm_tile.hpp
+++ b/sos-radiative-transfer_amd/csrc/jn_gemm_tile.hpp
@@ -366,8 +366,10 @@
 }
 
 constexpr int LR_ROWS = 4;
+constexpr int LR_BLOCKS = 4;
 template <bool COH>
-__device__ __forceinline__ void lowrank_rows(const GemmArgs& g, const int (&rows)[LR_ROWS], int lane) {
+__device__ __forceinline__ void lowrank_rows(const GemmArgs& g, const int (&rows)[LR_ROWS], int lane, unsigned leave = 0) {
+    static_assert(LR_ROWS == 4, "the shared butterfly steps pair four rows");
     const int D = g.D, R = g.lr_rank;
     __amdgpu_buffer_rsrc_t rA[LR_ROWS], rC[LR_ROWS];
     double cf[LR_ROWS];
@@ -376,38 +378,59 @@
         const int r = rows[i] >= 0 ? rows[i] : rows[0];
         const int bytes = rows[i] >= 0 ? D * 8 : 0;
         rA[i] = make_rsrc(g.A + (size_t)r * D, bytes);
-        rC[i] = make_rsrc(g.C + (size_t)r * D, bytes);
+        rC[i] = make_rsrc(g.C + (size_t)r * D, (leave >> i) & 1 ? 0 : bytes);
         cf[i] = rows[i] >= 0 ? g.ca[rows[i]] : 0.0;
     }
     const double* __restrict__ U = g.lrU;
     const double* __restrict__ V = g.lrV;
+    const bool h32 = (lane & 32) != 0, h16 = (lane & 16) != 0;
+    double macc[kLowRankMax];
+#pragma unroll
+    for (int q = 0; q < kLowRankMax; ++q) macc[q] = 0.0;
+    const int nblk = (D + 63) >> 6;
+    for (int b0 = 0; b0 < nblk; b0 += LR_BLOCKS) {
+        double x[LR_BLOCKS][LR_ROWS];
+#pragma unroll
+        for (int j = 0; j < LR_BLOCKS; ++j)
+#pragma unroll
+            for (int i = 0; i < LR_ROWS; ++i) x[j][i] = bload_aux<COH ? 16 : 0>(rA[i], ((b0 + j) * 64 + lane) * 8, 0);
+#pragma unroll
+        for (int j = 0; j < LR_BLOCKS; ++j) {
+            if (b0 + j >= nblk) break;
+            const int k = (b0 + j) * 64 + lane;
+#pragma unroll
+            for (int q = 0; q < kLowRankMax; ++q) {
+                if (q < R) {
+                    const double u = k < D ? U[(size_t)q * D + k] : 0.0;
+                    const double p0 = rec_hr(x[j][0], u), p1 = rec_hr(x[j][1], u), p2 = rec_hr(x[j][2], u), p3 = rec_hr(x[j][3], u);
+                    const double s01 = rec_add(h32 ? p1 : p0, __shfl_xor(h32 ? p0 : p1, 32));
+                    const double s23 = rec_add(h32 ? p3 : p2, __shfl_xor(h32 ? p2 : p3, 32));
+                    double t = rec_add(h16 ? s23 : s01, __shfl_xor(h16 ? s01 : s23, 16));
+#pragma unroll
+                    for (int s = 8; s >= 1; s >>= 1) t = rec_add(t, __shfl_xor(t, s));
+                    macc[q] = rec_add(macc[q], t);
+                }
+            }
+        }
+    }
     double m[LR_ROWS][kLowRankMax];
 #pragma unroll
     for (int i = 0; i < LR_ROWS; ++i)
 #pragma unroll
-        for (int q = 0; q < kLowRankMax; ++q) m[i][q] = 0.0;
-#pragma unroll 2
-    for (int k = 2 * lane; k < D; k += 128) {
-        double2 x[LR_ROWS];
-#pragma unroll
-        for (int i = 0; i < LR_ROWS; ++i) x[i] = bload2_aux<COH ? 16 : 0>(rA[i], k * 8, 0);
-#pragma unroll
-        for (int q = 0; q < kLowRankMax; ++q) {
-            if (q < R) {
-                const double2 u = *reinterpret_cast<const double2*>(U + (size_t)q * D + k);
-#pragma unroll
-                for (int i = 0; i < LR_ROWS; ++i) m[i][q] = __builtin_fma(x[i].y, u.y, __builtin_fma(x[i].x, u.x, m[i][q]));
-            }
-        }
-    }
-#pragma unroll
-    for (int s = 32; s >= 1; s >>= 1)
-#pragma unroll
-        for (int q = 0; q < kLowRankMax; ++q)
-            if (q < R) {
-#pragma unroll
-                for (int i = 0; i < LR_ROWS; ++i) m[i][q] += __shfl_xor(m[i][q], s);
-            }
+        for (int q = 0; q < kLowRankMax; ++q) m[i][q] = q < R ? readlane_f64(macc[q], 32 * (i & 1) + 16 * (i >> 1)) : 0.0;
+    if (leave) {
+        if (lane <= kLowRankMax) {
+#pragma unroll
+            for (int i = 0; i < LR_ROWS; ++i) {
+                if (!((leave >> i) & 1) || rows[i] < 0) continue;
+                double val = cf[i];
+#pragma unroll
+                for (int q = 0; q < kLowRankMax; ++q) val = lane == q ? m[i][q] : val;
+                g.moments[(size_t)rows[i] * kMomentRec + lane] = val;
+            }
+        }
+        if (leave == (1u << LR_ROWS) - 1) return;
+    }
 #pragma unroll 2
     for (int k = 2 * lane; k < D; k += 128) {
         double2 o[LR_ROWS];
@@ -449,7 +472,15 @@
 #pragma unroll
             for (int i = 1; i < LR_ROWS; ++i)
                 if (rows[i] >= 0) { rows[0] = rows[i]; rows[i] = -1; break; }
-        lowrank_rows<COH>(g, rows, lane);
+        unsigned leave = 0;
+        if (!COH && g.moments) {
+#pragma unroll
+            for (int i = 0; i < LR_ROWS; ++i) {
+                const int r = rows[i], b = r >= 0 ? r / g.L : 0;
+                if (r < 0 || row_in_plain_chunks(g.desc[b], g.L, r - b * g.L)) leave |= 1u << i;
+            }
+        }
+        lowrank_rows<COH>(g, rows, lane, leave);
     }
 }
 
diff --git a/sos-radiative-transfer_amd/csrc/kernels.hip b/sos-radiative-transfer_amd/csrc/kernels.hip
--- a/sos-radiative-transfer_amd/csrc/kernels.hip
+++ b/sos-radiative-transfer_amd/csrc/kernels.hip
@@ -1033,12 +1033,14 @@
 void launch_transport(hipStream_t s, const Grid& g, int B, const double* tau, const double* Jn, double* In, double* I,
                       double* saved, size_t saved_col_stride, const ColDesc* desc, Conv cv, int order,
                       int accumulate, const double* Etab, int mode, const int* erep, int live, const int* live_list,
-                      int ring_slots, int scan_split, double* scan_scratch, int* scan_sync, int nzcap) {
+                      int ring_slots, int scan_split, double* scan_scratch, int* scan_sync, int nzcap, const double* moments,
+                      int lr_rank, const double* lrV) {
     const int nt = round64(g.N);
     const size_t shm = (size_t)(g.L + 2 * TC * (nt + 2) + 2 * nt + nt / 64 + 2) * sizeof(double);
     TransportArgs a{g, tau, Jn, In, I, accumulate ? saved : nullptr, saved_col_stride, desc, cv, order, accumulate, Etab, Etab ? erep : nullptr, g_transport_stamps};
     a.slots = ring_slots;
     a.nzcap = nzcap > kRingZones ? nzcap : kRingZones;
+    if (mode == 3 && moments) { a.moments = moments; a.lr_rank = lr_rank; a.lrV = lrV; }
     if (mode == 4 && scan_split && scan_scratch && scan_sync) { a.scan_split = 1; a.scan_scratch = scan_scratch; a.scan_sync = scan_sync; }
     if ((mode == 3 || mode == 4) && accumulate && live > 0 && live < B && live_list) {
         a.live = live;
diff --git a/sos-radiative-transfer_amd/csrc/kernels.hpp b/sos-radiative-transfer_amd/csrc/kernels.hpp
--- a/sos-radiative-transfer_amd/csrc/kernels.hpp
+++ b/sos-radiative-transfer_amd/csrc/kernels.hpp
@@ -111,6 +111,9 @@
     int scan_split = 0;
     double* scan_scratch = nullptr;
     int* scan_sync = nullptr;
+    const double* moments = nullptr;
+    int lr_rank = 0;
+    const double* lrV = nullptr;
 };
 void launch_transport_fast(hipStream_t s, dim3 grid, dim3 block, const TransportArgs& a);
 bool transport_ring_ok(const Grid& g);
@@ -179,8 +182,24 @@
     int lr_rank = -1;
     const double* lrU = nullptr;
     const double* lrV = nullptr;
+    double* moments = nullptr;
+    const ColDesc* desc = nullptr;
 };
 constexpr int kLowRankMax = 4;
+constexpr int kMomentRec = 8, kMomentCa = kLowRankMax;
+__host__ __device__ inline bool row_in_plain_chunks(const ColDesc& d, int L, int t) {
+    const int nch = (L + TC - 1) / TC;
+    if (nch > 64 || L % TC) return false;
+    const int jd = t / TC, ju = (L - 1 - t) / TC;
+    if (jd == nch - 1 || ju == nch - 1) return false;
+    int zone = 0;
+    for (int k = 1; k < d.nz; ++k) {
+        const int rb = d.r0[k], re = rb - 1;
+        if (jd == rb / TC || jd == re / TC || ju == (L - 1 - rb) / TC || ju == (L - 1 - re) / TC) return false;
+        if (t >= rb) zone = k;
+    }
+    return d.mix[zone] == 0;
+}
 
 __device__ inline void publish_live_now(const GemmArgs& g) {
     const int live = __hip_atomic_load(g.nactive, __ATOMIC_RELAXED, __HIP_MEMORY_SCOPE_AGENT);
@@ -238,7 +257,7 @@
                       double* saved, size_t saved_col_stride, const ColDesc* desc, Conv cv, int order, int accumulate,
                       const double* Etab, int mode, const int* erep = nullptr, int live = 0, const int* live_list = nullptr,
                       int ring_slots = 0, int scan_split = 0, double* scan_scratch = nullptr, int* scan_sync = nullptr,
-                      int nzcap = kRingZones);
+                      int nzcap = kRingZones, const double* moments = nullptr, int lr_rank = 0, const double* lrV = nullptr);
 bool transport_fast_ok(const Plan& plan);
 void launch_attenuation(hipStream_t s, const Grid& g, int B, const double* tau, double* Etab, const int* erep);
 void launch_tau_groups(hipStream_t s, const Grid& g, int B, const double* tau, unsigned long long* hash, int* erep,
diff --git a/sos-radiative-transfer_amd/csrc/transport_ring.hip b/sos-radiative-transfer_amd/csrc/transport_ring.hip
--- a/sos-radiative-transfer_amd/csrc/transport_ring.hip
+++ b/sos-radiative-transfer_amd/csrc/transport_ring.hip
@@ -25,9 +25,11 @@
     asm volatile("s_waitcnt lgkmcnt(0)\n\ts_barrier" ::: "memory");
 }
 
-template <bool ACC, bool SAVED, int PIECES, bool MZ>
+template <bool ACC, bool SAVED, int PIECES, bool MZ, bool EXPAND = false>
 __global__ __launch_bounds__(512) void k_transport_ring(TransportArgs a, int NS, int dbg_arg, int fixcap) {
+    static_assert(!EXPAND || (ACC && !SAVED), "the expanding form is an accumulating order without saved orders");
     constexpr int NWL = 2;
+    static_assert(TC * kMomentRec * 8 == NWL * 256, "a loader brings its half of a chunk's records with 16 lanes of 16 bytes");
 #ifdef SOSRT_RING_DEBUG
     const int dbg = dbg_arg;
 #else
@@ -68,6 +70,7 @@
     double* s_x = s_S + (size_t)g.nsmall * L;
     double* s_prmu = s_x + TC * 16;
     int* s_nf = reinterpret_cast<int*>(s_prmu + 16);
+    double* s_M = sm + (((int)(s_prmu + 16 - sm) + (L + 63) / 64 + 1) & ~1);
     const int xb_dn = max(((N - 1) & 63) - 15, 0);
     __shared__ int s_flag[3];
     const ColDesc* __restrict__ dg = a.desc + b;
@@ -84,6 +87,7 @@
     const __amdgpu_buffer_rsrc_t rIl = make_rsrc(ACC ? a.I + (size_t)b * L * D : a.In, ACC ? lbytes : 0);
     const __amdgpu_buffer_rsrc_t rI = make_rsrc(ACC ? a.I + (size_t)b * L * D : a.In, ACC ? sbytes : 0);
     const __amdgpu_buffer_rsrc_t rS = make_rsrc(SAVED ? a.saved + (size_t)b * a.saved_col_stride : a.In, SAVED ? sbytes : 0);
+    const __amdgpu_buffer_rsrc_t rM = make_rsrc(EXPAND ? a.moments + (size_t)b * L * kMomentRec : a.In, EXPAND ? L * kMomentRec * 8 : 0);
     const int NCH = (L + TC - 1) / TC, NQ = 2 * NCH, R = NS - 1;
     const bool valid = tid < N;
     const int tidc = valid ? tid : N - 1;
@@ -92,6 +96,23 @@
         sp_dn |= zr.boundary_chunks(L, TC, false);
         sp_up |= zr.boundary_chunks(L, TC, true);
     }
+    unsigned long long fz_dn = 0, fz_up = 0;
+    if (EXPAND && NCH <= 64) {
+        bool fd = lane < NCH - 1, fu = fd;
+        for (int u = 0; u < TC; ++u) {
+            fd = fd && row_in_plain_chunks(*dg, L, min(lane * TC + u, L - 1));
+            fu = fu && row_in_plain_chunks(*dg, L, max(L - 1 - lane * TC - u, 0));
+        }
+        fz_dn = __ballot(fd) & ~sp_dn;
+        fz_up = __ballot(fu) & ~sp_up;
+    }
+    const int lrR = EXPAND ? a.lr_rank : 0;
+    double vdn[kLowRankMax] = {0, 0, 0, 0}, vup[kLowRankMax] = {0, 0, 0, 0};
+    if (EXPAND) {
+#pragma unroll
+        for (int q = 0; q < kLowRankMax; ++q)
+            if (q < lrR) { vdn[q] = a.lrV[(size_t)q * D + tidc]; vup[q] = a.lrV[(size_t)q * D + N + tidc]; }
+    }
     auto plain_run = [&](unsigned long long mask, int j) {
         const unsigned long long rest = NCH > 64 ? 1ull : mask >> j;
         return rest ? __builtin_ctzll(rest) : 0;
@@ -105,6 +126,12 @@
         const bool up = q >= NCH;
         const int j = up ? q - NCH : q;
         double* dst = ring + (size_t)slot_ld * SLOT;
+        const bool fz = EXPAND && (((up ? fz_up : fz_dn) >> j) & 1);
+        if (EXPAND && fz) {
+            const int r0 = (up ? L - TC - j * TC : j * TC) + lid * (TC / NWL);
+            if (lane < 16)
+                __builtin_amdgcn_raw_ptr_buffer_load_lds(rM, (lds_ptr_t)(s_M + (slot_ld * TC + lid * (TC / NWL)) * kMomentRec), 16, lane * 16, r0 * kMomentRec * 8, 0, 0);
+        }
         slot_ld = slot_ld + 1 == NS ? 0 : slot_ld + 1;
         const int half = up ? N * 8 : 0;
         const int vo = lane * 16;
@@ -115,7 +142,7 @@
 #pragma unroll
             for (int p = 0; p < PIECES; ++p) {
                 const int so = row * RB + half + p * 1024;
-                __builtin_amdgcn_raw_ptr_buffer_load_lds(rJ, (lds_ptr_t)(dst + (0 * TC + u) * RS + p * 128), 16, vo, so, 0, 0);
+                if (!fz) __builtin_amdgcn_raw_ptr_buffer_load_lds(rJ, (lds_ptr_t)(dst + (0 * TC + u) * RS + p * 128), 16, vo, so, 0, 0);
                 __builtin_amdgcn_raw_ptr_buffer_load_lds(rE, (lds_ptr_t)(dst + (1 * TC + u) * RS + p * 128), 16, vo, so, 0, 0);
                 if (ACC) __builtin_amdgcn_raw_ptr_buffer_load_lds(rIl, (lds_ptr_t)(dst + (2 * TC + u) * RS + p * 128), 16, vo, so, 0, 0);
             }
@@ -157,7 +184,7 @@
     const int seam_barriers = surface == SOSRT_SURFACE_NONE ? 0 : (surface == SOSRT_SURFACE_SPECULAR ? 1 : 3);
     double Bv = 0;
     if (loader) {
-        constexpr int PER = IPC / NWL;
+        constexpr int PER = EXPAND ? (NARR - 1) * TC * PIECES / NWL + 1 : IPC / NWL;
         auto run = [&](auto keep_t) {
             loader_phase(keep_t, 0, NCH);
             for (int i = 0; i < seam_barriers; ++i) wg_barrier();
@@ -311,13 +338,21 @@
         };
         auto chunk = [&](auto special_t, auto mode_t) __attribute__((always_inline)) {
             const double* sp = ring + (size_t)slot_rd * SLOT + tid;
+            const double* rec = s_M + slot_rd * TC * kMomentRec;
             slot_rd = slot_rd + 1 == NS ? 0 : slot_rd + 1;
             double Jc[TC], Ic[TC], Ec[TC];
+            const bool fz = EXPAND && !decltype(special_t)::value && ((fz_dn >> q) & 1);
 #pragma unroll
             for (int u = 0; u < TC; ++u) {
-                Jc[u] = sp[(0 * TC + u) * RS];
                 Ec[u] = sp[(1 * TC + u) * RS];
                 Ic[u] = ACC ? sp[(2 * TC + u) * RS] : 0.0;
+            }
+            if (EXPAND && fz) {
+#pragma unroll
+                for (int u = 0; u < TC; ++u) Jc[u] = expand_moments(rec + u * kMomentRec, vdn, lrR);
+            } else {
+#pragma unroll
+                for (int u = 0; u < TC; ++u) Jc[u] = sp[(0 * TC + u) * RS];
             }
             process(special_t, mode_t, sp - tid, Jc, Ic, Ec);
             wg_barrier();
@@ -487,13 +522,21 @@
         };
         auto chunk = [&](auto special_t, auto mode_t) __attribute__((always_inline)) {
             const double* sp = ring + (size_t)slot_rd * SLOT + tid;
+            const double* rec = s_M + slot_rd * TC * kMomentRec;
             slot_rd = slot_rd + 1 == NS ? 0 : slot_rd + 1;
             double Jc[TC], Ic[TC], Ec[TC];
+            const bool fz = EXPAND && !decltype(special_t)::value && ((fz_up >> (q - NCH)) & 1);
 #pragma unroll
             for (int u = 0; u < TC; ++u) {
-                Jc[u] = sp[(0 * TC + u) * RS];
                 Ec[u] = sp[(1 * TC + u) * RS];
                 Ic[u] = ACC ? sp[(2 * TC + u) * RS] : 0.0;
+            }
+            if (EXPAND && fz) {
+#pragma unroll
+                for (int u = 0; u < TC; ++u) Jc[u] = expand_moments(rec + (TC - 1 - u) * kMomentRec, vup, lrR);
+            } else {
+#pragma unroll
+                for (int u = 0; u < TC; ++u) Jc[u] = sp[(0 * TC + u) * RS];
             }
             process(special_t, mode_t, sp - tid, Jc, Ic, Ec);
             wg_barrier();
@@ -529,8 +572,13 @@
         }
     }
     if (s_flag[0]) {
-        const bool missing = redo_upward_sweep<ACC, SAVED, MZ>(L, N, RB, zr, s_hd, g.mu, rJ, rE, rIn, rI, rS, Bv, ring,
-                                                            rup_v, rup_i);
+        bool missing;
+        if constexpr (EXPAND) {
+            ExpandedJ ej{a.moments + (size_t)b * L * kMomentRec, dg, L, lrR, {vup[0], vup[1], vup[2], vup[3]}};
+            missing = redo_upward_sweep<ACC, SAVED, MZ, 0, 0, ExpandedJ>(L, N, RB, zr, s_hd, g.mu, rJ, rE, rIn, rI, rS, Bv, ring, rup_v, rup_i, ej);
+        } else {
+            missing = redo_upward_sweep<ACC, SAVED, MZ>(L, N, RB, zr, s_hd, g.mu, rJ, rE, rIn, rI, rS, Bv, ring, rup_v, rup_i);
+        }
         if (missing) {
             if (tid == 0) {
                 a.cv.status[b] = SOSRT_COL_INDEXERROR;
@@ -557,19 +605,23 @@
 }
 
 inline int ring_fixcap(const Grid& g) { return (int)(0.06 * g.N) + 1; }
-inline size_t ring_extra_doubles(const Grid& g, int nt, int nzcap = kRingZones) {
+constexpr int kRingMaxSlots = 6;
+inline size_t ring_extra_doubles(const Grid& g, int nt, int nzcap = kRingZones, bool expand = false) {
     const int rs = g.N <= 128 ? 128 : 256, fc = nzcap * ring_fixcap(g) * kFixMaxSrc;
-    return (size_t)(rs > fc ? rs : fc) + nt / 64 + 2 + g.L + 1 + (size_t)g.nsmall * g.L + TC * 16 + 16 + (g.L + 63) / 64;
+    return (size_t)(rs > fc ? rs : fc) + nt / 64 + 2 + g.L + 1 + (size_t)g.nsmall * g.L + TC * 16 + 16 + (g.L + 63) / 64 +
+           (expand ? kRingMaxSlots * TC * kMomentRec + 2 : 0);
 }
 
 template <int PIECES>
 void launch_p(hipStream_t s, dim3 grid, dim3 block, const TransportArgs& a, int NS) {
     const int nt = (int)block.x;
     const int narr = a.accumulate ? 3 : 2;
-    const size_t shm = ((size_t)NS * narr * TC * 128 * PIECES + ring_extra_doubles(a.g, nt, a.nzcap)) * sizeof(double);
-#define SOSRT_RING_LAUNCH_Z(ACC_, SAVED_, MZ_)                                                                 \
+    const bool expand = a.moments && a.accumulate && !a.saved;
+    const size_t shm = ((size_t)NS * narr * TC * 128 * PIECES + ring_extra_doubles(a.g, nt, a.nzcap, expand)) * sizeof(double);
+#define SOSRT_RING_LAUNCH_Z(ACC_, SAVED_, MZ_) SOSRT_RING_LAUNCH_E(ACC_, SAVED_, MZ_, false)
+#define SOSRT_RING_LAUNCH_E(ACC_, SAVED_, MZ_, EXP_)                                                           \
     do {                                                                                                       \
-        auto kern = k_transport_ring<ACC_, SAVED_, PIECES, MZ_>;                                               \
+        auto kern = k_transport_ring<ACC_, SAVED_, PIECES, MZ_, EXP_>;                                         \
         static PerDeviceOnce big_lds;                                                                                 \
         if (big_lds.first()) {                                                                                        \
             hipFuncSetAttribute(reinterpret_cast<const void*>(kern), hipFuncAttributeMaxDynamicSharedMemorySize, \
@@ -584,12 +636,17 @@
     } while (0)
     if (a.accumulate) {
         if (a.saved) SOSRT_RING_LAUNCH(true, true);
+        else if (expand) {
+            if (a.nzcap > kRingZones) SOSRT_RING_LAUNCH_E(true, false, true, true);
+            else SOSRT_RING_LAUNCH_E(true, false, false, true);
+        }
         else SOSRT_RING_LAUNCH(true, false);
     } else {
         SOSRT_RING_LAUNCH(false, false);
     }
 #undef SOSRT_RING_LAUNCH
 #undef SOSRT_RING_LAUNCH_Z
+#undef SOSRT_RING_LAUNCH_E
 }
 
 }
@@ -617,8 +674,9 @@
     const int narr = a.accumulate ? 3 : 2;
     const dim3 block((nwc + 2) * 64);
     const size_t slot_bytes = (size_t)narr * TC * 128 * pieces * sizeof(double);
-    const size_t extra = ring_extra_doubles(a.g, (int)block.x, a.nzcap) * sizeof(double);
+    const size_t extra = ring_extra_doubles(a.g, (int)block.x, a.nzcap, a.moments && a.accumulate && !a.saved) * sizeof(double);
     int NS = slots < 2 ? 2 : slots;
+    if (NS > kRingMaxSlots) NS = kRingMaxSlots;
     while (NS > 2 && NS * slot_bytes + extra > kRingLdsBytes) --NS;
     if (pieces == 1) launch_p<1>(s, grid, block, a, NS);
     else launch_p<2>(s, grid, block, a, NS);
diff --git a/sos-radiative-transfer_amd/csrc/transport_util.hpp b/sos-radiative-transfer_amd/csrc/transport_util.hpp
--- a/sos-radiative-transfer_amd/csrc/transport_util.hpp
+++ b/sos-radiative-transfer_amd/csrc/transport_util.hpp
@@ -261,11 +261,30 @@
 }
 
 constexpr int kRedoRows = 8;
-template <bool ACC, bool SAVED, bool MZ, int LDX = 0, int STX = 0>
+__device__ __forceinline__ double expand_moments(const double* rec, const double (&v)[kLowRankMax], int R) {
+    double o = 0.0;
+#pragma unroll
+    for (int q = 0; q < kLowRankMax; ++q)
+        if (q < R) o = __builtin_fma(rec[q], v[q], o);
+    return rec_hr(rec[kMomentCa], o);
+}
+struct StoredJ {
+    __device__ __forceinline__ double operator()(int, double j) const { return j; }
+};
+struct ExpandedJ {
+    const double* rec;
+    const ColDesc* d;
+    int L, R;
+    double v[kLowRankMax];
+    __device__ __forceinline__ double operator()(int t, double j) const {
+        return row_in_plain_chunks(*d, L, t) ? expand_moments(rec + (size_t)t * kMomentRec, v, R) : j;
+    }
+};
+template <bool ACC, bool SAVED, bool MZ, int LDX = 0, int STX = 0, class JOf = StoredJ>
 __device__ SOSRT_HELPER_INLINE bool redo_upward_sweep(int L, int N, int RB, const ZoneRows<MZ>& zr, const double* s_hd,
                                   const double* __restrict__ gmu, __amdgpu_buffer_rsrc_t rJ, __amdgpu_buffer_rsrc_t rE,
                                   __amdgpu_buffer_rsrc_t rIn, __amdgpu_buffer_rsrc_t rI, __amdgpu_buffer_rsrc_t rS, double U0,
-                                  double* s_work, double& rup_v, double& rup_i) {
+                                  double* s_work, double& rup_v, double& rup_i, JOf jof = JOf()) {
     const int tid = threadIdx.x;
     double* s_row = s_work;
     int* s_kf = reinterpret_cast<int*>(s_work + 2 * (N + 2));
@@ -284,7 +303,7 @@
 #pragma unroll
         for (int u = 0; u < kRedoRows; ++u) {
             const int t = max(t0 - u, 0);
-            Jc[u] = bload_aux<LDX>(rJ, vo, t * RB);
+            Jc[u] = jof(t, bload_aux<LDX>(rJ, vo, t * RB));
             Ec[u] = bload(rE, vo, t * RB);
             xo[u] = bload_aux<LDX ? LDX : 1>(rIn, vo, t * RB);
             Io[u] = ACC ? bload_aux<LDX ? LDX : 1>(rI, vo, t * RB) : 0.0;
diff --git a/sos-radiative-transfer_amd/sosrt/_lib.py b/sos-radiative-transfer_amd/sosrt/_lib.py
--- a/sos-radiative-transfer_amd/sosrt/_lib.py
+++ b/sos-radiative-transfer_amd/sosrt/_lib.py
@@ -32,6 +32,8 @@
     "sosrt_set_saved_orders": (c_int, [c_void_p, c_int]),
     "sosrt_set_order_budget": (c_int, [c_void_p, c_int]),
     "sosrt_set_contraction": (c_int, [c_void_p, c_int]),
+    "sosrt_set_expand": (c_int, [c_void_p, c_int]),
+    "sosrt_expand_stats": (c_int, [c_void_p, _ip, _ip]),
     "sosrt_phase_asymmetry": (c_int, [c_void_p, POINTER(c_double), _ip]),
     "sosrt_phase_rank": (c_int, [c_void_p, _ip, POINTER(c_double), _ip]),
     "sosrt_set_order_loop": (c_int, [c_void_p, c_int]),
diff --git a/sos-radiative-transfer_amd/sosrt/solver.py b/sos-radiative-transfer_amd/sosrt/solver.py
--- a/sos-radiative-transfer_amd/sosrt/solver.py
+++ b/sos-radiative-transfer_amd/sosrt/solver.py
@@ -87,6 +87,14 @@
         if m is None:
             raise ValueError("contraction must be 'f64', 'f64_dense', 'f64_full' or 'f32'")
         check(lib().sosrt_set_contraction(self._h, m))
+
+    def set_expand(self, on=True):
+        check(lib().sosrt_set_expand(self._h, int(on)))
+
+    def expand_stats(self):
+        planned, launches = ctypes.c_int(0), ctypes.c_int(0)
+        check(lib().sosrt_expand_stats(self._h, ctypes.byref(planned), ctypes.byref(launches)))
+        return bool(planned.value), launches.value
 
     def set_order_budget(self, max_orders: int):
         check(lib().sosrt_set_order_budget(self._h, int(max_orders)))
```

Measured after the change: 114,200. -3.0%, worse.
